# hsinnan75/Kart

Measured on AMD Instinct MI355X. Metric: mapped reads/sec (whole node), 150 bp PE, higher is better.
Workload: dtype u64

## Files before the change

### include/kart_amd.h

```cpp
#ifndef KART_AMD_H
#define KART_AMD_H

#include <stddef.h>
#include <stdint.h>

#ifdef __cplusplus
extern "C" {
#endif

#define KG_OK                0
#define KG_ERR_NO_DEVICE     1
#define KG_ERR_IO            2
#define KG_ERR_ARG           3
#define KG_ERR_CAPACITY      4
#define KG_ERR_NOMEM         5

#define KG_MODE_FAST         0
#define KG_MODE_SENSITIVE    1
#define KG_INPUT_ASCII    0x100

#define KG_OCC_THR_DEFAULT   50

#define KG_SA_SAMPLED        0
#define KG_SA_FULL           1
// ... 44 lines not shown
	uint64_t double_step_bytes;
} kg_traffic_t;

const char *kg_last_error(void);
int  kg_device_count(void);

int  kg_index_load(const char *prefix, int device, int sa_mode, kg_index **out);
void kg_index_destroy(kg_index *ix);
int  kg_index_info(const kg_index *ix, kg_index_info_t *info);
int  kg_index_contig(const kg_index *ix, int i, kg_contig_t *out);

int  kg_rank_sa_batch(kg_index *ix, const uint64_t *k, int64_t n, uint64_t *occ4, uint64_t *sa_walk, uint64_t *sa_full);
int  kg_index_selfcheck(kg_index *ix, int64_t samples, uint64_t seed, uint64_t *disagreements);

void *kg_host_alloc(size_t bytes);
void  kg_host_free(void *p);

int  kg_workspace_create(kg_index *ix, int64_t max_reads, int64_t max_bases, kg_workspace **out);
void kg_workspace_destroy(kg_workspace *ws);
int  kg_workspace_counters(kg_workspace *ws, kg_counters_t *out);
int  kg_workspace_traffic(kg_workspace *ws, kg_traffic_t *out);
int  kg_workspace_set_single_steps(kg_workspace *ws, int enabled);
int  kg_workspace_set_profiling(kg_workspace *ws, int enabled);
int  kg_workspace_kernel_ms(kg_workspace *ws, float ms[4]);

int  kg_seed_batch(kg_workspace *ws, int mode, int min_seed_len, int occ_thr,
                   const uint8_t *enc_bases, const int64_t *read_offsets, int64_t n_reads,
                   int64_t *seed_offsets, const kg_seed **seeds);

int  kg_seed_batch_device(kg_workspace *ws, int mode, int min_seed_len, int occ_thr,
                          const uint8_t *d_enc_bases, const int64_t *d_read_offsets, int64_t n_reads,
                          int64_t n_bases, int64_t *d_seed_offsets, kg_seed *d_seeds,
                          int64_t seed_capacity, void *stream);
int64_t kg_workspace_overflow(kg_workspace *ws);
int64_t kg_workspace_segment_fallbacks(kg_workspace *ws);

typedef struct {
	int64_t posDiff;
	int32_t score;
	int32_t count;
	int64_t first;
} kg_candidate;
int  kg_candidates_batch(kg_workspace *ws, int pacbio, int max_gaps, int64_t n_reads, int64_t n_seeds, int32_t *n_cands,
                         const kg_candidate **cands, int64_t *n_cands_total, const kg_seed **cand_seeds, int64_t *n_cand_seeds_total);

#define KG_ALN_NONE      0
#define KG_ALN_UNMAPPED  1
#define KG_ALN_MAPPED    2
#define KG_ALN_HOST      3
#define KG_ALN_CIGAR_MAX 48
typedef struct {
	int64_t pos;
	int64_t mate_pos;
	int32_t kind;
	int32_t flag, chr, mapq, tlen;
	int32_t score, sub_score;
	int32_t est_lo, est_hi;
	uint8_t has_mate;
	uint8_t flip;
	uint8_t cigar_len;
	uint8_t rescue;
	char    cigar[KG_ALN_CIGAR_MAX];
	int32_t next;
	uint8_t primary;
	uint8_t pad[3];
} kg_aln_record;

typedef struct {
	int64_t paired, distance;
	int64_t lo, hi;
	int32_t unmapped, unique;
	int32_t host_pairs;
	int32_t rescue_wanted;
} kg_chunk_stats;

int  kg_align_batch(kg_workspace *ws, const int64_t *chunk_off, const uint8_t *chunk_paired, int n_chunks,
                    int est_distance, int max_insert, int max_gaps, int multi_hit, int unset_flag,
                    const kg_aln_record **records, kg_chunk_stats *chunk_stats);

#define KG_STATS_RECORDS      0
#define KG_STATS_FLAG0        1
#define KG_STATS_FLAG_BITS    12
#define KG_STATS_PROPER       13
#define KG_STATS_BOTH_MAPPED  14
#define KG_STATS_SINGLETON    15
#define KG_STATS_CIGAR0       16
#define KG_STATS_CIGAR_CLASSES 5
#define KG_STATS_MAPQ0        26
#define KG_STATS_MAPQ_BINS    64
#define KG_STATS_ISIZE0       90
#define KG_STATS_ISIZE_MAX    2048
#define KG_STATS_WORDS        (KG_STATS_ISIZE0 + KG_STATS_ISIZE_MAX + 1)
int  kg_tally_records(const kg_aln_record *records, int64_t n_records, int64_t n_reads, const int64_t *chunk_off, int n_chunks, uint32_t *rows);

#define KG_ALN_CIGAR_POOLED 255
int  kg_longread_batch(kg_workspace *ws, const kg_aln_record **records, const char **cigar_pool, int64_t *cigar_bytes, int64_t *n_host_reads);
int  kg_longread_reasons(kg_workspace *ws, uint64_t out[16]);

int  kg_align_reasons(kg_workspace *ws, uint64_t out[16]);

#define KG_OP_DIAG 0
#define KG_OP_GAP1 1
#define KG_OP_GAP2 2
int  kg_nw_batch(kg_index *ix, const char *frag1, const int64_t *off1, const char *frag2,
                 const int64_t *off2, int64_t n, uint8_t *ops, int32_t *aln_len);
int  kg_nw_batch_device(kg_index *ix, const char *d_frag1, const int64_t *d_off1, const char *d_frag2,
                        const int64_t *d_off2, int64_t n, int64_t max_len, uint8_t *d_ops,
                        int32_t *d_aln_len, void *stream);

int  kg_fragments_batch(kg_index *ix, const char *frag1, const int64_t *off1, const int64_t *gpos, const int32_t *glen, int64_t n,
                        int pacbio, int max_gaps, uint8_t *ops, const int64_t *ops_off, int32_t *aln_len, uint8_t *status);

int  kg_bgzf_deflate(int device, const uint8_t *src, int64_t src_bytes, const int64_t *cuts, int64_t n_cuts,
                     uint8_t *dst, int64_t dst_capacity, int64_t *block_src, int64_t *block_off, int64_t max_blocks, int64_t *n_blocks);

#define KG_INFLATE_OK      0
#define KG_INFLATE_HEADER  1
#define KG_INFLATE_STREAM  2
#define KG_INFLATE_SIZE    3
#define KG_INFLATE_CRC     4
int  kg_bgzf_inflate(int device, const uint8_t *src, int64_t src_bytes, const int64_t *member_off, const int64_t *text_off,
                     int64_t n_members, uint8_t *dst, int64_t dst_capacity, int32_t *status);
typedef struct kg_inflater kg_inflater;
int  kg_inflater_create(int device, int64_t max_src_bytes, int64_t max_text_bytes, int64_t max_members, kg_inflater **out);
int  kg_inflater_reserve(kg_inflater *k, int64_t src_bytes, int64_t text_bytes, int64_t members);
uint8_t *kg_inflater_src(kg_inflater *k);
int  kg_inflater_run(kg_inflater *k, int64_t src_bytes, const int64_t *member_off, const int64_t *text_off, int64_t n_members,
                     const uint8_t **text, const int32_t **status, double *device_ms);
void kg_inflater_destroy(kg_inflater *k);

typedef struct kg_stream kg_stream;
typedef struct {
	int64_t max_reads;
	int64_t max_window;
	int32_t lanes;
	int32_t seed_group;
} kg_stream_config;
int   kg_stream_open(kg_index *ix, const kg_stream_config *cfg, kg_stream **out);
void  kg_stream_close(kg_stream *s);
#define KG_STREAM_FORMAT_SAM 0
#define KG_STREAM_FORMAT_BAM 1
#define KG_STREAM_FORMAT_BAM_BGZF 2
int   kg_stream_set_format(kg_stream *s, int format);
#define KG_STREAM_INPUT_FASTQ 0
#define KG_STREAM_INPUT_FASTA 1
int   kg_stream_set_input(kg_stream *s, int input);
#define KG_STREAM_TAG_MD 1
int   kg_stream_set_tags(kg_stream *s, int tags);
int   kg_stream_set_read_group(kg_stream *s, const char *id, int len);
int   kg_stream_set_unmapped(kg_stream *s, int on);
int   kg_stream_set_stats(kg_stream *s, int on);
char *kg_stream_staging(kg_stream *s, int lane, int file, int64_t *capacity);
int   kg_stream_upload(kg_stream *s, int lane, int file, int64_t from, int64_t to);

typedef struct {
	int64_t begin[2], end[2];
	int32_t eof[2];
	int32_t two_files;
	int32_t paired;
	int32_t chunk_reads;
	int32_t gz_lines;
	int64_t want_reads;
} kg_stream_window;
#define KG_STREAM_STOP_NONE      0
#define KG_STREAM_STOP_IRREGULAR 1
#define KG_STREAM_STOP_TAIL      2
typedef struct {
	int64_t n_reads, n_chunks, n_bases;
	int64_t used[2];
	int32_t stop;
	int32_t done;
} kg_stream_parsed;
int   kg_stream_parse(kg_stream *s, int lane, const kg_stream_window *w, kg_stream_parsed *out);

typedef struct {
	int32_t est_distance, max_insert, max_gaps, multi_hit, unset_flag;
	int32_t fetch_all;
} kg_stream_params;
typedef struct {
	int64_t n_reads, n_chunks;
	const char *sam;
	int64_t sam_bytes;
	const int64_t *sam_off;
	const kg_aln_record *records;
	int64_t n_records;
	const kg_chunk_stats *chunk_stats;
	const int32_t *host_reads;
	int64_t n_host_reads;
	const int64_t *cand_off;
	const kg_candidate *cands;
	const kg_seed *cand_seeds;
	const uint32_t *rec_start[2];
	const uint8_t *bgzf;
	int64_t bgzf_bytes;
	int64_t n_blocks;
	const int64_t *block_src;
	const int64_t *block_off;
	const uint8_t *un[2];
	int64_t un_bytes[2];
	const int64_t *un_off[2];
	int64_t n_units;
	const uint32_t *chunk_tally;
} kg_stream_result;
int   kg_stream_map(kg_stream *s, int lane, const kg_stream_params *prm, kg_stream_result *out);
int   kg_stream_fetch(kg_stream *s, int lane, int64_t first, int64_t count);
int   kg_stream_group_absent(kg_stream *s, int lane, int rounds);
int   kg_stream_group_abort(kg_stream *s);
int   kg_stream_fetch_reads(kg_stream *s, int lane, uint8_t *enc, int64_t *read_off);

typedef struct {
	int64_t batches, reads;
	double parse_ms, seed_ms, chain_ms, align_ms, format_ms, copy_ms;
	double search_kernel_ms;
	int64_t search_kernel_launches;
	double search_useful_bytes;
	double text_in_bytes, text_out_bytes;
	double candidates, candidate_seeds;
	double kernel_ms[16];
	int64_t kernel_launches[16];
	double aln_counts[8];
	double text_checksum[2];
	double un_kernel_ms[2];
	int64_t un_kernel_launches[2];
	double un_bytes;
	double stats_kernel_ms;
	int64_t stats_kernel_launches;
	double stats_bytes;
} kg_stream_timing_t;
int   kg_stream_timing(kg_stream *s, kg_stream_timing_t *out, int reset);

#ifdef __cplusplus
}
#endif
#endif
```

### kart_amd/api.py

```python
from __future__ import annotations

import ctypes as C
import os
import sys

import numpy as np

_HERE = os.path.dirname(os.path.abspath(__file__))
LIB_PATH = os.path.join(_HERE, "libkart_amd.so")

KG_OK = 0
KG_MODE_FAST, KG_MODE_SENSITIVE = 0, 1
KG_INPUT_ASCII = 0x100
KG_SA_SAMPLED, KG_SA_FULL = 0, 1
KG_STREAM_FORMAT_SAM, KG_STREAM_FORMAT_BAM, KG_STREAM_FORMAT_BAM_BGZF = 0, 1, 2
KG_STREAM_INPUT_FASTQ, KG_STREAM_INPUT_FASTA = 0, 1
KG_STREAM_TAG_MD = 1
KG_SA_AUTO = -1
KG_SA_FULL40 = 5
KG_SA_FULL40_WIDE = 6
KG_SA_DENSE4, KG_SA_DENSE8 = 4, 8
KG_OCC_THR_DEFAULT = 50
KG_OP_DIAG, KG_OP_GAP1, KG_OP_GAP2 = 0, 1, 2

SEED_DT = np.dtype([("gPos", "<i8"), ("rPos", "<i4"), ("len", "<i4")])
CAND_DT = np.dtype([("posDiff", "<i8"), ("score", "<i4"), ("count", "<i4"), ("first", "<i8")])
KG_ALN_NONE, KG_ALN_UNMAPPED, KG_ALN_MAPPED, KG_ALN_HOST = 0, 1, 2, 3
KG_ALN_CIGAR_MAX = 48
ALN_DT = np.dtype([("pos", "<i8"), ("mate_pos", "<i8"), ("kind", "<i4"), ("flag", "<i4"), ("chr", "<i4"), ("mapq", "<i4"), ("tlen", "<i4"),
                   ("score", "<i4"), ("sub_score", "<i4"), ("est_lo", "<i4"), ("est_hi", "<i4"), ("has_mate", "u1"), ("flip", "u1"), ("cigar_len", "u1"),
                   ("rescue", "u1"), ("cigar", "S%d" % KG_ALN_CIGAR_MAX), ("next", "<i4"), ("primary", "u1"), ("pad", "u1", (3,))])
CHUNK_STATS_DT = np.dtype([("paired", "<i8"), ("distance", "<i8"), ("lo", "<i8"), ("hi", "<i8"), ("unmapped", "<i4"), ("unique", "<i4"),
                           ("host_pairs", "<i4"), ("rescue_wanted", "<i4")])
assert ALN_DT.itemsize == 112 and CHUNK_STATS_DT.itemsize == 48
KG_STATS_RECORDS, KG_STATS_FLAG0, KG_STATS_FLAG_BITS, KG_STATS_PROPER, KG_STATS_BOTH_MAPPED, KG_STATS_SINGLETON = 0, 1, 12, 13, 14, 15
KG_STATS_CIGAR0, KG_STATS_CIGAR_CLASSES, KG_STATS_MAPQ0, KG_STATS_MAPQ_BINS, KG_STATS_ISIZE0, KG_STATS_ISIZE_MAX = 16, 5, 26, 64, 90, 2048
KG_STATS_WORDS = KG_STATS_ISIZE0 + KG_STATS_ISIZE_MAX + 1

ABI_SYMBOLS = (
    "kg_last_error", "kg_device_count", "kg_index_load", "kg_index_destroy", "kg_index_info",
    "kg_index_contig", "kg_host_alloc", "kg_host_free", "kg_rank_sa_batch", "kg_workspace_create", "kg_workspace_destroy", "kg_workspace_counters", "kg_workspace_traffic",
    "kg_workspace_overflow", "kg_workspace_segment_fallbacks", "kg_workspace_set_profiling", "kg_workspace_set_single_steps", "kg_index_selfcheck", "kg_workspace_kernel_ms", "kg_seed_batch", "kg_candidates_batch", "kg_align_batch", "kg_align_reasons", "kg_seed_batch_device", "kg_nw_batch", "kg_nw_batch_device",
    "kg_fragments_batch", "kg_longread_batch", "kg_longread_reasons",
    "kg_stream_open", "kg_stream_close", "kg_stream_staging", "kg_stream_upload", "kg_stream_parse", "kg_stream_map", "kg_stream_fetch", "kg_stream_fetch_reads", "kg_stream_timing",
    "kg_stream_group_absent", "kg_stream_group_abort", "kg_stream_set_format", "kg_stream_set_input", "kg_stream_set_tags", "kg_stream_set_read_group", "kg_stream_set_unmapped",
    "kg_stream_set_stats", "kg_tally_records",
    "kg_bgzf_deflate", "kg_bgzf_inflate", "kg_inflater_create", "kg_inflater_reserve", "kg_inflater_src", "kg_inflater_run", "kg_inflater_destroy",
)


HOST_LIB_PATH = os.path.join(_HERE, "libkart_host.so")
HOST_ABI_SYMBOLS = ("kh_last_error", "kh_open", "kh_map", "kh_close")


class KartAmdError(RuntimeError):
    pass


class IndexInfo(C.Structure):
    _fields_ = [("genome_size", C.c_int64), ("seq_len", C.c_uint64), ("primary", C.c_uint64),
                ("n_contigs", C.c_int32), ("min_seed_len", C.c_int32), ("sa_mode", C.c_int32),
                ("device", C.c_int32), ("device_bytes", C.c_uint64)]


class Contig(C.Structure):
    _fields_ = [("name", C.c_char_p), ("fwd_start", C.c_int64), ("rev_start", C.c_int64), ("len", C.c_int64)]


class Counters(C.Structure):
    _fields_ = [(n, C.c_uint64) for n in ("searches", "lf1", "lf2", "inv", "sa", "seeds", "bases")]

    def as_dict(self):
        return {n: int(getattr(self, n)) for n, _ in self._fields_}

    def algorithmic_bytes(self) -> int:
        return 64 * (self.lf1 + 2 * self.lf2 + self.inv) + 8 * self.sa + self.bases + 16 * self.seeds


class Traffic(C.Structure):
    _fields_ = [(n, C.c_uint64) for n in ("table_lookups", "rank_steps", "rank_steps_two_lines", "sa_gathers", "text_rounds", "window_words",
                                          "hits", "searches", "sa_entry_bytes", "rank_steps_two_lines_narrow", "double_steps", "double_steps_two_lines",
                                          "triple_steps", "double_step_bytes")]

    def as_dict(self):
        return {n: int(getattr(self, n)) for n, _ in self._fields_}

    def useful_bytes(self, n_reads: int) -> int:
        return (8 * self.table_lookups + 32 * self.rank_steps + self.double_step_bytes + self.sa_entry_bytes * self.sa_gathers + 48 * self.text_rounds
                + 8 * self.window_words + 20 * n_reads + 32 * self.hits)

    def min_lines(self, n_reads: int) -> int:
        return int(self.table_lookups + self.rank_steps + self.rank_steps_two_lines + self.double_steps + self.double_steps_two_lines + self.sa_gathers + self.text_rounds * (1.125 + 1.25)
                   + (8 * self.window_words + 20 * n_reads + 32 * self.hits) / 128)


class StreamConfig(C.Structure):
    _fields_ = [("max_reads", C.c_int64), ("max_window", C.c_int64), ("lanes", C.c_int32), ("seed_group", C.c_int32)]


class StreamWindow(C.Structure):
    _fields_ = [("begin", C.c_int64 * 2), ("end", C.c_int64 * 2), ("eof", C.c_int32 * 2), ("two_files", C.c_int32), ("paired", C.c_int32),
                ("chunk_reads", C.c_int32), ("gz_lines", C.c_int32), ("want_reads", C.c_int64)]


class StreamParsed(C.Structure):
    _fields_ = [("n_reads", C.c_int64), ("n_chunks", C.c_int64), ("n_bases", C.c_int64), ("used", C.c_int64 * 2), ("stop", C.c_int32), ("done", C.c_int32)]


class StreamParams(C.Structure):
    _fields_ = [(n, C.c_int32) for n in ("est_distance", "max_insert", "max_gaps", "multi_hit", "unset_flag", "fetch_all")]


class StreamResult(C.Structure):
    _fields_ = [("n_reads", C.c_int64), ("n_chunks", C.c_int64), ("sam", C.c_void_p), ("sam_bytes", C.c_int64), ("sam_off", C.POINTER(C.c_int64)),
                ("records", C.c_void_p), ("n_records", C.c_int64), ("chunk_stats", C.c_void_p), ("host_reads", C.POINTER(C.c_int32)), ("n_host_reads", C.c_int64),
                ("cand_off", C.POINTER(C.c_int64)), ("cands", C.c_void_p), ("cand_seeds", C.c_void_p), ("rec_start", C.POINTER(C.c_uint32) * 2),
                ("bgzf", C.c_void_p), ("bgzf_bytes", C.c_int64), ("n_blocks", C.c_int64), ("block_src", C.POINTER(C.c_int64)), ("block_off", C.POINTER(C.c_int64)),
                ("un", C.c_void_p * 2), ("un_bytes", C.c_int64 * 2), ("un_off", C.POINTER(C.c_int64) * 2), ("n_units", C.c_int64),
                ("chunk_tally", C.POINTER(C.c_uint32))]


class StreamTiming(C.Structure):
    _fields_ = [("batches", C.c_int64), ("reads", C.c_int64)] + [(n, C.c_double) for n in ("parse_ms", "seed_ms", "chain_ms", "align_ms", "format_ms", "copy_ms", "search_kernel_ms")] + \
               [("search_kernel_launches", C.c_int64)] + [(n, C.c_double) for n in ("search_useful_bytes", "text_in_bytes", "text_out_bytes", "candidates", "candidate_seeds")] + \
               [("kernel_ms", C.c_double * 16), ("kernel_launches", C.c_int64 * 16), ("aln_counts", C.c_double * 8), ("text_checksum", C.c_double * 2),
                ("un_kernel_ms", C.c_double * 2), ("un_kernel_launches", C.c_int64 * 2), ("un_bytes", C.c_double),
                ("stats_kernel_ms", C.c_double), ("stats_kernel_launches", C.c_int64), ("stats_bytes", C.c_double)]

    def as_dict(self):
        return {n: (list(getattr(self, n)) if n.startswith(("kernel_", "aln_counts", "un_kernel_")) else getattr(self, n)) for n, _ in self._fields_}


_lib = None


def _check_one_hip_runtime(L):
    try:
        paths = {l.split()[-1] for l in open("/proc/self/maps") if "libamdhip64" in l}
    except OSError:
        return
    if len({os.path.realpath(p_) for p_ in paths}) > 1 and "torch" in sys.modules and L.kg_device_count() <= 0:
        raise KartAmdError("two HIP runtimes are loaded in this process (%s): import torch BEFORE kart_amd.api.load_library(), or set KART_AMD_NO_TORCH=1 and do "
                           "not import torch afterwards" % ", ".join(sorted(paths)))


def load_library() -> C.CDLL:
    global _lib
    if _lib is not None:
        return _lib
    if not os.path.exists(LIB_PATH):
        raise KartAmdError(f"{LIB_PATH} is missing: build it with `python -c 'import __graft_entry__ as g; g.build()'` "
                           "(there is no CPU fallback)")
    if "torch" not in sys.modules and not os.environ.get("KART_AMD_NO_TORCH"):
        try:
            import torch
        except Exception:
            pass
    L = C.CDLL(LIB_PATH)
    _check_one_hip_runtime(L)
    L.kg_last_error.restype = C.c_char_p
    L.kg_index_load.argtypes = [C.c_char_p, C.c_int, C.c_int, C.POINTER(C.c_void_p)]
    L.kg_index_destroy.argtypes = [C.c_void_p]
    L.kg_index_destroy.restype = None
    L.kg_index_info.argtypes = [C.c_void_p, C.POINTER(IndexInfo)]
    L.kg_index_contig.argtypes = [C.c_void_p, C.c_int, C.POINTER(Contig)]
    L.kg_rank_sa_batch.argtypes = [C.c_void_p, C.c_void_p, C.c_int64, C.c_void_p, C.c_void_p, C.c_void_p]
    L.kg_workspace_create.argtypes = [C.c_void_p, C.c_int64, C.c_int64, C.POINTER(C.c_void_p)]
    L.kg_workspace_destroy.argtypes = [C.c_void_p]
    L.kg_workspace_destroy.restype = None
    L.kg_workspace_counters.argtypes = [C.c_void_p, C.POINTER(Counters)]
    L.kg_workspace_traffic.argtypes = [C.c_void_p, C.POINTER(Traffic)]
    L.kg_workspace_overflow.argtypes = [C.c_void_p]
    L.kg_workspace_set_profiling.argtypes = [C.c_void_p, C.c_int]
    L.kg_workspace_set_single_steps.argtypes = [C.c_void_p, C.c_int]
    L.kg_index_selfcheck.argtypes = [C.c_void_p, C.c_int64, C.c_uint64, C.POINTER(C.c_uint64)]
    L.kg_workspace_kernel_ms.argtypes = [C.c_void_p, C.POINTER(C.c_float * 4)]
    L.kg_workspace_overflow.restype = C.c_int64
    L.kg_workspace_segment_fallbacks.argtypes = [C.c_void_p]
    L.kg_workspace_segment_fallbacks.restype = C.c_int64
    L.kg_seed_batch.argtypes = [C.c_void_p, C.c_int, C.c_int, C.c_int, C.c_void_p, C.c_void_p, C.c_int64,
                                C.c_void_p, C.POINTER(C.c_void_p)]
    L.kg_seed_batch_device.argtypes = [C.c_void_p, C.c_int, C.c_int, C.c_int, C.c_void_p, C.c_void_p, C.c_int64,
                                       C.c_int64, C.c_void_p, C.c_void_p, C.c_int64, C.c_void_p]
    L.kg_candidates_batch.argtypes = [C.c_void_p, C.c_int, C.c_int, C.c_int64, C.c_int64, C.c_void_p, C.POINTER(C.c_void_p), C.POINTER(C.c_int64),
                                      C.POINTER(C.c_void_p), C.POINTER(C.c_int64)]
    L.kg_align_batch.argtypes = [C.c_void_p, C.c_void_p, C.c_void_p, C.c_int, C.c_int, C.c_int, C.c_int, C.c_int, C.c_int, C.POINTER(C.c_void_p), C.c_void_p]
    L.kg_align_reasons.argtypes = [C.c_void_p, C.c_void_p]
    L.kg_nw_batch.argtypes = [C.c_void_p, C.c_void_p, C.c_void_p, C.c_void_p, C.c_void_p, C.c_int64, C.c_void_p, C.c_void_p]
    L.kg_nw_batch_device.argtypes = [C.c_void_p, C.c_void_p, C.c_void_p, C.c_void_p, C.c_void_p, C.c_int64, C.c_int64,
                                     C.c_void_p, C.c_void_p, C.c_void_p]
    L.kg_fragments_batch.argtypes = [C.c_void_p, C.c_void_p, C.c_void_p, C.c_void_p, C.c_void_p, C.c_int64, C.c_int, C.c_int, C.c_void_p, C.c_void_p, C.c_void_p, C.c_void_p]
    L.kg_stream_open.argtypes = [C.c_void_p, C.POINTER(StreamConfig), C.POINTER(C.c_void_p)]
    L.kg_stream_close.argtypes = [C.c_void_p]
    L.kg_stream_close.restype = None
    L.kg_stream_staging.argtypes = [C.c_void_p, C.c_int, C.c_int, C.POINTER(C.c_int64)]
    L.kg_stream_staging.restype = C.c_void_p
    L.kg_stream_upload.argtypes = [C.c_void_p, C.c_int, C.c_int, C.c_int64, C.c_int64]
    L.kg_stream_parse.argtypes = [C.c_void_p, C.c_int, C.POINTER(StreamWindow), C.POINTER(StreamParsed)]
    L.kg_stream_map.argtypes = [C.c_void_p, C.c_int, C.POINTER(StreamParams), C.POINTER(StreamResult)]
    L.kg_stream_fetch.argtypes = [C.c_void_p, C.c_int, C.c_int64, C.c_int64]
    L.kg_stream_fetch_reads.argtypes = [C.c_void_p, C.c_int, C.c_void_p, C.c_void_p]
    L.kg_stream_group_absent.argtypes = [C.c_void_p, C.c_int, C.c_int]
    L.kg_stream_group_abort.argtypes = [C.c_void_p]
    L.kg_stream_set_format.argtypes = [C.c_void_p, C.c_int]
    L.kg_stream_set_input.argtypes = [C.c_void_p, C.c_int]
    L.kg_stream_set_tags.argtypes = [C.c_void_p, C.c_int]
    L.kg_stream_set_read_group.argtypes = [C.c_void_p, C.c_char_p, C.c_int]
    L.kg_stream_set_unmapped.argtypes = [C.c_void_p, C.c_int]
    L.kg_stream_set_stats.argtypes = [C.c_void_p, C.c_int]
    L.kg_tally_records.argtypes = [C.c_void_p, C.c_int64, C.c_int64, C.c_void_p, C.c_int, C.c_void_p]
    L.kg_stream_timing.argtypes = [C.c_void_p, C.POINTER(StreamTiming), C.c_int]
    L.kg_bgzf_deflate.argtypes = [C.c_int, C.c_void_p, C.c_int64, C.c_void_p, C.c_int64, C.c_void_p, C.c_int64, C.c_void_p, C.c_void_p, C.c_int64, C.POINTER(C.c_int64)]
    L.kg_bgzf_inflate.argtypes = [C.c_int, C.c_void_p, C.c_int64, C.c_void_p, C.c_void_p, C.c_int64, C.c_void_p, C.c_int64, C.c_void_p]
    L.kg_inflater_create.argtypes = [C.c_int, C.c_int64, C.c_int64, C.c_int64, C.POINTER(C.c_void_p)]
    L.kg_inflater_reserve.argtypes = [C.c_void_p, C.c_int64, C.c_int64, C.c_int64]
    L.kg_inflater_src.argtypes = [C.c_void_p]
    L.kg_inflater_src.restype = C.c_void_p
    L.kg_inflater_run.argtypes = [C.c_void_p, C.c_int64, C.c_void_p, C.c_void_p, C.c_int64, C.POINTER(C.c_void_p), C.POINTER(C.c_void_p), C.POINTER(C.c_double)]
    L.kg_inflater_destroy.argtypes = [C.c_void_p]
    L.kg_inflater_destroy.restype = None
    _lib = L
    return L


def _check(rc: int, what: str):
    if rc != KG_OK:
        raise KartAmdError(f"{what} failed (status {rc}): {load_library().kg_last_error().decode()}")


def device_count() -> int:
    return int(load_library().kg_device_count())


def _ptr(a):
    return a.ctypes.data_as(C.c_void_p)


BGZF_PAYLOAD = 0xff00


def bgzf_deflate(data: bytes, cuts=None, device: int = 0, dst_capacity: int | None = None, max_blocks: int | None = None):
    cuts = np.ascontiguousarray([0, len(data)] if cuts is None else cuts, dtype=np.int64)
    spans = np.maximum(np.diff(cuts), 0)
    need = int(((spans + BGZF_PAYLOAD - 1) // BGZF_PAYLOAD).sum())
    max_blocks = need if max_blocks is None else int(max_blocks)
    dst_capacity = len(data) + 31 * need if dst_capacity is None else int(dst_capacity)
    src = np.frombuffer(data, dtype=np.uint8) if len(data) else np.zeros(1, dtype=np.uint8)
    dst = np.zeros(max(1, dst_capacity), dtype=np.uint8)
    block_src = np.zeros(max_blocks + 1, dtype=np.int64)
    block_off = np.zeros(max_blocks + 1, dtype=np.int64)
    n = C.c_int64()
    _check(load_library().kg_bgzf_deflate(device, _ptr(src), len(data), _ptr(cuts), len(cuts), _ptr(dst), dst_capacity, _ptr(block_src), _ptr(block_off),
                                          max_blocks, C.byref(n)), "kg_bgzf_deflate")
    return dst[:int(block_off[n.value])].tobytes(), block_src[:n.value + 1].copy(), block_off[:n.value + 1].copy()


KG_INFLATE_OK, KG_INFLATE_HEADER, KG_INFLATE_STREAM, KG_INFLATE_SIZE, KG_INFLATE_CRC = 0, 1, 2, 3, 4
BGZF_MEMBER_MAX = 65536


def bgzf_members(data: bytes):
    member_off, text_off, at = [0], [0], 0
    while at < len(data):
        size = 0
        if len(data) - at >= 18 and data[at:at + 2] == b"\x1f\x8b":
            xlen = int.from_bytes(data[at + 10:at + 12], "little")
            x = at + 12
            while x + 6 <= min(at + 12 + xlen, len(data)):
                slen = int.from_bytes(data[x + 2:x + 4], "little")
                if data[x:x + 2] == b"BC" and slen == 2:
                    size = int.from_bytes(data[x + 4:x + 6], "little") + 1
                    break
                x += 4 + slen
        if size < 8 or at + size > len(data):
            raise KartAmdError(f"no whole BGZF member at byte {at}")
        isize = int.from_bytes(data[at + size - 4:at + size], "little")
        at += size
        member_off.append(at)
        text_off.append(text_off[-1] + (isize if isize <= BGZF_MEMBER_MAX else 0))
    return np.asarray(member_off, dtype=np.int64), np.asarray(text_off, dtype=np.int64)


def bgzf_inflate(data: bytes, member_off=None, text_off=None, device: int = 0, dst_capacity: int | None = None):
    if member_off is None:
        member_off, text_off = bgzf_members(data)
    member_off = np.ascontiguousarray(member_off, dtype=np.int64)
    if text_off is None:
        sizes = [int.from_bytes(data[e - 4:e], "little") if e >= 4 else 0 for e in member_off[1:].tolist()]
        text_off = np.concatenate([[0], np.cumsum([s if s <= BGZF_MEMBER_MAX else 0 for s in sizes], dtype=np.int64)])
    text_off = np.ascontiguousarray(text_off, dtype=np.int64)
    if len(member_off) < 1 or len(member_off) != len(text_off):
        raise KartAmdError("bgzf_inflate: member_off and text_off are tables of n + 1 offsets each")
    n = len(member_off) - 1
    dst_capacity = int(text_off[-1]) if dst_capacity is None else int(dst_capacity)
    src = np.frombuffer(data, dtype=np.uint8) if len(data) else np.zeros(1, dtype=np.uint8)
    dst = np.zeros(max(1, dst_capacity), dtype=np.uint8)
    status = np.full(max(1, n), -1, dtype=np.int32)
    _check(load_library().kg_bgzf_inflate(device, _ptr(src), len(data), _ptr(member_off), _ptr(text_off), n, _ptr(dst), dst_capacity, _ptr(status)),
           "kg_bgzf_inflate")
    return dst[:int(text_off[-1])].tobytes(), text_off.copy(), status[:n].copy()


class Inflater:

    def __init__(self, max_src_bytes: int, max_text_bytes: int, max_members: int, device: int = 0):
        self.lib = load_library()
        h = C.c_void_p()
        _check(self.lib.kg_inflater_create(device, max_src_bytes, max_text_bytes, max_members, C.byref(h)), "kg_inflater_create")
        self.h = h
        self.src_room = max_src_bytes

    def reserve(self, src_bytes: int, text_bytes: int, members: int):
        _check(self.lib.kg_inflater_reserve(self.h, src_bytes, text_bytes, members), "kg_inflater_reserve")
        self.src_room = max(self.src_room, src_bytes)

    def run(self, data: bytes, member_off, text_off):
        member_off = np.ascontiguousarray(member_off, dtype=np.int64)
        text_off = np.ascontiguousarray(text_off, dtype=np.int64)
        n = len(member_off) - 1
        src = self.lib.kg_inflater_src(self.h)
        if 0 < len(data) <= self.src_room and src:
            C.memmove(src, data, len(data))
        text, status, ms = C.c_void_p(), C.c_void_p(), C.c_double()
        _check(self.lib.kg_inflater_run(self.h, len(data), _ptr(member_off), _ptr(text_off), n, C.byref(text), C.byref(status), C.byref(ms)), "kg_inflater_run")
        out = C.string_at(text, int(text_off[-1])) if n and text_off[-1] else b""
        st = np.frombuffer(C.string_at(status, 4 * n), dtype=np.int32).copy() if n else np.zeros(0, dtype=np.int32)
        return out, st, ms.value

    def close(self):
        if self.h:
            self.lib.kg_inflater_destroy(self.h)
            self.h = None


def concat_reads(reads):
    lens = np.fromiter((len(r) for r in reads), dtype=np.int64, count=len(reads))
    offsets = np.zeros(len(reads) + 1, dtype=np.int64)
    np.cumsum(lens, out=offsets[1:])
    enc = np.concatenate(reads).astype(np.uint8, copy=False) if len(reads) else np.zeros(0, dtype=np.uint8)
    return np.ascontiguousarray(enc), offsets


class Workspace:
    def __init__(self, index: "Index", max_reads: int, max_bases: int):
        self.index = index
        self.lib = index.lib
        h = C.c_void_p()
        _check(self.lib.kg_workspace_create(index.h, max_reads, max_bases, C.byref(h)), "kg_workspace_create")
        self.h = h
        self.max_reads, self.max_bases = max_reads, max_bases
# ... 139 lines not shown

    def selfcheck(self, samples: int = 1 << 20, seed: int = 1) -> int:
        bad = C.c_uint64(0)
        _check(self.lib.kg_index_selfcheck(self.h, samples, seed, C.byref(bad)), "kg_index_selfcheck")
        return int(bad.value)

    def rank_sa(self, ks):
        ks = np.ascontiguousarray(ks, dtype=np.uint64)
        n = len(ks)
        occ4 = np.zeros((n, 4), dtype=np.uint64)
        walk = np.zeros(n, dtype=np.uint64)
        full = np.zeros(n, dtype=np.uint64)
        _check(self.lib.kg_rank_sa_batch(self.h, _ptr(ks), n, _ptr(occ4), _ptr(walk), _ptr(full)), "kg_rank_sa_batch")
        return occ4, walk, full

    def _seed(self, reads, mode, min_seed_len, occ_thr):
        enc, offsets = concat_reads(reads)
        ws = self.workspace(len(reads), len(enc))
        so, seeds = ws.seed_batch(enc, offsets, mode, min_seed_len, occ_thr)
        return [seeds[so[i]:so[i + 1]] for i in range(len(reads))]

    def IdentifySeedPairs_FastMode(self, reads, min_seed_len=None, occ_thr=KG_OCC_THR_DEFAULT):
        return self._seed(reads, KG_MODE_FAST, min_seed_len, occ_thr)

    def IdentifySeedPairs_SensitiveMode(self, reads, min_seed_len=None, occ_thr=KG_OCC_THR_DEFAULT):
        return self._seed(reads, KG_MODE_SENSITIVE, min_seed_len, occ_thr)

    def nw_ops(self, pairs):
        n = len(pairs)
        if n == 0:
            return []
        off1 = np.zeros(n + 1, dtype=np.int64)
        off2 = np.zeros(n + 1, dtype=np.int64)
        np.cumsum([len(a) for a, _ in pairs], out=off1[1:])
        np.cumsum([len(b) for _, b in pairs], out=off2[1:])
        f1 = np.frombuffer(b"".join(a for a, _ in pairs) + b"\0", dtype=np.uint8).copy()
        f2 = np.frombuffer(b"".join(b for _, b in pairs) + b"\0", dtype=np.uint8).copy()
        ops = np.zeros(int(off1[n] + off2[n]) + 1, dtype=np.uint8)
        alen = np.zeros(n, dtype=np.int32)
        _check(self.lib.kg_nw_batch(self.h, _ptr(f1), _ptr(off1), _ptr(f2), _ptr(off2), n, _ptr(ops), _ptr(alen)), "kg_nw_batch")
        oo = off1 + off2
        return [ops[oo[i]:oo[i] + alen[i]].copy() for i in range(n)]

    def fragments_ops(self, frags, gpos, glen, pacbio=True, max_gaps=5):
        n = len(frags)
        if n == 0:
            return [], np.zeros(0, np.uint8)
        off1 = np.zeros(n + 1, dtype=np.int64)
        np.cumsum([len(a) for a in frags], out=off1[1:])
        f1 = np.frombuffer(b"".join(frags) + b"\0" * 64, dtype=np.uint8).copy()
        g = np.ascontiguousarray(gpos, dtype=np.int64)
        gl = np.ascontiguousarray(glen, dtype=np.int32)
        oo = np.zeros(n + 1, dtype=np.int64)
        np.cumsum(np.diff(off1) + gl, out=oo[1:])
        ops = np.zeros(int(oo[n]) + 64, dtype=np.uint8)
        alen = np.zeros(n, dtype=np.int32)
        status = np.zeros(n, dtype=np.uint8)
        _check(self.lib.kg_fragments_batch(self.h, _ptr(f1), _ptr(off1), _ptr(g), _ptr(gl), n, int(pacbio), max_gaps, _ptr(ops), _ptr(oo), _ptr(alen), _ptr(status)), "kg_fragments_batch")
        return [ops[oo[i]:oo[i] + alen[i]].copy() for i in range(n)], status

    def GenerateNormalPairAlignment(self, frags, gpos, glen, text, pacbio=True, max_gaps=5):
        ops, status = self.fragments_ops(frags, gpos, glen, pacbio, max_gaps)
        out = []
        for i, a in enumerate(frags):
            out.append(None if status[i] else apply_ops(a, bytes(text[int(gpos[i]):int(gpos[i]) + int(glen[i])]), ops[i]))
        return out, status

    def nw_alignment(self, pairs):
        out = []
        for (s1, s2), ops in zip(pairs, self.nw_ops(pairs)):
            out.append(apply_ops(s1, s2, ops))
        return out


class Stream:

    FORMATS = {"sam": KG_STREAM_FORMAT_SAM, "bam": KG_STREAM_FORMAT_BAM, "bgzf": KG_STREAM_FORMAT_BAM_BGZF}
    INPUTS = {"fastq": KG_STREAM_INPUT_FASTQ, "fasta": KG_STREAM_INPUT_FASTA}

    def __init__(self, index: "Index", max_reads: int = 16000, max_window: int = 8 << 20, lanes: int = 1, seed_group: int = 0):
        self.lib = load_library()
        self.index = index
        cfg = StreamConfig(max_reads, max_window, lanes, seed_group)
        h = C.c_void_p()
        _check(self.lib.kg_stream_open(index.h, C.byref(cfg), C.byref(h)), "kg_stream_open")
        self.h = h
        self.max_window = max_window
        self.last_blocks = None
        self._last_un = {}
        self._last_stats = {}

    def close(self):
        if self.h:
            self.lib.kg_stream_close(self.h)
            self.h = None

    def set_format(self, fmt):
        _check(self.lib.kg_stream_set_format(self.h, self.FORMATS.get(fmt, fmt) if isinstance(fmt, str) else int(fmt)), "kg_stream_set_format")

    def set_input(self, kind):
        _check(self.lib.kg_stream_set_input(self.h, self.INPUTS.get(kind, -1) if isinstance(kind, str) else int(kind)), "kg_stream_set_input")

    def set_tags(self, md: bool = False):
        _check(self.lib.kg_stream_set_tags(self.h, KG_STREAM_TAG_MD if md else 0), "kg_stream_set_tags")

    def set_read_group(self, id):
        if id is None:
            _check(self.lib.kg_stream_set_read_group(self.h, None, 0), "kg_stream_set_read_group")
            return
        try:
            raw = id.encode("ascii") if isinstance(id, str) else bytes(id)
        except UnicodeEncodeError as e:
            raise KartAmdError("kg_stream_set_read_group: the ID holds a character outside '!'..'~': %s" % e) from None
        _check(self.lib.kg_stream_set_read_group(self.h, raw, len(raw)), "kg_stream_set_read_group")

    def set_unmapped(self, on: bool):
        _check(self.lib.kg_stream_set_unmapped(self.h, 1 if on else 0), "kg_stream_set_unmapped")

    def last_unmapped(self, lane: int = 0):
        return self._last_un.get(lane, [])

    def set_stats(self, on: bool):
        _check(self.lib.kg_stream_set_stats(self.h, 1 if on else 0), "kg_stream_set_stats")

    def last_stats(self, lane: int = 0):
        return self._last_stats.get(lane)

    def group_absent(self, lane: int, rounds: int):
        _check(self.lib.kg_stream_group_absent(self.h, lane, rounds), "kg_stream_group_absent")

    def group_abort(self):
        _check(self.lib.kg_stream_group_abort(self.h), "kg_stream_group_abort")

    def parse(self, text1: bytes, text2: bytes | None = None, paired: bool = True, chunk_reads: int = 4000, want_reads: int | None = None,
              eof=(True, True), begin=(0, 0), lane: int = 0, gz_lines: int = 0) -> StreamParsed:
        w = StreamWindow()
        texts = [text1] + ([text2] if text2 is not None else [])
        for f, t in enumerate(texts):
            cap = C.c_int64()
            p = self.lib.kg_stream_staging(self.h, lane, f, C.byref(cap))
            assert p and begin[f] + len(t) <= cap.value
            C.memmove(p + begin[f], t, len(t))
            w.begin[f], w.end[f], w.eof[f] = begin[f], begin[f] + len(t), 1 if eof[f] else 0
            _check(self.lib.kg_stream_upload(self.h, lane, f, begin[f], begin[f] + len(t)), "kg_stream_upload")
        w.two_files = 1 if text2 is not None else 0
        w.paired = 1 if paired else 0
        w.chunk_reads = chunk_reads
        w.gz_lines = 1 if gz_lines else 0
        w.want_reads = want_reads if want_reads is not None else chunk_reads
        out = StreamParsed()
        _check(self.lib.kg_stream_parse(self.h, lane, C.byref(w), C.byref(out)), "kg_stream_parse")
        return out

    def fetch_reads(self, parsed: StreamParsed, lane: int = 0):
        off = np.zeros(parsed.n_reads + 1, dtype=np.int64)
        enc = np.zeros(max(1, parsed.n_bases), dtype=np.uint8)
        _check(self.lib.kg_stream_fetch_reads(self.h, lane, _ptr(enc), _ptr(off)), "kg_stream_fetch_reads")
        raw = enc.tobytes()
        return [raw[off[i]:off[i + 1]] for i in range(parsed.n_reads)]

    def map(self, est_distance: int = 1500, max_insert: int = 1500, max_gaps: int = 5, multi_hit: bool = False, unset_flag: int = 0, lane: int = 0):
        prm = StreamParams(est_distance, max_insert, max_gaps, 1 if multi_hit else 0, unset_flag, 1)
        res = StreamResult()
        _check(self.lib.kg_stream_map(self.h, lane, C.byref(prm), C.byref(res)), "kg_stream_map")
        n = res.n_reads
        off = np.ctypeslib.as_array(res.sam_off, shape=(n + 1,)).copy()
        sam = C.string_at(res.sam, res.sam_bytes)
        host = [int(res.host_reads[i]) for i in range(res.n_host_reads)]
        self._last_un[lane] = [(C.string_at(res.un[f], res.un_bytes[f]) if res.un_bytes[f] else b"", np.ctypeslib.as_array(res.un_off[f], shape=(res.n_units + 1,)).copy())
                               for f in range(2) if res.un_off[f]]
        self._last_stats[lane] = np.ctypeslib.as_array(res.chunk_tally, shape=(int(res.n_chunks), KG_STATS_WORDS)).copy() if res.chunk_tally else None
        self.last_blocks = None
        if res.block_src:
            nb = res.n_blocks
            self.last_blocks = (C.string_at(res.bgzf, res.bgzf_bytes), np.ctypeslib.as_array(res.block_src, shape=(nb + 1,)).copy(),
                                np.ctypeslib.as_array(res.block_off, shape=(nb + 1,)).copy())
        return [sam[off[i]:off[i + 1]] for i in range(n)], host

    def timing(self, reset: bool = False) -> dict:
        t = StreamTiming()
        _check(self.lib.kg_stream_timing(self.h, C.byref(t), 1 if reset else 0), "kg_stream_timing")
        return t.as_dict()


def tally_records(records, n_reads: int, chunk_off):
    lib = load_library()
    recs = np.ascontiguousarray(records, dtype=ALN_DT)
    off = np.ascontiguousarray(chunk_off, dtype=np.int64)
    rows = np.zeros((max(0, len(off) - 1), KG_STATS_WORDS), dtype=np.uint32)
    _check(lib.kg_tally_records(_ptr(recs) if len(recs) else None, len(recs), int(n_reads), _ptr(off), len(off) - 1, _ptr(rows) if rows.size else _ptr(np.zeros(1, np.uint32))),
           "kg_tally_records")
    return rows


def apply_ops(s1: bytes, s2: bytes, ops: np.ndarray):
    a, b = bytearray(), bytearray()
    i = j = 0
    for op in ops:
        if op == KG_OP_DIAG:
            a.append(s1[i]); b.append(s2[j]); i += 1; j += 1
        elif op == KG_OP_GAP1:
            a.append(0x2D); b.append(s2[j]); j += 1
        else:
            a.append(s1[i]); b.append(0x2D); i += 1
    assert i == len(s1) and j == len(s2), "op string does not consume both fragments"
    return bytes(a), bytes(b)


class HostStats(C.Structure):
    _fields_ = [("total_reads", C.c_int64), ("unmapped", C.c_int64), ("unique", C.c_int64), ("paired", C.c_int64), ("distance", C.c_int64),
                ("respeculated", C.c_int64), ("map_seconds", C.c_double), ("sharded", C.c_int32), ("pad", C.c_int32),
                ("stream_reads", C.c_int64), ("stream_batches", C.c_int64), ("stage_ms", C.c_double * 6), ("search_kernel_ms", C.c_double),
                ("search_kernel_launches", C.c_int64), ("search_useful_bytes", C.c_double), ("text_in_bytes", C.c_double), ("text_out_bytes", C.c_double),
                ("candidates", C.c_double), ("candidate_seeds", C.c_double), ("kernel_ms", C.c_double * 16), ("kernel_launches", C.c_int64 * 16), ("aln_counts", C.c_double * 8),
                ("lane_seconds", C.c_double * 6), ("lanes", C.c_int32), ("pad2", C.c_int32), ("text_checksum", C.c_double * 2),
                ("bgzf_device_bytes", C.c_int64), ("bgzf_host_bytes", C.c_int64),
                ("inflate_device_bytes", C.c_int64), ("inflate_host_bytes", C.c_int64), ("inflate_device_ms", C.c_double),
                ("un_kernel_ms", C.c_double * 2), ("un_kernel_launches", C.c_int64 * 2), ("un_bytes", C.c_double),
                ("stats_kernel_ms", C.c_double), ("stats_kernel_launches", C.c_int64), ("stats_bytes", C.c_double)]

    def as_dict(self):
        return {n: (list(getattr(self, n)) if n.startswith(("kernel_", "stage_", "aln_counts", "un_kernel_")) else getattr(self, n)) for n, _ in self._fields_}


_host_lib = None


def load_host_library() -> C.CDLL:
    global _host_lib
    if _host_lib is not None:
        return _host_lib
    if not os.path.exists(HOST_LIB_PATH):
        raise KartAmdError(f"{HOST_LIB_PATH} is missing: build it with `python -c 'import __graft_entry__ as g; g.build()'`")
    load_library()
    L = C.CDLL(HOST_LIB_PATH)
    L.kh_last_error.restype = C.c_char_p
    L.kh_open.argtypes = [C.c_char_p, C.c_int, C.c_int, C.POINTER(C.c_void_p)]
    L.kh_map.argtypes = [C.c_void_p, C.c_int, C.POINTER(C.c_char_p), C.POINTER(HostStats)]
    L.kh_close.argtypes = [C.c_void_p]
    L.kh_close.restype = None
    _host_lib = L
    return L


class HostSession:

    def __init__(self, prefix: str, device: int = 0, threads: int = 4):
        self.lib = load_host_library()
        h = C.c_void_p()
        if self.lib.kh_open(prefix.encode(), device, threads, C.byref(h)) != 0:
            raise KartAmdError("kh_open failed: " + self.lib.kh_last_error().decode())
        self.h = h

    def map(self, args) -> HostStats:
        argv = (C.c_char_p * len(args))(*[str(a).encode() for a in args])
        st = HostStats()
        if self.lib.kh_map(self.h, len(args), argv, C.byref(st)) != 0:
            raise KartAmdError("kh_map failed: " + self.lib.kh_last_error().decode())
        return st

    def close(self):
        if self.h:
            self.lib.kh_close(self.h)
            self.h = None
```

### kart_amd/csrc/abi_stream.hip

```cpp
#include "abi_internal.hpp"
#include "stream_kernels.hpp"
#include "un_kernels.hpp"
#include "stats_kernels.hpp"
#include "bgzf_kernels.hpp"

#include <algorithm>
#include <chrono>
#include <condition_variable>
#include <cstdlib>
#include <cstring>
#include <memory>

#define fail kg_fail

namespace {

enum LaneWord {
	LW_TEXT_BYTES = 0,
	LW_HOST_READS = 1,
	LW_FORMAT_ERRORS = 2,
	LW_EXTRA_RECORDS = 3,
	LW_ALN_COUNTS = 8,
	LW_ALN_TRIVIAL = 14,
	LW_ALN_GENERAL = 15,
	LW_CHECKSUM = 16,
	LW_FETCH_SEEDS = 18,
	LW_BGZF = 20,
	LW_UN_BYTES = 24,
	LW_UN_CTL = 26,
	LW_WORDS = 32
};

struct Lane {
	kg_workspace *ws = nullptr;
	uint8_t *d_text[2] = {nullptr, nullptr};
	int32_t *d_tile[2] = {nullptr, nullptr};
	uint32_t *d_line_end[2] = {nullptr, nullptr};
	uint32_t *d_rec[2] = {nullptr, nullptr};
	uint64_t *d_line_acc[2] = {nullptr, nullptr};
	uint32_t *d_rec_line[2] = {nullptr, nullptr};
	int64_t *d_meta = nullptr;
	int32_t *d_read_len = nullptr;
	void *d_scan = nullptr;
	size_t scan_bytes = 0;
	int32_t *d_sam_len = nullptr, *d_host_list = nullptr;
	int64_t *d_sam_off = nullptr;
	unsigned long long *d_sam_ctl = nullptr;
	uint8_t *d_sam = nullptr;
	int64_t d_sam_capacity = 0;
	int64_t *d_cuts = nullptr, *d_range_first = nullptr;
	int64_t *d_block_src = nullptr, *d_block_off = nullptr;
	int32_t *d_block_bytes = nullptr;
	uint8_t *d_slots = nullptr, *d_bgzf = nullptr;
	int64_t bgzf_blocks = 0, d_bgzf_capacity = 0;
	unsigned long long *d_bgzf_ctl = nullptr;
	void *d_bgzf_scan = nullptr;
	size_t bgzf_scan_bytes = 0;
	int32_t *d_un_len[2] = {nullptr, nullptr};
	int64_t *d_un_off[2] = {nullptr, nullptr};
	uint8_t *d_un[2] = {nullptr, nullptr};
	int64_t d_un_capacity[2] = {0, 0};
	unsigned long long *d_un_ctl = nullptr;
	int64_t *h_un_off[2] = {nullptr, nullptr};
	uint8_t *h_un[2] = {nullptr, nullptr};
	int64_t h_un_capacity[2] = {0, 0};
	uint32_t *d_tally = nullptr, *h_tally = nullptr;
	int64_t tally_capacity = 0, h_tally_capacity = 0;
	uint8_t *h_bgzf = nullptr;
	int64_t h_bgzf_capacity = 0;
	int64_t *h_block_src = nullptr, *h_block_off = nullptr;
	char *h_text[2] = {nullptr, nullptr};
	int64_t *h_meta = nullptr;
	char *h_sam = nullptr;
	int64_t h_sam_capacity = 0;
	int64_t *h_sam_off = nullptr, *h_cand_off = nullptr;
	int32_t *h_host_list = nullptr;
	uint32_t *h_rec_hdr[2] = {nullptr, nullptr};
	kg_aln_record *h_records = nullptr;
	int64_t record_capacity = 0;
	kg_chunk_stats *h_chunk_stats = nullptr;
	int64_t chunk_capacity = 0;
	kg_candidate *h_cands = nullptr;
	kg_seed *h_cand_seeds = nullptr;
	int64_t h_cand_capacity = 0;
	unsigned long long *h_ctl = nullptr;
	int64_t mapped_reads = 0;
	const kg_aln_record *d_records = nullptr;
	kg_stream_window win{};
	kg_stream_parsed parsed{};
	bool have_batch = false;
	bool fasta = false;
	hipEvent_t ev[8] = {nullptr, nullptr, nullptr, nullptr, nullptr, nullptr, nullptr, nullptr};
	hipEvent_t ev_parsed = nullptr;
};

struct SeedGroup {
	int first = 0, size = 0;
	int64_t stride = 0, seg_bases = 0;
	kg_workspace *ws = nullptr;
	unsigned long long *h_ctl = nullptr;
	std::mutex mu;
	std::condition_variable cv;
	int64_t round = 0;
	int arrived = 0;
	bool present[kMaxSeedSegments] = {false};
	int absent_rounds[kMaxSeedSegments] = {0};
	int64_t n_reads[kMaxSeedSegments] = {0};
	int rc = KG_OK;
	int64_t seed_base[kMaxSeedSegments + 1] = {0};
	bool aborted = false;
	int order[kMaxSeedSegments] = {0};
	int n_order = 0, turn = 0;
};

struct GroupTurn {
	SeedGroup *sg = nullptr;
	bool held = false;
	bool acquire(SeedGroup &g, int j)
	{
		sg = &g;
		std::unique_lock<std::mutex> lk(g.mu);
		g.cv.wait(lk, [&]() { return g.aborted || (g.turn < g.n_order && g.order[g.turn] == j); });
		held = !g.aborted;
		return held;
	}
	void release()
	{
		if (!held) return;
		held = false;
		std::lock_guard<std::mutex> lk(sg->mu);
		sg->turn++;
		sg->cv.notify_all();
	}
	~GroupTurn() { release(); }
};

}

struct kg_stream {
	kg_index *ix = nullptr;
	kg_stream_config cfg{};
	int64_t text_capacity = 0, line_capacity = 0, rec_capacity = 0;
	std::vector<Lane> lanes;
	std::vector<std::unique_ptr<SeedGroup>> groups;
	uint8_t *d_chr_names = nullptr;
	int32_t *d_chr_name_off = nullptr;
	int min_seed_len = 13;
	int format = KG_STREAM_FORMAT_SAM;
	int input = KG_STREAM_INPUT_FASTQ;
	int tags = 0;
	bool unmapped = false;
	bool stats = false;
	uint8_t *d_rg = nullptr;
	int rg_len = 0;
	bool fasta_sized = false;
	std::mutex mu;
	kg_stream_timing_t total{};
};

namespace {

void free_lane(Lane &l)
{
	if (l.ws && l.ws->enc_borrowed) l.ws->d_enc = nullptr;
	if (l.ev_parsed) (void)hipEventDestroy(l.ev_parsed);
	if (l.ws) kg_workspace_destroy(l.ws);
	for (int f = 0; f < 2; ++f) {
		if (l.d_text[f]) (void)hipFree(l.d_text[f]);
		if (l.d_tile[f]) (void)hipFree(l.d_tile[f]);
		if (l.d_line_end[f]) (void)hipFree(l.d_line_end[f]);
		if (l.d_rec[f]) (void)hipFree(l.d_rec[f]);
		if (l.d_line_acc[f]) (void)hipFree(l.d_line_acc[f]);
		if (l.d_rec_line[f]) (void)hipFree(l.d_rec_line[f]);
		if (l.h_text[f]) (void)hipHostFree(l.h_text[f]);
		if (l.h_rec_hdr[f]) (void)hipHostFree(l.h_rec_hdr[f]);
		for (void *p : {(void *)l.d_un_len[f], (void *)l.d_un_off[f], (void *)l.d_un[f]})
			if (p) (void)hipFree(p);
		for (void *p : {(void *)l.h_un_off[f], (void *)l.h_un[f]})
			if (p) (void)hipHostFree(p);
	}
	if (l.d_un_ctl) (void)hipFree(l.d_un_ctl);
	if (l.d_tally) (void)hipFree(l.d_tally);
	if (l.h_tally) (void)hipHostFree(l.h_tally);
	for (void *p : {(void *)l.d_meta, (void *)l.d_read_len, l.d_scan, (void *)l.d_sam_len, (void *)l.d_host_list, (void *)l.d_sam_off, (void *)l.d_sam_ctl, (void *)l.d_sam,
	                (void *)l.d_cuts, (void *)l.d_range_first, (void *)l.d_block_src, (void *)l.d_block_off, (void *)l.d_block_bytes, (void *)l.d_slots, (void *)l.d_bgzf,
	                (void *)l.d_bgzf_ctl, l.d_bgzf_scan})
		if (p) (void)hipFree(p);
	for (void *p : {(void *)l.h_meta, (void *)l.h_sam, (void *)l.h_sam_off, (void *)l.h_cand_off, (void *)l.h_host_list, (void *)l.h_records, (void *)l.h_chunk_stats,
	                (void *)l.h_cands, (void *)l.h_cand_seeds, (void *)l.h_ctl, (void *)l.h_bgzf, (void *)l.h_block_src, (void *)l.h_block_off})
		if (p) (void)hipHostFree(p);
	for (hipEvent_t e : l.ev)
		if (e) (void)hipEventDestroy(e);
	l = Lane();
}

FqWindow window_of(const kg_stream *s, const Lane &l, int f)
{
	FqWindow w;
	w.text = l.d_text[f];
	w.begin = l.win.begin[f]; w.end = l.win.end[f]; w.eof = l.win.eof[f];
	w.tile_lines = l.d_tile[f];
	w.line_end = l.d_line_end[f];
	w.line_capacity = s->line_capacity;
	uint32_t *r = l.d_rec[f];
	const size_t c = (size_t)s->rec_capacity;
	w.rec_hdr = r; w.rec_name = r + c; w.rec_seq = r + 2 * c; w.rec_qual = r + 3 * c;
	w.rec_rlen = (int32_t *)(r + 4 * c); w.rec_qlen = (int32_t *)(r + 5 * c);
	w.rec_capacity = s->rec_capacity;
	w.line_acc = l.d_line_acc[f]; w.rec_line = l.d_rec_line[f];
	return w;
}

int64_t out_capacity(const kg_stream_config &cfg, int format)
{
	return 2 * cfg.max_window + (format != KG_STREAM_FORMAT_SAM ? 144 : 64) * cfg.max_reads + 4096;
}

constexpr int kRgMaxId = 255, kRgBamAt = 512, kRgBytes = 1024;
static_assert(6 + kRgMaxId + 16 <= kRgBamAt && kRgBamAt + 4 + kRgMaxId + 16 <= kRgBytes, "both forms of the longest ID and their slack must fit");

int64_t out_capacity(const kg_stream_config &cfg, int format, int tags)
{
	return out_capacity(cfg, format) + ((tags & KG_STREAM_TAG_MD) ? 32 : 0) * cfg.max_reads;
}

enum GrowOrder { kFreeFirst, kAllocFirst };
template <class T> hipError_t grow_device(T *&p, size_t bytes, GrowOrder order = kFreeFirst)
{
	T *old = p;
	if (order == kFreeFirst) {
		if (old) { hipError_t e = hipFree(old); if (e != hipSuccess) return e; }
		p = old = nullptr;
	}
	T *fresh = nullptr;
	hipError_t e = hipMalloc((void **)&fresh, bytes);
	if (e != hipSuccess) return e;
	if (old) (void)hipFree(old);
	p = fresh;
	return hipSuccess;
}
template <class T> hipError_t grow_pinned(T *&p, size_t bytes)
{
	if (p) { hipError_t e = hipHostFree(p); if (e != hipSuccess) return e; }
	p = nullptr;
	return hipHostMalloc((void **)&p, bytes, hipHostMallocDefault);
}

double search_useful_bytes(const kg_index *ix, const unsigned long long *c, int64_t reads)
{
	const double sa_bytes = ix->view.fsa32 ? 4.0 : 8.0;
	return 8.0 * (double)c[17] + 32.0 * (double)c[18] + (double)c[25] + sa_bytes * (double)c[8] + 48.0 * (double)c[20] + 8.0 * (double)c[21] + 20.0 * (double)reads + 32.0 * (double)c[1];
}

template <class T, class C> hipError_t grow_device(T *&p, C &capacity, C want, size_t bytes)
{
	hipError_t e = grow_device(p, bytes);
	capacity = e == hipSuccess ? want : p ? capacity : 0;
	return e;
}
template <class T, class C> hipError_t grow_pinned(T *&p, C &capacity, C want, size_t bytes)
{
	hipError_t e = grow_pinned(p, bytes);
	capacity = e == hipSuccess ? want : p ? capacity : 0;
	return e;
}

bool round_complete(const SeedGroup &sg)
{
	int accounted = sg.arrived;
	for (int i = 0; i < sg.size; ++i) accounted += (!sg.present[i] && sg.absent_rounds[i] != 0) ? 1 : 0;
	return accounted >= sg.size;
}

float elapsed(hipEvent_t a, hipEvent_t b)
{
	float ms = 0;
	if (hipEventElapsedTime(&ms, a, b) != hipSuccess) { (void)hipGetLastError(); return 0; }
	return ms;
}

}

extern "C" {

int kg_stream_open(kg_index *ix, const kg_stream_config *cfg, kg_stream **out)
{
	if (!ix || !cfg || !out) return fail(KG_ERR_ARG, "kg_stream_open: null argument");
	*out = nullptr;
	if (cfg->lanes < 1 || cfg->lanes > 16 || cfg->max_reads < 2 || cfg->max_window < 4096 || cfg->max_window > 0xF0000000ll)
		return fail(KG_ERR_ARG, "kg_stream_open: bad configuration (%d lanes, %lld reads, %lld bytes per window)", cfg->lanes, (long long)cfg->max_reads, (long long)cfg->max_window);
	const int group = cfg->seed_group > 1 ? cfg->seed_group : 0;
	if (group && (group > kMaxSeedSegments || cfg->lanes % group != 0))
		return fail(KG_ERR_ARG, "kg_stream_open: seed_group %d must divide the %d lanes and be at most %d", group, cfg->lanes, kMaxSeedSegments);
	if (!ix->d_text) return fail(KG_ERR_ARG, "kg_stream_open: the index holds no text");
	HIP_TRY(hipSetDevice(ix->device));
	std::unique_ptr<kg_stream, void (*)(kg_stream *)> s(new kg_stream(), kg_stream_close);
	s->ix = ix;
	s->cfg = *cfg;
	s->text_capacity = (cfg->max_window + 4096 + 255) & ~255ll;
	s->line_capacity = cfg->max_window / 16 + 4096;
	s->rec_capacity = s->line_capacity / 4 + 1;
	{
		kg_index_info_t info;
		kg_index_info(ix, &info);
		s->min_seed_len = info.min_seed_len;
		std::vector<int32_t> off{0};
		std::string names;
		for (const ContigRec &c : ix->contigs) { names += c.name; off.push_back((int32_t)names.size()); }
		HIP_TRY(hipMalloc((void **)&s->d_chr_names, names.size() + 16));
		HIP_TRY(hipMalloc((void **)&s->d_chr_name_off, 4 * off.size()));
		HIP_TRY(hipMemcpy(s->d_chr_names, names.data(), names.size(), hipMemcpyHostToDevice));
		HIP_TRY(hipMemcpy(s->d_chr_name_off, off.data(), 4 * off.size(), hipMemcpyHostToDevice));
		HIP_TRY(hipMalloc((void **)&s->d_rg, kRgBytes));
		HIP_TRY(hipMemset(s->d_rg, 0, kRgBytes));
	}
	s->lanes.resize((size_t)cfg->lanes);
	const int64_t n = cfg->max_reads;
	const int64_t seg_bases = (cfg->max_window + 4096 + 64 + 255) & ~255ll;
	for (int g = 0; group && g < cfg->lanes / group; ++g) {
		s->groups.push_back(std::unique_ptr<SeedGroup>(new SeedGroup()));
		SeedGroup *sg = s->groups.back().get();
		sg->first = g * group; sg->size = group;
		sg->stride = n + 8; sg->seg_bases = seg_bases;
		int rc = kg_workspace_create(ix, sg->stride * group, seg_bases * group, &sg->ws);
		if (rc != KG_OK) return rc;
		kg_workspace *gw = sg->ws;
		HIP_TRY(hipMalloc((void **)&gw->d_enc, (size_t)gw->max_bases + 64));
		HIP_TRY(hipMalloc((void **)&gw->d_read_off, 8 * (size_t)(gw->max_reads + 1)));
		HIP_TRY(hipMalloc((void **)&gw->d_seed_off, 8 * (size_t)(gw->max_reads + 1)));
		HIP_TRY(hipMalloc((void **)&gw->group_read_len, 4 * (size_t)(gw->max_reads + 1)));
		HIP_TRY(hipMemsetAsync(gw->d_enc, 'N', (size_t)gw->max_bases + 64, gw->stream));
		HIP_TRY(hipMemsetAsync(gw->d_read_off, 0, 8 * (size_t)(gw->max_reads + 1), gw->stream));
		HIP_TRY(hipMemsetAsync(gw->group_read_len, 0, 4 * (size_t)(gw->max_reads + 1), gw->stream));
		HIP_TRY(hipStreamSynchronize(gw->stream));
		HIP_TRY(hipHostMalloc((void **)&sg->h_ctl, 8 * kCtlWords, hipHostMallocDefault));
		(void)kg_workspace_set_profiling(gw, 1);
	}
	for (size_t li = 0; li < s->lanes.size(); ++li) {
		Lane &l = s->lanes[li];
		int rc = kg_workspace_create(ix, n + 8, cfg->max_window + 4096, &l.ws);
		if (rc != KG_OK) return rc;
		kg_workspace *ws = l.ws;
		if (group) {
			SeedGroup &sg = *s->groups[li / (size_t)group];
			ws->d_enc = sg.ws->d_enc + (int64_t)(li % (size_t)group) * sg.seg_bases;
			ws->enc_borrowed = true;
			HIP_TRY(hipEventCreateWithFlags(&l.ev_parsed, hipEventDisableTiming));
		} else
		HIP_TRY(hipMalloc((void **)&ws->d_enc, (size_t)ws->max_bases + 64));
		HIP_TRY(hipMalloc((void **)&ws->d_read_off, 8 * (size_t)(ws->max_reads + 1)));
		HIP_TRY(hipMalloc((void **)&ws->d_seed_off, 8 * (size_t)(ws->max_reads + 1)));
		(void)kg_workspace_set_profiling(ws, 1);
		const int64_t n_tiles = s->text_capacity / kFqTile + 2;
		for (int f = 0; f < 2; ++f) {
			HIP_TRY(hipMalloc((void **)&l.d_text[f], (size_t)s->text_capacity));
			HIP_TRY(hipMalloc((void **)&l.d_tile[f], 4 * (size_t)(n_tiles + 1)));
			HIP_TRY(hipMalloc((void **)&l.d_line_end[f], 4 * (size_t)s->line_capacity));
			HIP_TRY(hipMalloc((void **)&l.d_rec[f], 4 * 6 * (size_t)s->rec_capacity));
			HIP_TRY(hipHostMalloc((void **)&l.h_text[f], (size_t)s->text_capacity, hipHostMallocDefault));
			HIP_TRY(hipHostMalloc((void **)&l.h_rec_hdr[f], 4 * (size_t)(n + 8), hipHostMallocDefault));
		}
		HIP_TRY(hipMalloc((void **)&l.d_meta, 8 * FQM_WORDS));
		HIP_TRY(hipMalloc((void **)&l.d_read_len, 4 * (size_t)(n + 8)));
		l.scan_bytes = fq_scan_temp_bytes(std::max<int64_t>(n + 8, n_tiles + 1));
		HIP_TRY(hipMalloc(&l.d_scan, l.scan_bytes ? l.scan_bytes : 256));
		HIP_TRY(hipMalloc((void **)&l.d_sam_len, 4 * (size_t)(n + 8)));
		HIP_TRY(hipMalloc((void **)&l.d_host_list, 4 * (size_t)(n + 8)));
		HIP_TRY(hipMalloc((void **)&l.d_sam_off, 8 * (size_t)(n + 8)));
		HIP_TRY(hipMalloc((void **)&l.d_sam_ctl, 8 * 4));
		HIP_TRY(hipHostMalloc((void **)&l.h_meta, 8 * (FQM_WORDS + LW_WORDS), hipHostMallocDefault));
		HIP_TRY(hipHostMalloc((void **)&l.h_sam_off, 8 * (size_t)(n + 8), hipHostMallocDefault));
		HIP_TRY(hipHostMalloc((void **)&l.h_cand_off, 8 * (size_t)(n + 8), hipHostMallocDefault));
		HIP_TRY(hipHostMalloc((void **)&l.h_host_list, 4 * (size_t)(n + 8), hipHostMallocDefault));
		HIP_TRY(hipHostMalloc((void **)&l.h_ctl, 8 * kCtlWords, hipHostMallocDefault));
		l.d_sam_capacity = out_capacity(*cfg, KG_STREAM_FORMAT_SAM);
		HIP_TRY(hipMalloc((void **)&l.d_sam, (size_t)l.d_sam_capacity));
		l.h_sam_capacity = l.d_sam_capacity;
		HIP_TRY(hipHostMalloc((void **)&l.h_sam, (size_t)l.h_sam_capacity, hipHostMallocDefault));
		l.record_capacity = n + n / 4 + 4096;
		HIP_TRY(hipHostMalloc((void **)&l.h_records, sizeof(kg_aln_record) * (size_t)l.record_capacity, hipHostMallocDefault));
		for (hipEvent_t &e : l.ev) HIP_TRY(hipEventCreate(&e));
	}
	HIP_TRY(hipDeviceSynchronize());
	*out = s.release();
	return KG_OK;
}

void kg_stream_close(kg_stream *s)
{
	if (!s) return;
	(void)hipSetDevice(s->ix->device);
	for (Lane &l : s->lanes) free_lane(l);
	for (std::unique_ptr<SeedGroup> &sg : s->groups) {
		if (sg->ws && sg->ws->group_read_len) { (void)hipFree(sg->ws->group_read_len); sg->ws->group_read_len = nullptr; }
		if (sg->ws) kg_workspace_destroy(sg->ws);
		if (sg->h_ctl) (void)hipHostFree(sg->h_ctl);
	}
	if (s->d_chr_names) (void)hipFree(s->d_chr_names);
	if (s->d_chr_name_off) (void)hipFree(s->d_chr_name_off);
	if (s->d_rg) (void)hipFree(s->d_rg);
	delete s;
}

static int bgzf_room(kg_stream *s, Lane &l, int64_t blocks, int64_t bytes)
{
	if (!l.d_cuts) {
		const size_t n = (size_t)s->cfg.max_reads + 8;
		HIP_TRY(hipMalloc((void **)&l.d_cuts, 8 * n));
		HIP_TRY(hipMalloc((void **)&l.d_range_first, 8 * n));
		HIP_TRY(hipMalloc((void **)&l.d_bgzf_ctl, 8 * BGZ_WORDS));
	}
	if (blocks > l.bgzf_blocks) {
		const int64_t want = blocks + blocks / 4 + 64;
		const size_t scan_bytes = bgzf_scan_temp_bytes(std::max<int64_t>(s->cfg.max_reads + 8, want + 1));
		l.bgzf_blocks = 0;
		HIP_TRY(grow_device(l.d_block_src, 8 * (size_t)(want + 1)));
		HIP_TRY(grow_device(l.d_block_off, 8 * (size_t)(want + 1)));
		HIP_TRY(grow_device(l.d_block_bytes, 4 * (size_t)(want + 1)));
		HIP_TRY(grow_device(l.d_slots, (size_t)(want * kBgzfSlot)));
		HIP_TRY(grow_device(l.d_bgzf_scan, scan_bytes ? scan_bytes : 256));
		HIP_TRY(grow_pinned(l.h_block_src, 8 * (size_t)(want + 1)));
		HIP_TRY(grow_pinned(l.h_block_off, 8 * (size_t)(want + 1)));
		l.bgzf_scan_bytes = scan_bytes;
		l.bgzf_blocks = want;
	}
	const int64_t room = bytes + 31 * blocks;
	if (room > l.d_bgzf_capacity) HIP_TRY(grow_device(l.d_bgzf, l.d_bgzf_capacity, room + room / 8, (size_t)(room + room / 8)));
	if (!l.h_bgzf) HIP_TRY(grow_pinned(l.h_bgzf, l.h_bgzf_capacity, room / 2 + 4096, (size_t)(room / 2 + 4096)));
	return KG_OK;
}

static int grow_output(kg_stream *s, int64_t want)
{
	for (Lane &l : s->lanes) {
		if (l.d_sam_capacity < want) {
			HIP_TRY(hipStreamSynchronize(l.ws->stream));
			HIP_TRY(grow_device(l.d_sam, l.d_sam_capacity, want, (size_t)want));
		}
		if (l.h_sam_capacity < want) {
			HIP_TRY(hipStreamSynchronize(l.ws->stream));
			HIP_TRY(grow_pinned(l.h_sam, l.h_sam_capacity, want, (size_t)want));
		}
	}
	return KG_OK;
}

int kg_stream_set_format(kg_stream *s, int format)
{
	if (!s) return fail(KG_ERR_ARG, "kg_stream_set_format: null stream");
	if (format != KG_STREAM_FORMAT_SAM && format != KG_STREAM_FORMAT_BAM && format != KG_STREAM_FORMAT_BAM_BGZF)
		return fail(KG_ERR_ARG, "kg_stream_set_format: unknown format %d (KG_STREAM_FORMAT_SAM, KG_STREAM_FORMAT_BAM or KG_STREAM_FORMAT_BAM_BGZF)", format);
	HIP_TRY(hipSetDevice(s->ix->device));
	const int64_t want = out_capacity(s->cfg, format, s->tags);
	{
		int rc = grow_output(s, want);
		if (rc != KG_OK) return rc;
	}
	for (Lane &l : s->lanes) {
		if (format == KG_STREAM_FORMAT_BAM_BGZF) {
			HIP_TRY(hipStreamSynchronize(l.ws->stream));
			int rc = bgzf_room(s, l, bgzf_max_blocks(want, s->cfg.max_reads / 4000 + s->cfg.max_reads / 100 + 1), want);
			if (rc != KG_OK) return rc;
		}
	}
	s->format = format;
	return KG_OK;
}

int kg_stream_set_tags(kg_stream *s, int tags)
{
	if (!s) return fail(KG_ERR_ARG, "kg_stream_set_tags: null stream");
	if (tags & ~KG_STREAM_TAG_MD) return fail(KG_ERR_ARG, "kg_stream_set_tags: unknown tags 0x%x (KG_STREAM_TAG_MD)", tags);
	HIP_TRY(hipSetDevice(s->ix->device));
	int rc = grow_output(s, out_capacity(s->cfg, s->format, tags));
	if (rc != KG_OK) return rc;
	s->tags = tags;
	return KG_OK;
}

int kg_stream_set_read_group(kg_stream *s, const char *id, int len)
{
	if (!s) return fail(KG_ERR_ARG, "kg_stream_set_read_group: null stream");
	if (!id && len != 0) return fail(KG_ERR_ARG, "kg_stream_set_read_group: no ID but a length of %d", len);
	if (id && (len < 1 || len > kRgMaxId)) return fail(KG_ERR_ARG, "kg_stream_set_read_group: an ID has 1 to %d bytes, not %d (NULL clears the read group)", kRgMaxId, len);
	for (int i = 0; id && i < len; ++i)
		if (id[i] < '!' || id[i] > '~') return fail(KG_ERR_ARG, "kg_stream_set_read_group: byte %d of the ID (0x%02x) is outside '!'..'~'", i, (unsigned)(unsigned char)id[i]);
	HIP_TRY(hipSetDevice(s->ix->device));
	if (id) {
		uint8_t form[kRgBytes] = {0};
		memcpy(form, "\tRG:Z:", 6); memcpy(form + 6, id, (size_t)len);
		memcpy(form + kRgBamAt, "RGZ", 3); memcpy(form + kRgBamAt + 3, id, (size_t)len);
		HIP_TRY(hipMemcpy(s->d_rg, form, kRgBytes, hipMemcpyHostToDevice));
	}
	s->rg_len = id ? len : 0;
	return KG_OK;
}

int kg_stream_set_unmapped(kg_stream *s, int on)
{
	if (!s) return fail(KG_ERR_ARG, "kg_stream_set_unmapped: null stream");
	s->unmapped = on != 0;
	return KG_OK;
}

int kg_stream_set_stats(kg_stream *s, int on)
{
	if (!s) return fail(KG_ERR_ARG, "kg_stream_set_stats: null stream");
	s->stats = on != 0;
	return KG_OK;
}

int kg_stream_set_input(kg_stream *s, int input)
{
	if (!s) return fail(KG_ERR_ARG, "kg_stream_set_input: null stream");
	if (input != KG_STREAM_INPUT_FASTQ && input != KG_STREAM_INPUT_FASTA) return fail(KG_ERR_ARG, "kg_stream_set_input: unknown input %d (KG_STREAM_INPUT_FASTQ or KG_STREAM_INPUT_FASTA)", input);
	HIP_TRY(hipSetDevice(s->ix->device));
	if (input == KG_STREAM_INPUT_FASTA) {
		const size_t want_scan = fa_scan_temp_bytes(s->line_capacity);
		const int64_t rec_capacity = s->line_capacity / 2 + 1;
		for (Lane &l : s->lanes) {
			if (s->fasta_sized) break;
			HIP_TRY(hipStreamSynchronize(l.ws->stream));
			for (int f = 0; f < 2; ++f) {
				HIP_TRY(grow_device(l.d_rec[f], 4 * 6 * (size_t)rec_capacity, kAllocFirst));
				if (!l.d_line_acc[f]) HIP_TRY(hipMalloc((void **)&l.d_line_acc[f], 8 * (size_t)(s->line_capacity + 1)));
				if (!l.d_rec_line[f]) HIP_TRY(hipMalloc((void **)&l.d_rec_line[f], 4 * (size_t)(rec_capacity + 1)));
				HIP_TRY(hipMemset(l.d_line_acc[f], 0, 8 * (size_t)(s->line_capacity + 1)));
				HIP_TRY(hipMemset(l.d_rec_line[f], 0, 4 * (size_t)(rec_capacity + 1)));
			}
			if (l.scan_bytes < want_scan) {
				HIP_TRY(hipStreamSynchronize(l.ws->stream));
				HIP_TRY(grow_device(l.d_scan, l.scan_bytes, want_scan, want_scan));
			}
		}
	}
	if (input == KG_STREAM_INPUT_FASTA && !s->fasta_sized) { s->rec_capacity = s->line_capacity / 2 + 1; s->fasta_sized = true; }
	s->input = input;
	return KG_OK;
}

char *kg_stream_staging(kg_stream *s, int lane, int file, int64_t *capacity)
{
	if (!s || lane < 0 || lane >= (int)s->lanes.size() || file < 0 || file > 1) return nullptr;
	if (capacity) *capacity = s->cfg.max_window;
	return s->lanes[(size_t)lane].h_text[file];
}

int kg_stream_upload(kg_stream *s, int lane, int file, int64_t from, int64_t to)
{
	if (!s || lane < 0 || lane >= (int)s->lanes.size() || file < 0 || file > 1) return fail(KG_ERR_ARG, "kg_stream_upload: bad argument");
	if (from < 0 || to < from || to > s->cfg.max_window) return fail(KG_ERR_ARG, "kg_stream_upload: range [%lld, %lld) outside the staging buffer", (long long)from, (long long)to);
	if (to == from) return KG_OK;
	Lane &l = s->lanes[(size_t)lane];
	HIP_TRY(hipSetDevice(s->ix->device));
	HIP_TRY(hipMemcpyAsync(l.d_text[file] + from, l.h_text[file] + from, (size_t)(to - from), hipMemcpyHostToDevice, l.ws->stream));
	return KG_OK;
}

int kg_stream_parse(kg_stream *s, int lane, const kg_stream_window *w, kg_stream_parsed *out)
{
	if (!s || !w || !out || lane < 0 || lane >= (int)s->lanes.size()) return fail(KG_ERR_ARG, "kg_stream_parse: bad argument");
	Lane &l = s->lanes[(size_t)lane];
	const int nf = w->two_files ? 2 : 1;
	for (int f = 0; f < nf; ++f)
		if (w->begin[f] < 0 || w->end[f] < w->begin[f] || w->end[f] > s->cfg.max_window) return fail(KG_ERR_ARG, "kg_stream_parse: window %d outside the staging buffer", f);
	if (w->chunk_reads < 2 || (w->chunk_reads & 1) || w->want_reads < w->chunk_reads || w->want_reads > s->cfg.max_reads || w->want_reads % w->chunk_reads)
		return fail(KG_ERR_ARG, "kg_stream_parse: want_reads must be a multiple of chunk_reads (an even number) within the stream's batch size");
	HIP_TRY(hipSetDevice(s->ix->device));
	l.win = *w;
	l.have_batch = false;
	l.fasta = s->input == KG_STREAM_INPUT_FASTA;
	kg_workspace *ws = l.ws;
	FqArgs a;
	a.w[0] = window_of(s, l, 0);
	a.w[1] = window_of(s, l, 1);
	if (!w->two_files) { a.w[1].begin = a.w[1].end = 0; a.w[1].eof = 1; }
	a.two_files = w->two_files ? 1 : 0;
	a.paired = w->paired ? 1 : 0;
	a.chunk_reads = w->chunk_reads;
	a.fasta = s->input == KG_STREAM_INPUT_FASTA ? 1 : 0;
	a.gz_lines = w->gz_lines ? 1 : 0;
	a.max_reads = s->cfg.max_reads;
	a.want_reads = w->want_reads;
	a.meta = l.d_meta;
	a.read_len = l.d_read_len;
	a.read_off = ws->d_read_off;
	a.enc = ws->d_enc;
	a.n_reads = 0;
	hipStream_t st = ws->stream;
	KtUse kt_use(ws->profiling ? &ws->kt : nullptr);
	HIP_TRY(hipEventRecord(l.ev[0], st));
	HIP_TRY(launch_fq_parse(a, l.d_scan, l.scan_bytes, s->ix->n_cu, st));
	HIP_TRY(hipMemcpyAsync(l.h_meta, l.d_meta, 8 * FQM_WORDS, hipMemcpyDeviceToHost, st));
	HIP_TRY(kgi_sync(ws));
	kg_stream_parsed &p = l.parsed;
	p.n_reads = l.h_meta[FQM_READS]; p.n_chunks = l.h_meta[FQM_CHUNKS]; p.n_bases = l.h_meta[FQM_BASES];
	p.used[0] = l.h_meta[FQM_USED0]; p.used[1] = w->two_files ? l.h_meta[FQM_USED1] : 0;
	p.stop = (int32_t)l.h_meta[FQM_STOP]; p.done = (int32_t)l.h_meta[FQM_DONE];
	if (p.n_bases > ws->max_bases) return fail(KG_ERR_CAPACITY, "kg_stream_parse: %lld bases exceed the lane's workspace (%lld)", (long long)p.n_bases, (long long)ws->max_bases);
	if (p.n_reads > 0) {
		a.n_reads = p.n_reads;
		HIP_TRY(launch_fq_materialise(a, s->ix->n_cu, st));
		const int64_t r0 = w->two_files ? p.n_reads / 2 : p.n_reads;
		HIP_TRY(hipMemcpyAsync(l.h_rec_hdr[0], a.w[0].rec_hdr, 4 * (size_t)r0, hipMemcpyDeviceToHost, st));
		if (w->two_files) HIP_TRY(hipMemcpyAsync(l.h_rec_hdr[1], a.w[1].rec_hdr, 4 * (size_t)r0, hipMemcpyDeviceToHost, st));
	}
	if (!s->groups.empty() && p.n_reads > 0) {
		SeedGroup &sg = *s->groups[(size_t)lane / (size_t)s->cfg.seed_group];
		const int j = lane - sg.first;
		HIP_TRY(launch_group_publish(ws->d_read_off, p.n_reads, sg.stride, (int64_t)j * sg.seg_bases, sg.ws->d_read_off + (int64_t)j * sg.stride,
		                             sg.ws->group_read_len + (int64_t)j * sg.stride, s->ix->n_cu, st));
		HIP_TRY(hipEventRecord(l.ev_parsed, st));
	}
	HIP_TRY(hipEventRecord(l.ev[1], st));
	l.have_batch = p.n_reads > 0;
	*out = p;
	return KG_OK;
}

static int group_seed(kg_stream *s, int lane, int64_t n, int64_t n_bases, int64_t *n_seeds, bool *was_leader, float *search_ms, double *useful_bytes)
{
	SeedGroup &sg = *s->groups[(size_t)lane / (size_t)s->cfg.seed_group];
	Lane &l = s->lanes[(size_t)lane];
	const int j = lane - sg.first;
	*was_leader = false;
	std::unique_lock<std::mutex> lk(sg.mu);
	if (sg.aborted) return fail(KG_ERR_ARG, "kg_stream_map: the stream's seeding groups were aborted");
	if (sg.absent_rounds[j] < 0) return fail(KG_ERR_ARG, "kg_stream_map: lane %d was declared absent until further notice (kg_stream_group_absent) and arrives with a batch", lane);
	if (!sg.cv.wait_for(lk, std::chrono::seconds(600), [&]() { return sg.absent_rounds[j] == 0 || sg.aborted; })) {
		sg.aborted = true;
		sg.cv.notify_all();
		return fail(KG_ERR_ARG, "kg_stream_map: lane %d waited 600 s for the round it declared itself absent from", lane);
	}
	if (sg.aborted) return fail(KG_ERR_ARG, "kg_stream_map: the stream's seeding groups were aborted");
	const int64_t my_round = sg.round;
	sg.present[j] = true;
	sg.n_reads[j] = n;
	sg.arrived++;
	auto run_round = [&]() {
		kg_workspace *gw = sg.ws;
		int64_t counts[kMaxSeedSegments];
		int rc = KG_OK;
		for (int i = 0; i < sg.size && rc == KG_OK; ++i) {
			counts[i] = sg.present[i] ? sg.n_reads[i] : 0;
			if (hipStreamWaitEvent(gw->stream, s->lanes[(size_t)(sg.first + i)].ev_parsed, 0) != hipSuccess) rc = fail(KG_ERR_NO_DEVICE, "kg_stream_map: hipStreamWaitEvent");
		}
		if (rc == KG_OK) rc = kgi_seed_group(gw, KG_MODE_FAST | KG_INPUT_ASCII, s->min_seed_len, KG_OCC_THR_DEFAULT, sg.size, sg.stride, counts, sg.seed_base);
		if (rc == KG_OK && (hipMemcpyAsync(sg.h_ctl, gw->d_ctl, 8 * kCtlWords, hipMemcpyDeviceToHost, gw->stream) != hipSuccess || kgi_sync(gw) != hipSuccess))
			rc = fail(KG_ERR_NO_DEVICE, "kg_stream_map: reading the group's counters back");
		sg.rc = rc;
		sg.n_order = 0; sg.turn = 0;
		for (int i = 0; i < sg.size; ++i)
			if (sg.present[i]) sg.order[sg.n_order++] = i;
		for (int i = 0; i < sg.size; ++i) {
			sg.present[i] = false;
			if (sg.absent_rounds[i] > 0) sg.absent_rounds[i]--;
		}
		sg.arrived = 0;
		sg.round++;
		sg.cv.notify_all();
	};
	const std::chrono::steady_clock::time_point give_up = std::chrono::steady_clock::now() + std::chrono::seconds(600);
	auto leave = [&]() {
		if (sg.round == my_round && sg.present[j]) { sg.present[j] = false; sg.arrived--; }
	};
	for (;;) {
		if (sg.aborted) { leave(); return fail(KG_ERR_ARG, "kg_stream_map: the stream's seeding groups were aborted"); }
		if (sg.round != my_round) break;
		if (round_complete(sg)) {
			run_round();
			*was_leader = true;
			if (sg.rc == KG_OK) {
				kg_workspace *gw = sg.ws;
				*search_ms = gw->profiling && gw->ev[0] ? elapsed(gw->ev[0], gw->ev[1]) : 0;
				*useful_bytes = search_useful_bytes(s->ix, sg.h_ctl, gw->group_prefix[sg.size]);
			}
			break;
		}
		if (sg.cv.wait_until(lk, give_up) == std::cv_status::timeout) {
			sg.aborted = true;
			sg.cv.notify_all();
			leave();
			return fail(KG_ERR_ARG, "kg_stream_map: lane %d waited 600 s for the other lanes of its seeding group (a lane without a batch must call kg_stream_group_absent)", lane);
		}
	}
	if (sg.rc != KG_OK) return sg.rc;
	const int64_t first = sg.seed_base[j], count = (j + 1 < sg.size ? sg.seed_base[j + 1] : sg.seed_base[sg.size]) - first;
	lk.unlock();
	kg_workspace *ws = l.ws, *gw = sg.ws;
	if (count > ws->seed_capacity) {
		if (ws->d_seeds) HIP_TRY(hipFree(ws->d_seeds));
		ws->d_seeds = nullptr;
		const int64_t want = std::max<int64_t>(count + count / 4, 8 * ws->max_reads + 1024);
		HIP_TRY(hipMalloc((void **)&ws->d_seeds, sizeof(kg_seed) * (size_t)want));
		ws->seed_capacity = want;
	}
	HIP_TRY(launch_group_rebase(gw->d_seed_off + (int64_t)j * sg.stride, n, first, ws->d_seed_off, s->ix->n_cu, ws->stream));
	if (count > 0) HIP_TRY(hipMemcpyAsync(ws->d_seeds, gw->d_seeds + first, sizeof(kg_seed) * (size_t)count, hipMemcpyDeviceToDevice, ws->stream));
	ws->last_reads = n; ws->last_seeds = count; ws->last_cands = -1; ws->last_ascii = true;
	(void)n_bases;
	*n_seeds = count;
	return KG_OK;
}


struct MapCall {
	const kg_stream_params *prm = nullptr;
	int64_t n = 0;
	int n_chunks = 0;
	bool grouped = false, group_leader = false;
	float group_search_ms = 0;
	double group_useful = 0;
	int64_t n_seeds = 0, totals[2] = {0, 0};
	AlnArgs a;
	SamArgs q;
	MdRef mdref{};
	bool md = false;
	bool checksum = false;
	bool bgzf = false;
	bool un = false;
	UnArgs u{};
	int64_t un_bytes[2] = {0, 0};
	bool tally = false;
	int64_t sam_bytes = 0, n_host = 0, extra = 0;
};

static int map_seed(kg_stream *s, int lane, MapCall &m, GroupTurn &turn)
{
	Lane &l = s->lanes[(size_t)lane];
	kg_workspace *ws = l.ws;
	int rc;
	if (m.grouped) {
		rc = group_seed(s, lane, m.n, l.parsed.n_bases, &m.n_seeds, &m.group_leader, &m.group_search_ms, &m.group_useful);
		static const bool no_turns = getenv("KG_GROUP_NO_TURNS") != nullptr;
		SeedGroup &sg = *s->groups[(size_t)lane / (size_t)s->cfg.seed_group];
		if (rc == KG_OK && !no_turns && !turn.acquire(sg, lane - sg.first)) rc = fail(KG_ERR_ARG, "kg_stream_map: the stream's seeding groups were aborted");
		if (rc != KG_OK) {
			std::lock_guard<std::mutex> lk(sg.mu);
			sg.aborted = true;
			sg.cv.notify_all();
		}
	} else rc = kgi_seed_resident(ws, KG_MODE_FAST | KG_INPUT_ASCII, s->min_seed_len, KG_OCC_THR_DEFAULT, m.n, l.parsed.n_bases, &m.n_seeds);
	if (rc != KG_OK) return rc;
	if (!m.grouped) HIP_TRY(hipMemcpyAsync(l.h_ctl, ws->d_ctl, 8 * kCtlWords, hipMemcpyDeviceToHost, ws->stream));
	HIP_TRY(hipEventRecord(l.ev[2], ws->stream));
	return KG_OK;
}

static int map_chain(Lane &l, MapCall &m)
{
	int rc = kgi_chain_resident(l.ws, 0, m.prm->max_gaps, m.totals);
	if (rc != KG_OK) return rc;
	HIP_TRY(hipEventRecord(l.ev[3], l.ws->stream));
	return KG_OK;
}

static int map_report(Lane &l, MapCall &m)
{
	const int n_chunks = m.n_chunks;
	std::vector<int64_t> chunk_off((size_t)n_chunks + 1);
	std::vector<uint8_t> chunk_paired((size_t)n_chunks, (uint8_t)(l.win.paired ? 1 : 0));
	for (int c = 0; c <= n_chunks; ++c) chunk_off[(size_t)c] = std::min<int64_t>(m.n, (int64_t)c * l.win.chunk_reads);
	if (n_chunks > l.chunk_capacity) {
		const int64_t want = n_chunks + n_chunks / 2 + 64;
		HIP_TRY(grow_pinned(l.h_chunk_stats, l.chunk_capacity, want, sizeof(kg_chunk_stats) * (size_t)want));
	}
	int rc = kgi_align_resident(l.ws, chunk_off.data(), chunk_paired.data(), n_chunks, m.prm->est_distance, m.prm->max_insert, m.prm->max_gaps, m.prm->multi_hit,
	                            m.prm->unset_flag, l.record_capacity, m.a);
// ... 140 lines not shown
	if (m.n_chunks > l.h_tally_capacity) {
		const int64_t want = m.n_chunks + m.n_chunks / 2 + 64;
		HIP_TRY(grow_pinned(l.h_tally, l.h_tally_capacity, want, 4 * (size_t)KG_STATS_WORDS * (size_t)want));
	}
	StatsArgs t{};
	t.records = m.a.records;
	t.n_reads = m.n; t.n_records = m.n + m.extra;
	t.chunk_off = m.a.chunk_off; t.n_chunks = m.n_chunks;
	t.rows = l.d_tally;
	HIP_TRY(launch_stats_tally(t, l.ws->stream));
	m.tally = true;
	return KG_OK;
}

static int map_format(kg_stream *s, Lane &l, MapCall &m)
{
	hipStream_t st = l.ws->stream;
	HIP_TRY(launch_text_format(m.q, s->format != KG_STREAM_FORMAT_SAM, m.md ? &m.mdref : nullptr, s->ix->n_cu, st));
	m.checksum = getenv("KG_STREAM_CHECKSUM") != nullptr;
	if (m.checksum) HIP_TRY(launch_sam_checksum(m.q, s->ix->n_cu, st));
	if (m.un && m.un_bytes[0] + m.un_bytes[1] > 0) HIP_TRY(launch_un_copy(m.u, s->ix->n_cu, st));
	if (s->stats) {
		int rc = map_tally(l, m);
		if (rc != KG_OK) return rc;
	}
	if (s->format == KG_STREAM_FORMAT_BAM_BGZF) {
		int rc = map_bgzf(s, l, m);
		if (rc != KG_OK) return rc;
	}
	HIP_TRY(hipEventRecord(l.ev[5], st));
	return KG_OK;
}

static int map_copy_out(Lane &l, MapCall &m, kg_stream_result *out)
{
	kg_workspace *ws = l.ws;
	hipStream_t st = ws->stream;
	const int64_t n = m.n, n_host = m.n_host, extra = m.extra, *totals = m.totals;
	const AlnArgs &a = m.a;
	int64_t *word = l.h_meta + FQM_WORDS;
	int64_t n_blocks = 0, bgzf_bytes = 0;
	if (m.bgzf) {
		HIP_TRY(kgi_sync(ws));
		const int64_t *z = word + LW_BGZF;
		n_blocks = z[BGZ_RUN]; bgzf_bytes = z[BGZ_BYTES];
		if (z[BGZ_BLOCKS] != n_blocks || n_blocks > l.bgzf_blocks) return fail(KG_ERR_NO_DEVICE, "kg_stream_map: the records make %lld BGZF blocks, the lane was sized for %lld", (long long)z[BGZ_BLOCKS], (long long)l.bgzf_blocks);
		if (z[BGZ_ERRORS] != 0) return fail(KG_ERR_NO_DEVICE, "kg_stream_map: %lld BGZF members missed the size computed for them", (long long)z[BGZ_ERRORS]);
		if (bgzf_bytes > l.d_bgzf_capacity) return fail(KG_ERR_NO_DEVICE, "kg_stream_map: %lld bytes of BGZF blocks where at most %lld can be", (long long)bgzf_bytes, (long long)l.d_bgzf_capacity);
		if (bgzf_bytes > l.h_bgzf_capacity) HIP_TRY(grow_pinned(l.h_bgzf, l.h_bgzf_capacity, bgzf_bytes + bgzf_bytes / 4, (size_t)(bgzf_bytes + bgzf_bytes / 4)));
		if (bgzf_bytes > 0) HIP_TRY(hipMemcpyAsync(l.h_bgzf, l.d_bgzf, (size_t)bgzf_bytes, hipMemcpyDeviceToHost, st));
		HIP_TRY(hipMemcpyAsync(l.h_block_src, l.d_block_src, 8 * (size_t)(n_blocks + 1), hipMemcpyDeviceToHost, st));
		HIP_TRY(hipMemcpyAsync(l.h_block_off, l.d_block_off, 8 * (size_t)(n_blocks + 1), hipMemcpyDeviceToHost, st));
	}
	if (m.sam_bytes > 0) HIP_TRY(hipMemcpyAsync(l.h_sam, l.d_sam, (size_t)m.sam_bytes, hipMemcpyDeviceToHost, st));
	HIP_TRY(hipMemcpyAsync(l.h_sam_off, l.d_sam_off, 8 * (size_t)(n + 1), hipMemcpyDeviceToHost, st));
	if (m.un) {
		for (int f = 0; f < (l.win.two_files ? 2 : 1); ++f) {
			if (m.un_bytes[f] > 0) HIP_TRY(hipMemcpyAsync(l.h_un[f], l.d_un[f], (size_t)m.un_bytes[f], hipMemcpyDeviceToHost, st));
			HIP_TRY(hipMemcpyAsync(l.h_un_off[f], l.d_un_off[f], 8 * (size_t)(m.u.n_units + 1), hipMemcpyDeviceToHost, st));
		}
		HIP_TRY(hipMemcpyAsync(&word[LW_UN_CTL], l.d_un_ctl, 8 * 3, hipMemcpyDeviceToHost, st));
	}
	const bool all = m.prm->fetch_all != 0;
	l.mapped_reads = n; l.d_records = a.records;
	if (all) HIP_TRY(hipMemcpyAsync(l.h_records, a.records, sizeof(kg_aln_record) * (size_t)(n + extra), hipMemcpyDeviceToHost, st));
	else if (extra > 0) HIP_TRY(hipMemcpyAsync(l.h_records + n, a.records + n, sizeof(kg_aln_record) * (size_t)extra, hipMemcpyDeviceToHost, st));
	HIP_TRY(hipMemcpyAsync(l.h_chunk_stats, ws->d_chunk_stats, sizeof(kg_chunk_stats) * (size_t)m.n_chunks, hipMemcpyDeviceToHost, st));
	if (m.tally) HIP_TRY(hipMemcpyAsync(l.h_tally, l.d_tally, 4 * (size_t)KG_STATS_WORDS * (size_t)m.n_chunks, hipMemcpyDeviceToHost, st));
	if (all) HIP_TRY(hipMemcpyAsync(l.h_cand_off, ws->d_cand_off, 8 * (size_t)(n + 1), hipMemcpyDeviceToHost, st));
	if (n_host > 0) HIP_TRY(hipMemcpyAsync(l.h_host_list, l.d_host_list, 4 * (size_t)n_host, hipMemcpyDeviceToHost, st));
	if (all && totals[0] > 0) HIP_TRY(hipMemcpyAsync(l.h_cands, ws->d_dense_cands, sizeof(kg_candidate) * (size_t)totals[0], hipMemcpyDeviceToHost, st));
	if (all && totals[1] > 0) HIP_TRY(hipMemcpyAsync(l.h_cand_seeds, ws->d_dense_seeds, sizeof(kg_seed) * (size_t)totals[1], hipMemcpyDeviceToHost, st));
	HIP_TRY(hipMemcpyAsync(&word[LW_FORMAT_ERRORS], l.d_sam_ctl + 1, 8, hipMemcpyDeviceToHost, st));
	HIP_TRY(hipMemcpyAsync(&word[LW_ALN_COUNTS], ws->d_aln_ctl, 8 * 7, hipMemcpyDeviceToHost, st));
	HIP_TRY(hipMemcpyAsync(&word[LW_ALN_GENERAL], ws->d_aln_ctl + 32, 8, hipMemcpyDeviceToHost, st));
	word[LW_CHECKSUM] = word[LW_CHECKSUM + 1] = 0;
	if (m.checksum) HIP_TRY(hipMemcpyAsync(&word[LW_CHECKSUM], l.d_sam_ctl + 2, 16, hipMemcpyDeviceToHost, st));
	HIP_TRY(hipMemcpyAsync(&word[LW_ALN_TRIVIAL], ws->d_aln_ctl + 36, 8, hipMemcpyDeviceToHost, st));
	HIP_TRY(hipEventRecord(l.ev[6], st));
	HIP_TRY(kgi_sync(ws));
	if (word[LW_FORMAT_ERRORS] != 0) return fail(KG_ERR_NO_DEVICE, "kg_stream_map: %lld records were formatted to a size other than the one announced", (long long)word[LW_FORMAT_ERRORS]);
	if (m.un) {
		const bool copied = m.un_bytes[0] + m.un_bytes[1] > 0;
		for (int f = 0; f < 2; ++f)
			if (word[LW_UN_CTL + f] != (copied ? m.un_bytes[f] : 0)) return fail(KG_ERR_NO_DEVICE, "kg_stream_map: %lld bytes of unmapped reads were written for file %d, %lld announced", (long long)word[LW_UN_CTL + f], f, (long long)m.un_bytes[f]);
		if (word[LW_UN_CTL + 2] != 0) return fail(KG_ERR_NO_DEVICE, "kg_stream_map: %lld spans of unmapped reads lie outside their window or buffer", (long long)word[LW_UN_CTL + 2]);
	}
	std::sort(l.h_host_list, l.h_host_list + n_host);
	out->n_reads = n; out->n_chunks = m.n_chunks;
	out->sam = l.h_sam; out->sam_bytes = m.sam_bytes; out->sam_off = l.h_sam_off;
	out->records = l.h_records; out->n_records = n + extra;
	out->chunk_stats = l.h_chunk_stats;
	out->host_reads = l.h_host_list; out->n_host_reads = n_host;
	out->cand_off = l.h_cand_off; out->cands = l.h_cands; out->cand_seeds = l.h_cand_seeds;
	out->rec_start[0] = l.h_rec_hdr[0]; out->rec_start[1] = l.win.two_files ? l.h_rec_hdr[1] : nullptr;
	if (m.bgzf) {
		out->bgzf = l.h_bgzf; out->bgzf_bytes = bgzf_bytes; out->n_blocks = n_blocks;
		out->block_src = l.h_block_src; out->block_off = l.h_block_off;
	}
	if (m.un) {
		for (int f = 0; f < (l.win.two_files ? 2 : 1); ++f) { out->un[f] = l.h_un[f]; out->un_bytes[f] = m.un_bytes[f]; out->un_off[f] = l.h_un_off[f]; }
		out->n_units = m.u.n_units;
	}
	if (m.tally) out->chunk_tally = l.h_tally;
	l.have_batch = false;
	return KG_OK;
}

static void map_account(kg_stream *s, Lane &l, const MapCall &m)
{
	kg_workspace *ws = l.ws;
	const int64_t *word = l.h_meta + FQM_WORDS;
	float sk = 0;
	if (!m.grouped && ws->profiling && ws->ev[0]) sk = elapsed(ws->ev[0], ws->ev[1]);
	double useful = m.grouped ? 0.0 : search_useful_bytes(s->ix, l.h_ctl, m.n);
	if (m.grouped && m.group_leader) { sk = m.group_search_ms; useful = m.group_useful; }
	std::lock_guard<std::mutex> lk(s->mu);
	kg_stream_timing_t &t = s->total;
	t.batches += 1; t.reads += m.n;
	t.parse_ms += elapsed(l.ev[0], l.ev[1]); t.seed_ms += elapsed(l.ev[1], l.ev[2]); t.chain_ms += elapsed(l.ev[2], l.ev[3]);
	t.align_ms += elapsed(l.ev[3], l.ev[4]); t.format_ms += elapsed(l.ev[4], l.ev[5]); t.copy_ms += elapsed(l.ev[5], l.ev[6]);
	t.search_kernel_ms += sk; t.search_kernel_launches += (!m.grouped || m.group_leader) ? 1 : 0; t.search_useful_bytes += useful;
	t.text_in_bytes += (double)((l.parsed.used[0] - l.win.begin[0]) + (l.win.two_files ? l.parsed.used[1] - l.win.begin[1] : 0));
	t.text_out_bytes += (double)m.sam_bytes;
	t.un_bytes += (double)(m.un_bytes[0] + m.un_bytes[1]);
	if (m.tally) t.stats_bytes += 4.0 * KG_STATS_WORDS * (double)m.n_chunks;
	t.candidates += (double)m.totals[0]; t.candidate_seeds += (double)m.totals[1];
	for (int i = 0; i < 8; ++i) t.aln_counts[i] += (double)word[LW_ALN_COUNTS + i];
	t.text_checksum[0] += (double)(uint64_t)word[LW_CHECKSUM]; t.text_checksum[1] += (double)(uint64_t)word[LW_CHECKSUM + 1];
	for (int i = 0; i < KT_SLOTS; ++i) {
		const int used = ws->kt.used[i];
		if (!used) continue;
		ws->kt.used[i] = 0;
		double &ms = i < 16 ? t.kernel_ms[i] : i == KT_STATS ? t.stats_kernel_ms : t.un_kernel_ms[i - 16];
		for (int j = 0; j < used; ++j) ms += elapsed(ws->kt.b[i][j], ws->kt.e[i][j]);
		(i < 16 ? t.kernel_launches[i] : i == KT_STATS ? t.stats_kernel_launches : t.un_kernel_launches[i - 16]) += used;
	}
}

int kg_stream_map(kg_stream *s, int lane, const kg_stream_params *prm, kg_stream_result *out)
{
	if (!s || !prm || !out || lane < 0 || lane >= (int)s->lanes.size()) return fail(KG_ERR_ARG, "kg_stream_map: bad argument");
	Lane &l = s->lanes[(size_t)lane];
	if (!l.have_batch) return fail(KG_ERR_ARG, "kg_stream_map: no parsed batch in lane %d (kg_stream_parse first)", lane);
	memset(out, 0, sizeof(*out));
	HIP_TRY(hipSetDevice(s->ix->device));
	KtUse kt_use(l.ws->profiling ? &l.ws->kt : nullptr);
	MapCall m;
	m.prm = prm;
	m.n = l.parsed.n_reads;
	m.n_chunks = (int)l.parsed.n_chunks;
	m.grouped = !s->groups.empty();
	GroupTurn turn;
	int rc;
	if ((rc = map_seed(s, lane, m, turn)) != KG_OK) return rc;
	if ((rc = map_chain(l, m)) != KG_OK) return rc;
	if ((rc = map_report(l, m)) != KG_OK) return rc;
	if ((rc = map_size_text(s, l, m)) != KG_OK) return rc;
	if ((rc = map_format(s, l, m)) != KG_OK) return rc;
	static const bool turn_early = getenv("KG_GROUP_TURN_EARLY") != nullptr;
	if (turn_early) turn.release();
	if ((rc = map_copy_out(l, m, out)) != KG_OK) return rc;
	map_account(s, l, m);
	return KG_OK;
}

int kg_stream_group_absent(kg_stream *s, int lane, int rounds)
{
	if (!s || lane < 0 || lane >= (int)s->lanes.size()) return fail(KG_ERR_ARG, "kg_stream_group_absent: bad argument");
	if (s->groups.empty()) return KG_OK;
	SeedGroup &sg = *s->groups[(size_t)lane / (size_t)s->cfg.seed_group];
	const int j = lane - sg.first;
	std::unique_lock<std::mutex> lk(sg.mu);
	if (sg.present[j]) return fail(KG_ERR_ARG, "kg_stream_group_absent: lane %d is inside a round", lane);
	if (rounds != 0) {
		Lane &l = s->lanes[(size_t)lane];
		HIP_TRY(hipSetDevice(s->ix->device));
		HIP_TRY(launch_group_publish(l.ws->d_read_off, 0, sg.stride, (int64_t)j * sg.seg_bases, sg.ws->d_read_off + (int64_t)j * sg.stride, sg.ws->group_read_len + (int64_t)j * sg.stride,
		                             s->ix->n_cu, l.ws->stream));
		HIP_TRY(hipEventRecord(l.ev_parsed, l.ws->stream));
	}
	sg.absent_rounds[j] = rounds;
	if (rounds == 0) sg.aborted = false;
	const bool complete = round_complete(sg);
	if (rounds != 0 && sg.arrived > 0 && complete) sg.cv.notify_all();
	if (rounds > 0 && sg.arrived == 0 && complete) {
		for (int i = 0; i < sg.size; ++i)
			if (sg.absent_rounds[i] > 0) sg.absent_rounds[i]--;
		sg.round++;
		sg.cv.notify_all();
	}
	return KG_OK;
}

int kg_stream_group_abort(kg_stream *s)
{
	if (!s) return fail(KG_ERR_ARG, "kg_stream_group_abort: null stream");
	for (std::unique_ptr<SeedGroup> &sg : s->groups) {
		std::lock_guard<std::mutex> lk(sg->mu);
		sg->aborted = true;
		sg->cv.notify_all();
	}
	return KG_OK;
}

int kg_stream_fetch_reads(kg_stream *s, int lane, uint8_t *enc, int64_t *read_off)
{
	if (!s || lane < 0 || lane >= (int)s->lanes.size() || !read_off) return fail(KG_ERR_ARG, "kg_stream_fetch_reads: bad argument");
	Lane &l = s->lanes[(size_t)lane];
	if (!l.have_batch) return fail(KG_ERR_ARG, "kg_stream_fetch_reads: no parsed batch in lane %d", lane);
	HIP_TRY(hipSetDevice(s->ix->device));
	HIP_TRY(kgi_sync(l.ws));
	HIP_TRY(hipMemcpy(read_off, l.ws->d_read_off, 8 * (size_t)(l.parsed.n_reads + 1), hipMemcpyDeviceToHost));
	if (enc && l.parsed.n_bases > 0) HIP_TRY(hipMemcpy(enc, l.ws->d_enc, (size_t)l.parsed.n_bases, hipMemcpyDeviceToHost));
	return KG_OK;
}

int kg_stream_fetch(kg_stream *s, int lane, int64_t first, int64_t count)
{
	if (!s || lane < 0 || lane >= (int)s->lanes.size()) return fail(KG_ERR_ARG, "kg_stream_fetch: bad lane");
	Lane &l = s->lanes[(size_t)lane];
	if (first < 0 || count < 0 || first + count > l.mapped_reads || !l.d_records) return fail(KG_ERR_ARG, "kg_stream_fetch: reads [%lld, %lld) are not of the lane's mapped batch (%lld reads)", (long long)first, (long long)(first + count), (long long)l.mapped_reads);
	if (count == 0) return KG_OK;
	kg_workspace *ws = l.ws;
	HIP_TRY(hipSetDevice(ws->ix->device));
	hipStream_t st = ws->stream;
	int64_t *seeds_at = l.h_meta + FQM_WORDS + LW_FETCH_SEEDS;
	HIP_TRY(hipMemcpyAsync(l.h_records + first, l.d_records + first, sizeof(kg_aln_record) * (size_t)count, hipMemcpyDeviceToHost, st));
	HIP_TRY(hipMemcpyAsync(l.h_cand_off + first, ws->d_cand_off + first, 8 * (size_t)(count + 1), hipMemcpyDeviceToHost, st));
	HIP_TRY(hipMemcpyAsync(&seeds_at[0], ws->d_cseed_off + first, 8, hipMemcpyDeviceToHost, st));
	HIP_TRY(hipMemcpyAsync(&seeds_at[1], ws->d_cseed_off + first + count, 8, hipMemcpyDeviceToHost, st));
	HIP_TRY(kgi_sync(ws));
	const int64_t c0 = l.h_cand_off[first], c1 = l.h_cand_off[first + count], s0 = seeds_at[0], s1 = seeds_at[1];
	if (c0 < 0 || c1 < c0 || c1 > l.h_cand_capacity || s0 < 0 || s1 < s0 || s1 > l.h_cand_capacity) return fail(KG_ERR_NO_DEVICE, "kg_stream_fetch: the batch's candidate offsets are not what kg_stream_map left");
	if (c1 > c0) HIP_TRY(hipMemcpyAsync(l.h_cands + c0, ws->d_dense_cands + c0, sizeof(kg_candidate) * (size_t)(c1 - c0), hipMemcpyDeviceToHost, st));
	if (s1 > s0) HIP_TRY(hipMemcpyAsync(l.h_cand_seeds + s0, ws->d_dense_seeds + s0, sizeof(kg_seed) * (size_t)(s1 - s0), hipMemcpyDeviceToHost, st));
	HIP_TRY(kgi_sync(ws));
	return KG_OK;
}

int kg_tally_records(const kg_aln_record *records, int64_t n_records, int64_t n_reads, const int64_t *chunk_off, int n_chunks, uint32_t *rows)
{
	if (!chunk_off || !rows || n_chunks < 0 || n_reads < 0 || n_records < n_reads || (n_records > 0 && !records)) return fail(KG_ERR_ARG, "kg_tally_records: bad argument");
	for (int c = 0; c < n_chunks; ++c)
		if (chunk_off[c] < 0 || chunk_off[c + 1] < chunk_off[c] || chunk_off[c + 1] > n_reads)
			return fail(KG_ERR_ARG, "kg_tally_records: chunk %d is reads [%lld, %lld) of %lld", c, (long long)chunk_off[c], (long long)chunk_off[c + 1], (long long)n_reads);
	if (n_chunks == 0) return KG_OK;
	struct Buffers {
		kg_aln_record *records = nullptr;
		int64_t *chunk_off = nullptr;
		uint32_t *rows = nullptr;
		~Buffers() { for (void *p : {(void *)records, (void *)chunk_off, (void *)rows}) if (p) (void)hipFree(p); }
	} d;
	const size_t row_bytes = 4 * (size_t)KG_STATS_WORDS * (size_t)n_chunks;
	HIP_TRY(hipMalloc((void **)&d.records, sizeof(kg_aln_record) * (size_t)std::max<int64_t>(n_records, 1)));
	HIP_TRY(hipMalloc((void **)&d.chunk_off, 8 * (size_t)(n_chunks + 1)));
	HIP_TRY(hipMalloc((void **)&d.rows, row_bytes));
	if (n_records > 0) HIP_TRY(hipMemcpy(d.records, records, sizeof(kg_aln_record) * (size_t)n_records, hipMemcpyHostToDevice));
	HIP_TRY(hipMemcpy(d.chunk_off, chunk_off, 8 * (size_t)(n_chunks + 1), hipMemcpyHostToDevice));
	StatsArgs t{};
	t.records = d.records;
	t.n_reads = n_reads; t.n_records = n_records;
	t.chunk_off = d.chunk_off; t.n_chunks = n_chunks;
	t.rows = d.rows;
	HIP_TRY(launch_stats_tally(t, nullptr));
	HIP_TRY(hipDeviceSynchronize());
	HIP_TRY(hipMemcpy(rows, d.rows, row_bytes, hipMemcpyDeviceToHost));
	return KG_OK;
}

int kg_stream_timing(kg_stream *s, kg_stream_timing_t *out, int reset)
{
	if (!s || !out) return fail(KG_ERR_ARG, "kg_stream_timing: null argument");
	std::lock_guard<std::mutex> lk(s->mu);
	*out = s->total;
	if (reset) s->total = kg_stream_timing_t{};
	return KG_OK;
}

}
```

### kart_amd/csrc/host/detail/stream.inc

```

class TaskPool {
public:
	explicit TaskPool(int n, int nice_level = 0)
	{
		for (int t = 0; t < std::max(1, n); ++t) th_.emplace_back([this, nice_level]() {
			if (nice_level > 0) setpriority(PRIO_PROCESS, (id_t)syscall(SYS_gettid), nice_level);
			loop();
		});
	}
	~TaskPool()
	{
		{
			std::lock_guard<std::mutex> lk(mu_);
			stop_ = true;
		}
		cv_.notify_all();
		for (std::thread &t : th_) t.join();
	}
	int size() const { return (int)th_.size(); }
	void run(int n, const std::function<void(int)> &fn)
	{
		if (n <= 0) return;
		if (n == 1) { fn(0); return; }
		Group g;
// ... 181 lines not shown
	bool fetched_all = false;
	std::vector<ChunkState> chunks;
	std::vector<Read> no_reads;
	std::atomic<int> writes_pending{0};
	bool last = false;
	size_t text_begin[2] = {0, 0}, text_end[2] = {0, 0};
};

inline MappedFile &file_of(Source &src, int f) { return f ? src.m2 : src.m1; }
inline const MappedFile &file_of(const Source &src, int f) { return f ? src.m2 : src.m1; }

void stream_record_cursor(const Source &src, const StreamBatch &b, int64_t r, MappedFile &one)
{
	const int f = src.sep ? (int)(r & 1) : 0;
	const int64_t j = src.sep ? r >> 1 : r;
	const MappedFile &mf = file_of(src, f);
	one.data = mf.data; one.size = mf.grow ? b.text_end[f] : mf.map_size; one.pos = b.abs0[f] + (size_t)b.res.rec_start[f][j];
	one.gz_lines = mf.gz_lines;
}

void stream_own_reads_fasta(const Ctx &cx, const Source &src, const StreamBatch &b, ChunkState &ck)
{
	const size_t nh = ck.hq.size();
	std::vector<FastaView> views(nh);
	std::vector<size_t> size_of(nh);
	size_t own = 0;
	for (size_t k = 0; k < nh; ++k) {
		const int64_t r = ck.begin + ck.hq[k];
		MappedFile one;
		stream_record_cursor(src, b, r, one);
		size_of[k] = one.size;
		if (!fasta_view_next(one, views[k])) { fprintf(stderr, "Error! a record the device parsed cannot be read back\n"); exit(1); }
		if (views[k].joined || (cx.opt.paired && (r & 1))) own += (size_t)views[k].rlen;
	}
	ck.own_chars.assign(own, '\0');
	std::string joined;
	size_t at = 0;
	for (size_t k = 0; k < nh; ++k) {
		const FastaView &v = views[k];
		const int64_t r = ck.begin + ck.hq[k];
		const bool flip = cx.opt.paired && (r & 1);
		Read &rd = ck.own_reads[k];
		rd.name = header_view(v.hdr, v.hdr_len);
		rd.raw = std::string_view(v.hdr, v.raw_len);
		rd.rlen = v.rlen;
		if (!v.joined && !flip) { rd.seq = std::string_view(v.seq ? v.seq : "", (size_t)v.rlen); continue; }
		char *dst = &ck.own_chars[at];
		const char *seq = v.seq;
		if (v.joined) {
			char *to = dst;
			if (flip) { joined.assign((size_t)v.rlen, '\0'); to = &joined[0]; }
			fasta_join(file_of(src, src.sep ? (int)(r & 1) : 0).data, size_of[k], v, to);
			seq = to;
		}
		if (flip) revcomp_into(dst, seq, (size_t)v.rlen);
		rd.seq = std::string_view(dst, (size_t)v.rlen);
		at += (size_t)v.rlen;
	}
}

void stream_own_reads_fastq(const Ctx &cx, const Source &src, const StreamBatch &b, ChunkState &ck)
{
	const size_t nh = ck.hq.size();
	size_t flipped = 0;
	std::vector<RecView> views(nh);
	for (size_t k = 0; k < nh; ++k) {
		const int64_t r = ck.begin + ck.hq[k];
		MappedFile one;
		stream_record_cursor(src, b, r, one);
		RecView &v = views[k];
		if (!view_next(one, v)) { fprintf(stderr, "Error! a record the device parsed cannot be read back\n"); exit(1); }
		v.flip = cx.opt.paired && (r & 1);
		if (v.flip) flipped += (size_t)v.rlen;
	}
	ck.own_chars.assign(flipped, '\0');
	size_t at = 0;
	for (size_t k = 0; k < nh; ++k) {
		const RecView &v = views[k];
		Read &rd = ck.own_reads[k];
		rd.name = header_view(v.hdr, v.hdr_len);
		rd.raw = std::string_view(v.hdr, (size_t)v.raw_len);
		rd.rlen = v.rlen;
		int ql = std::min(v.qual_len, v.rlen);
		const char *z = ql > 0 ? (const char *)memchr(v.qual, '\0', (size_t)ql) : nullptr;
		if (z) ql = (int)(z - v.qual);
		rd.qual = std::string_view(v.qual ? v.qual : "", (size_t)ql);
		if (!v.flip) { rd.seq = std::string_view(v.seq, (size_t)v.rlen); continue; }
		revcomp_into(&ck.own_chars[at], v.seq, (size_t)v.rlen);
		rd.seq = std::string_view(&ck.own_chars[at], (size_t)v.rlen);
		rd.qual_rev = true;
		at += (size_t)v.rlen;
	}
}

void stream_own_reads(const Ctx &cx, const Source &src, const StreamBatch &b, ChunkState &ck)
{
	ck.own_reads.assign(ck.hq.size(), Read());
	if (cx.fastq) stream_own_reads_fastq(cx, src, b, ck);
	else stream_own_reads_fasta(cx, src, b, ck);
}

void stream_chunk_pieces(const StreamBatch &b, const ChunkState &ck, std::vector<TextPiece> &out, size_t &total)
{
	const int64_t *off = b.res.sam_off;
	const char *sam = b.res.sam;
	const int step = ck.paired ? 2 : 1;
	int64_t from = ck.begin;
	size_t piece = 0;
	total = 0;
	for (size_t k = 0; k < ck.hq.size(); k += (size_t)step) {
		const int64_t r = ck.begin + ck.hq[k];
		if (off[r] > off[from]) { out.push_back(TextPiece{sam + off[from], (size_t)(off[r] - off[from])}); total += out.back().n; }
		const uint32_t n = ck.host_len[piece++];
		if (n) { out.push_back(TextPiece{nullptr, n}); total += n; }
		from = r + step;
	}
	const int64_t end = ck.begin + ck.count;
	if (off[end] > off[from]) { out.push_back(TextPiece{sam + off[from], (size_t)(off[end] - off[from])}); total += out.back().n; }
}

void stream_chunk_un_pieces(const StreamBatch &b, const ChunkState &ck, int f, std::vector<TextPiece> &out, size_t &total)
{
	const int64_t *off = b.res.un_off[f];
	const char *un = (const char *)b.res.un[f];
	const int step = ck.paired ? 2 : 1;
	int64_t from = ck.begin / step;
	size_t piece = 0;
	total = 0;
	for (size_t k = 0; k < ck.hq.size(); k += (size_t)step) {
		const int64_t u = (ck.begin + ck.hq[k]) / step;
		if (off[u] > off[from]) { out.push_back(TextPiece{un + off[from], (size_t)(off[u] - off[from])}); total += out.back().n; }
		const uint32_t n = ck.un_host_len[f][piece++];
		if (n) { out.push_back(TextPiece{nullptr, n}); total += n; }
		from = u + 1;
	}
	const int64_t end = (ck.begin + ck.count) / step;
	if (off[end] > off[from]) { out.push_back(TextPiece{un + off[from], (size_t)(off[end] - off[from])}); total += out.back().n; }
}

void stream_list_host_reads(const StreamBatch &b, ChunkState &ck)
{
	ck.hq.clear();
	const int32_t *hl = b.res.host_reads, *he = hl + b.res.n_host_reads;
	const int32_t *lo = std::lower_bound(hl, he, (int32_t)ck.begin), *hi = std::lower_bound(lo, he, (int32_t)(ck.begin + ck.count));
	if (ck.force.empty()) {
		for (const int32_t *p = lo; p < hi; ++p) ck.hq.push_back((int)(*p - ck.begin));
		return;
	}
	for (int q = 0; q < ck.count; ++q)
		if (ck.recs[ck.begin + q].kind == KG_ALN_HOST || ck.force[(size_t)q]) ck.hq.push_back(q);
}

constexpr size_t kNoEnd = ~(size_t)0;

inline int64_t stream_block_bytes(int64_t want, int nf, int64_t batches_between, size_t raw, size_t pos, double bpr, int64_t bulk_cap)
{
	const double recs = (double)want / (double)nf;
	double outstanding = (double)(raw - pos) - (double)batches_between * recs * bpr;
	if (outstanding < 0) outstanding = 0;
	const double w = recs * bpr * 1.02 + 65536 - outstanding;
	return (int64_t)std::max(0.0, std::min(w, (double)bulk_cap));
}

struct WindowPlace {
	int64_t begin = 0, end = 0;
	bool eof = false;
	size_t abs0 = 0;
	size_t text_begin = 0, text_end = 0;
	bool fits = false;
};
inline WindowPlace stream_place_window(size_t blk0, size_t blk1, size_t pos, size_t file_end, int64_t carry_cap)
{
	const int64_t carry = (int64_t)(blk0 - pos);
	WindowPlace p;
	p.fits = carry <= carry_cap;
	p.begin = carry_cap - carry;
	p.end = carry_cap + (int64_t)(blk1 - blk0);
	p.eof = blk1 == file_end;
	p.abs0 = blk0 - (size_t)carry_cap;
	p.text_begin = blk0 - (size_t)std::max<int64_t>(0, carry);
	p.text_end = blk1;
	return p;
}

struct StreamBlock {
	size_t blk0[2] = {0, 0}, blk1[2] = {0, 0};
	int64_t want = 0;
};

struct StreamFeed {
	std::mutex mu;
	std::condition_variable cv;
	int nf = 1, K = 1;
	MappedFile *file[2] = {nullptr, nullptr};
	int64_t dispatched = 0;
	int64_t parsed = 0;
	size_t pos[2] = {0, 0};
	size_t raw[2] = {0, 0};
	size_t end[2] = {0, 0};
	double bpr[2] = {0, 0};
	int64_t target = 4000;
	bool finished = false;
	bool fallback = false;
	std::map<int64_t, StreamBatch *> ready;
	int64_t committed = 0;
	bool failed = false;

	bool lane_may_start(int64_t s, const StreamBatch &b)
	{
		std::unique_lock<std::mutex> lk(mu);
		cv.wait(lk, [&]() { return failed || (b.writes_pending.load() == 0 && committed + K > s); });
		return !failed;
	}
	bool claim_block(int64_t s, int64_t bulk_cap, int64_t full_target, StreamBlock &blk)
	{
		std::unique_lock<std::mutex> lk(mu);
		cv.wait(lk, [&]() { return failed || finished || dispatched == s; });
		if (failed || finished) return false;
		blk.want = target;
		int64_t bytes_of[2] = {0, 0};
		bool grows = false;
		for (int f = 0; f < nf; ++f) {
			bytes_of[f] = stream_block_bytes(blk.want, nf, s - parsed, raw[f], pos[f], bpr[f], bulk_cap);
			grows = grows || (file[f]->grow && end[f] == kNoEnd);
		}
		if (grows) {
			size_t upto[2] = {raw[0] + (size_t)bytes_of[0], raw[1] + (size_t)bytes_of[1]};
			lk.unlock();
			size_t have[2] = {0, 0};
			bool ended[2] = {false, false};
			for (int f = 0; f < nf; ++f)
				if (file[f]->grow) have[f] = file[f]->grow->wait_for(upto[f], ended[f]);
			lk.lock();
			if (failed || finished) return false;
			for (int f = 0; f < nf; ++f)
				if (file[f]->grow) {
					if (have[f] > file[f]->size) file[f]->size = file[f]->map_size = have[f];
					if (ended[f]) end[f] = have[f];
				}
		}
		for (int f = 0; f < nf; ++f) {
			blk.blk0[f] = raw[f];
			blk.blk1[f] = std::min(end[f], raw[f] + (size_t)bytes_of[f]);
			raw[f] = blk.blk1[f];
		}
		dispatched = s + 1;
		target = std::min<int64_t>(full_target, target * 4);
		cv.notify_all();
		return true;
	}
	bool wait_parsed_before(int64_t s)
	{
		std::unique_lock<std::mutex> lk(mu);
		cv.wait(lk, [&]() { return failed || finished || parsed == s; });
		return !(failed || finished);
	}
	bool place_in_staging(int64_t s, StreamBatch &b, const StreamBlock &blk, int64_t carry_cap, kg_stream_window &w)
	{
		std::lock_guard<std::mutex> lk(mu);
		bool give_up = false, nothing = true;
		for (int f = 0; f < nf; ++f) {
			const WindowPlace p = stream_place_window(blk.blk0[f], blk.blk1[f], pos[f], end[f], carry_cap);
			if (!p.fits) give_up = true;
			w.begin[f] = p.begin; w.end[f] = p.end; w.eof[f] = p.eof;
			b.abs0[f] = p.abs0; b.text_begin[f] = p.text_begin; b.text_end[f] = p.text_end;
			nothing = nothing && p.end == p.begin;
		}
		if (give_up) fallback = true;
		if (give_up || nothing) hand_over_last(b, s);
		return !(give_up || nothing);
	}
	void publish_parse(int64_t s, StreamBatch &b, bool fits)
	{
		std::lock_guard<std::mutex> lk(mu);
		if (!fits) { finished = true; fallback = true; b.parsed = kg_stream_parsed{}; }
		else {
			for (int f = 0; f < nf; ++f) {
				const size_t before = pos[f];
				pos[f] = b.abs0[f] + (size_t)b.parsed.used[f];
				const int64_t recs = nf == 2 ? b.parsed.n_reads / 2 : b.parsed.n_reads;
				if (recs > 0) bpr[f] = (double)(pos[f] - before) / (double)recs;
			}
			if (b.parsed.done) finished = true;
			else if (b.parsed.stop != KG_STREAM_STOP_NONE) { finished = true; fallback = true; }
			else if (b.parsed.n_reads == 0 && b.win.eof[0] && (nf == 1 || b.win.eof[1])) { finished = true; fallback = true; }
		}
		b.last = finished;
		parsed = s + 1;
		cv.notify_all();
	}
	void hand_over(int64_t s, StreamBatch &b)
	{
		std::lock_guard<std::mutex> lk(mu);
		ready[s] = &b;
		cv.notify_all();
	}

	StreamBatch &take(int64_t s)
	{
		std::unique_lock<std::mutex> lk(mu);
		cv.wait(lk, [&]() { return ready.count(s) != 0; });
		std::map<int64_t, StreamBatch *>::iterator it = ready.find(s);
		StreamBatch *b = it->second;
		ready.erase(it);
		return *b;
	}
	void publish_commit(int64_t s)
	{
		std::lock_guard<std::mutex> lk(mu);
		committed = s + 1;
		cv.notify_all();
	}
	void wait_writes_done(const std::vector<std::unique_ptr<StreamBatch>> &batches)
	{
		std::unique_lock<std::mutex> lk(mu);
		cv.wait(lk, [&]() {
			for (const std::unique_ptr<StreamBatch> &b : batches)
				if (b->writes_pending.load() != 0) return false;
			return true;
		});
	}

private:
	void hand_over_last(StreamBatch &b, int64_t s)
	{
		b.seq = s; b.last = true;
		b.parsed = kg_stream_parsed{}; b.res = kg_stream_result{}; b.chunks.clear();
		finished = true;
		parsed = s + 1;
		ready[s] = &b;
		cv.notify_all();
	}
};

struct LaneTimers {
	enum Step { kWaitLane, kReadUpload, kWaitParse, kParse, kMap, kHostReads, kSteps };
	std::atomic<int64_t> ns[kSteps];
	LaneTimers() { for (std::atomic<int64_t> &a : ns) a.store(0); }
	void add(Step s, double t0) { ns[s] += (int64_t)((now_s() - t0) * 1e9); }
	double seconds(int s) const { return 1e-9 * (double)ns[s].load(); }
};

void add_timing(kg_stream_timing_t &into, const kg_stream_timing_t &from)
{
	into.batches += from.batches; into.reads += from.reads;
	into.parse_ms += from.parse_ms; into.seed_ms += from.seed_ms; into.chain_ms += from.chain_ms; into.align_ms += from.align_ms; into.format_ms += from.format_ms; into.copy_ms += from.copy_ms;
	into.search_kernel_ms += from.search_kernel_ms; into.search_kernel_launches += from.search_kernel_launches; into.search_useful_bytes += from.search_useful_bytes;
	into.text_in_bytes += from.text_in_bytes; into.text_out_bytes += from.text_out_bytes;
	into.candidates += from.candidates; into.candidate_seeds += from.candidate_seeds;
	for (int i = 0; i < 16; ++i) { into.kernel_ms[i] += from.kernel_ms[i]; into.kernel_launches[i] += from.kernel_launches[i]; }
	for (int i = 0; i < 8; ++i) into.aln_counts[i] += from.aln_counts[i];
	into.text_checksum[0] += from.text_checksum[0]; into.text_checksum[1] += from.text_checksum[1];
	for (int i = 0; i < 2; ++i) { into.un_kernel_ms[i] += from.un_kernel_ms[i]; into.un_kernel_launches[i] += from.un_kernel_launches[i]; }
	into.un_bytes += from.un_bytes;
	into.stats_kernel_ms += from.stats_kernel_ms; into.stats_kernel_launches += from.stats_kernel_launches; into.stats_bytes += from.stats_bytes;
}

struct StreamRun {
	Ctx &cx;
	Source &src;
	StreamBackend &sb;
	Writer *writer;
	std::vector<DeferredChunk> *held;
	Stats &st;
	RunTotals &tot;
	std::atomic<int> &est_latest;
	const Shard *shard;
	int64_t &bytes_out;
	static constexpr int chunk_limit = 4000;
	const int nf, K;
	const int64_t bulk_cap, carry_cap;
	const int64_t max_reads, full_target;
	const bool verbose;
	StreamFeed feed;
	std::unique_ptr<TaskPool> pool;
	std::unique_ptr<BamPacker> packer;
	std::vector<std::unique_ptr<StreamBatch>> batches;
	LaneTimers timers;

	StreamRun(Ctx &cx_, Source &src_, StreamBackend &sb_, Writer *writer_, Stats &st_, RunTotals &tot_, std::atomic<int> &est_latest_,
	          std::vector<DeferredChunk> *held_, int64_t &bytes_out_, const Shard *shard_)
		: cx(cx_), src(src_), sb(sb_), writer(writer_), held(held_), st(st_), tot(tot_), est_latest(est_latest_), shard(shard_), bytes_out(bytes_out_),
		  nf(src_.sep ? 2 : 1), K(sb_.lanes()), bulk_cap(sb_.max_window() / 4 * 3), carry_cap(sb_.max_window() - bulk_cap),
		  max_reads(sb_.max_reads() / chunk_limit * chunk_limit),
		  full_target(std::max<int64_t>(chunk_limit, std::min<int64_t>(max_reads, cx_.opt.batch_reads / chunk_limit * chunk_limit))),
		  verbose(getenv("KART_AMD_VERBOSE") != nullptr)
	{
		{ kg_stream_timing_t drop{}; sb.timing(drop, true); }
	}

	void prime(int64_t ramp_from)
	{
		feed.nf = nf; feed.K = K;
		for (int f = 0; f < nf; ++f) {
			MappedFile &mf = file_of(src, f);
			feed.file[f] = &mf;
			feed.pos[f] = feed.raw[f] = mf.pos;
			feed.end[f] = mf.size;
			if (mf.grow) {
				bool ended = false;
				const size_t have = mf.grow->wait_for(mf.pos + ((size_t)1 << 18), ended);
				mf.size = mf.map_size = have;
				feed.end[f] = ended ? have : kNoEnd;
			}
		}
		feed.target = std::max<int64_t>(chunk_limit, std::min<int64_t>(full_target, ramp_from));
		for (int f = 0; f < nf; ++f) {
			const MappedFile &mf = file_of(src, f);
			size_t lo = feed.pos[f], hi = std::min(std::min(feed.end[f], mf.size), lo + ((size_t)1 << 18));
			int64_t lines = 0, blank = 0;
			count_lines(mf.data, lo, hi, lines, blank);
			feed.bpr[f] = !cx.fastq ? fasta_bytes_per_record(mf.data, lo, hi) : lines >= 8 ? 4.0 * (double)(hi - lo) / (double)lines : 400.0;
		}
		if (writer && !held) {
			double text = 0;
			for (int f = 0; f < nf; ++f) text += feed.end[f] != kNoEnd ? (double)(feed.end[f] - feed.pos[f]) : 4.5 * (double)src.gz_packed[f];
			writer->expect((size_t)(1.2 * text));
		}
		pool.reset(new TaskPool(std::max(1, cx.opt.threads / 2), 5));
		if (cx.opt.bam && writer && !held) packer.reset(new BamPacker(writer, std::max(1, cx.opt.threads), &feed.mu, &feed.cv));
		for (int l = 0; l < K; ++l) { batches.emplace_back(new StreamBatch()); batches.back()->lane = l; }
	}

	void lane_thread(int lane)
	{
		pin_lane_thread();
		StreamBatch &b = *batches[(size_t)lane];
		for (int64_t s = lane; lane_batch(b, s); s += K) {}
		sb.group_absent(lane, -1);
	}
	bool lane_batch(StreamBatch &b, int64_t s)
	{
		StreamBlock blk;
		kg_stream_window w{};
		if (!wait_lane_free(b, s)) return false;
		if (!feed.claim_block(s, bulk_cap, full_target, blk)) return false;
		read_and_upload(b.lane, blk);
		if (!place_window(b, s, blk, w)) return false;
		parse_and_publish(b, s, blk.want, w);
		map_or_sit_out(b);
		feed.hand_over(s, b);
		return !b.last;
	}
	bool wait_lane_free(StreamBatch &b, int64_t s)
	{
		double t0 = now_s();
		if (!feed.lane_may_start(s, b)) return false;
		timers.add(LaneTimers::kWaitLane, t0);
		return true;
	}
	void read_and_upload(int lane, const StreamBlock &blk)
	{
		double t0 = now_s();
		for (int f = 0; f < nf; ++f) {
			const MappedFile &mf = file_of(src, f);
			char *stg = sb.staging(lane, f);
			const size_t piece = (size_t)8 << 20, blk0 = blk.blk0[f], blk1 = blk.blk1[f];
			for (size_t a = blk0; a < blk1; a += piece) {
				size_t e = std::min(blk1, a + piece);
				static const bool use_pread = getenv("KART_AMD_NO_PREAD") == nullptr;
				bool done = false;
				if (use_pread && mf.fd >= 0) {
					size_t got = 0;
					while (got < e - a) {
						ssize_t k = ::pread(mf.fd, stg + carry_cap + (a - blk0) + got, e - a - got, (off_t)(a + got));
						if (k <= 0) break;
						got += (size_t)k;
					}
					done = got == e - a;
				}
				if (!done) memcpy(stg + carry_cap + (a - blk0), mf.data + a, e - a);
				sb.upload(lane, f, carry_cap + (int64_t)(a - blk0), carry_cap + (int64_t)(e - blk0));
			}
		}
		timers.add(LaneTimers::kReadUpload, t0);
	}
	bool place_window(StreamBatch &b, int64_t s, const StreamBlock &blk, kg_stream_window &w)
	{
		double t0 = now_s();
		const bool go_on = feed.wait_parsed_before(s);
		timers.add(LaneTimers::kWaitParse, t0);
		if (!go_on || !feed.place_in_staging(s, b, blk, carry_cap, w)) return false;
		for (int f = 0; f < nf; ++f) {
			const int64_t carry = carry_cap - w.begin[f];
			if (carry > 0) {
				memcpy(sb.staging(b.lane, f) + w.begin[f], file_of(src, f).data + (blk.blk0[f] - (size_t)carry), (size_t)carry);
				sb.upload(b.lane, f, w.begin[f], carry_cap);
			}
		}
		return true;
	}
	void parse_and_publish(StreamBatch &b, int64_t s, int64_t want, kg_stream_window &w)
	{
		w.two_files = src.sep ? 1 : 0;
		w.gz_lines = src.m1.gz_lines ? 1 : 0;
		w.paired = cx.opt.paired ? 1 : 0;
		w.chunk_reads = chunk_limit;
		w.want_reads = std::min<int64_t>(max_reads, std::max<int64_t>(chunk_limit, (want + want / 4) / chunk_limit * chunk_limit));
		b.win = w;
		b.seq = s;
		double tp = now_s();
		const bool fits = sb.parse(b.lane, w, b.parsed);
		timers.add(LaneTimers::kParse, tp);
		feed.publish_parse(s, b, fits);
	}
	void map_or_sit_out(StreamBatch &b)
	{
		if (b.parsed.n_reads <= 0) { b.res = kg_stream_result{}; b.chunks.clear(); sb.group_absent(b.lane, 1); return; }
		kg_stream_params prm;
		prm.est_distance = b.est_dev = est_latest.load();
		prm.max_insert = cx.opt.max_insert; prm.max_gaps = cx.opt.max_gaps; prm.multi_hit = cx.opt.multi_hit ? 1 : 0; prm.unset_flag = g_unset_flag;
		static const bool fetch_all_env = getenv("KART_AMD_FETCH_ALL") != nullptr;
		prm.fetch_all = (g_check_align || fetch_all_env) ? 1 : 0;
		b.fetched_all = prm.fetch_all != 0;
		double tm = now_s();
		sb.map(b.lane, prm, b.res);
		timers.add(LaneTimers::kMap, tm);
		double th = now_s();
		host_stage(b);
		timers.add(LaneTimers::kHostReads, th);
	}
	void host_stage(StreamBatch &b)
	{
		const kg_stream_result &res = b.res;
		b.chunks.assign((size_t)res.n_chunks, ChunkState());
		std::vector<int> busy;
		for (int c = 0; c < (int)res.n_chunks; ++c) {
			ChunkState &ck = b.chunks[(size_t)c];
			ck.begin = c * chunk_limit;
			ck.count = (int)std::min<int64_t>(chunk_limit, res.n_reads - ck.begin);
			ck.paired = cx.opt.paired;
			ck.recs = res.records;
			ck.dev = res.chunk_stats[c];
			ck.stream = true;
			if (cx.stats) {
				if (!res.chunk_tally) run_fail("the device stream returned no tally for a batch of a -stats run");
				else ck.dev_tally = res.chunk_tally + (size_t)c * KG_STATS_WORDS;
				ck.n_records_reads = res.n_reads; ck.n_records = res.n_records;
			}
			stream_list_host_reads(b, ck);
			if (!ck.hq.empty()) busy.push_back(c);
		}
		for (ChunkState &ck : b.chunks)
			if (ck.hq.empty()) {
				chunk_stage_a(cx, b.no_reads, res.cand_off, res.cands, res.cand_seeds, ck, b.est_dev); ck.text.clear(); ck.host_len.clear(); ck.st.total_reads = ck.count;
				if (cx.stats) { ck.tally = std::make_shared<Tally>(); chunk_device_tally(ck); }
			}
		if (!b.fetched_all)
			for (int c : busy) sb.fetch(b.lane, b.chunks[(size_t)c].begin, b.chunks[(size_t)c].count);
		pool->run((int)busy.size(), [&](int i) {
			ChunkState &ck = b.chunks[(size_t)busy[(size_t)i]];
			stream_own_reads(cx, src, b, ck);
			chunk_stage_a(cx, b.no_reads, res.cand_off, res.cands, res.cand_seeds, ck, b.est_dev);
		});
		std::vector<NwJobs *> parts;
		for (int c : busy)
			if (b.chunks[(size_t)c].jobs.size() > 0) parts.push_back(&b.chunks[(size_t)c].jobs);
		if (!parts.empty()) cx.kern.nw_batch(parts);
		pool->run((int)busy.size(), [&](int i) { chunk_stage_c(cx, b.no_reads, b.chunks[(size_t)busy[(size_t)i]]); });
	}

	void commit()
	{
		for (int64_t s = 0;; ++s) {
			StreamBatch &b = feed.take(s);
			double t0 = now_s();
			if (!b.chunks.empty()) {
				settle_estimates(b);
				emit_chunks(b);
				est_latest.store(est_speculated(cx, shard, tot.iPaired, tot.iDistance));
				if (shard && shard->active() && shard->rank == 0) { shard->rdv->hint_paired.store(tot.iPaired); shard->rdv->hint_distance.store(tot.iDistance); }
			}
			tot.t_commit += now_s() - t0;
			const bool last = b.last;
			const size_t text_begin[2] = {b.text_begin[0], b.text_begin[1]};
			feed.publish_commit(s);
			for (int f = 0; f < nf; ++f)
				if (file_of(src, f).grow) file_of(src, f).grow->release(text_begin[f]);
			if (last) break;
		}
	}
	void settle_estimates(StreamBatch &b)
	{
		const kg_stream_result &res = b.res;
		for (;;) {
			std::vector<std::pair<size_t, int>> redo;
			int64_t paired = tot.iPaired, distance = tot.iDistance;
			for (size_t c = 0; c < b.chunks.size(); ++c) {
				ChunkState &ck = b.chunks[c];
				if (ck.paired) {
					int est_true = held ? ck.est_used : est_distance(cx, paired, distance);
					bool valid = est_true == ck.est_used ||
					             (ck.ps.lo < est_true && est_true <= ck.ps.hi &&
					              (!ck.ps.rescue_used || std::min(est_true, cx.opt.max_insert) == std::min(ck.est_used, cx.opt.max_insert)));
					if (!valid) redo.emplace_back(c, est_true);
				}
				paired += ck.ps.paired;
				distance += ck.ps.distance;
			}
			if (redo.empty()) return;
			st.respeculated += (int64_t)redo.size();
			if (!b.fetched_all)
				for (const std::pair<size_t, int> &rd_ : redo) sb.fetch(b.lane, b.chunks[rd_.first].begin, b.chunks[rd_.first].count);
			pool->run((int)redo.size(), [&](int i) {
				ChunkState &ck = b.chunks[redo[(size_t)i].first];
				ck.force_invalid_pairs(redo[(size_t)i].second, cx.opt.max_insert);
				stream_list_host_reads(b, ck);
				stream_own_reads(cx, src, b, ck);
				chunk_stage_a(cx, b.no_reads, res.cand_off, res.cands, res.cand_seeds, ck, redo[(size_t)i].second);
				if (ck.jobs.size() > 0) { std::vector<NwJobs *> parts{&ck.jobs}; cx.kern.nw_batch(parts); }
				chunk_stage_c(cx, b.no_reads, ck);
			});
		}
	}
	void emit_chunks(StreamBatch &b)
	{
		const int n_un = cx.un_writer[0] ? (cx.un_writer[1] ? 2 : 1) : 0;
		b.writes_pending.store((int)b.chunks.size() * (1 + n_un));
		for (size_t c = 0; c < b.chunks.size(); ++c) {
			ChunkState &ck = b.chunks[c];
			for (int f = 0; f < n_un; ++f) {
				std::vector<TextPiece> un_pieces;
				size_t un_total = 0;
				stream_chunk_un_pieces(b, ck, f, un_pieces, un_total);
				cx.un_writer[f]->push_pieces(std::move(un_pieces), un_total, std::move(ck.un_text[f]), &b.writes_pending, &feed.mu, &feed.cv);
			}
			std::vector<TextPiece> pieces;
			size_t total = 0;
			stream_chunk_pieces(b, ck, pieces, total);
			if (!held) bytes_out += (int64_t)total;
			tot.dev_reads += ck.count - ck.n_host; tot.host_reads += ck.n_host;
			tot.iPaired += ck.ps.paired;
			tot.iDistance += ck.ps.distance;
			st.stream_reads += ck.count;
			if (held) { hold_chunk(b, ck, pieces, total); continue; }
			st.total_reads += ck.count;
			st.unmapped += ck.st.unmapped;
			st.unique += ck.st.unique;
			if (st.tally && ck.tally) *st.tally += *ck.tally;
			if (packer) packer->push(std::move(pieces), total, std::move(ck.text), &b.writes_pending, &b.res);
			else writer->push_pieces(std::move(pieces), total, std::move(ck.text), &b.writes_pending, &feed.mu, &feed.cv);
		}
	}
	void hold_chunk(StreamBatch &b, ChunkState &ck, const std::vector<TextPiece> &pieces, size_t total)
	{
		DeferredChunk d;
		d.paired = ck.paired; d.est_used = ck.est_used; d.ps = ck.ps; d.st = ck.st;
		d.st.total_reads = ck.count;
		d.text.reserve(total);
		size_t host_at = 0;
		for (const TextPiece &tp : pieces) {
			if (tp.p) d.text.append(tp.p, tp.n);
			else { d.text.append(ck.text.data() + host_at, tp.n); host_at += tp.n; }
		}
		const int64_t r0 = ck.begin;
		d.from_stream = true;
		d.count = ck.count;
		d.fpos[0] = b.abs0[0] + (size_t)b.res.rec_start[0][src.sep ? r0 >> 1 : r0];
		d.fpos[1] = src.sep ? b.abs0[1] + (size_t)b.res.rec_start[1][r0 >> 1] : 0;
		held->push_back(std::move(d));
		if (writer) write_held_chunk(writer, held->back());
		b.writes_pending.fetch_sub(1);
	}

	void finish()
	{
		feed.wait_writes_done(batches);
		if (packer) packer->finish();
		if (packer) { st.bgzf_device_bytes += packer->device_bytes(); st.bgzf_host_bytes += packer->host_bytes(); }
		src.m1.pos = feed.pos[0];
		if (src.sep) src.m2.pos = feed.pos[1];
	}
	void report()
	{
		for (int i = 0; i < LaneTimers::kSteps; ++i) st.lane_seconds[i] += timers.seconds(i);
		st.lanes = K;
		if (verbose)
			fprintf(stdout, "stream: lane-thread seconds (summed over %d lanes): waiting for the lane %.3f | read + upload %.3f | waiting for the parse before %.3f | parse %.3f | map (device) %.3f | host reads %.3f\n", K,
			        timers.seconds(LaneTimers::kWaitLane), timers.seconds(LaneTimers::kReadUpload), timers.seconds(LaneTimers::kWaitParse), timers.seconds(LaneTimers::kParse),
			        timers.seconds(LaneTimers::kMap), timers.seconds(LaneTimers::kHostReads));
		kg_stream_timing_t t{};
		if (!sb.timing(t, true) || t.batches <= 0) return;
		add_timing(st.device, t);
		if (verbose)
			fprintf(stdout, "device stream: %lld batches, %lld reads | stage ms (summed over lanes, stages of different lanes overlap): parse %.1f, seed %.1f (search_kernel %.2f in %lld launches, %.1f useful MB), chain %.1f, align %.1f, format %.1f, copy-out %.1f | text in %.1f MB, out %.1f MB\n",
			        (long long)t.batches, (long long)t.reads, t.parse_ms, t.seed_ms, t.search_kernel_ms, (long long)t.search_kernel_launches, t.search_useful_bytes / 1e6, t.chain_ms, t.align_ms,
			        t.format_ms, t.copy_ms, t.text_in_bytes / 1e6, t.text_out_bytes / 1e6);
	}
};

bool map_library_stream(Ctx &cx, Source &src, StreamBackend &sb, Writer *writer, Stats &st, RunTotals &tot, std::atomic<int> &est_latest,
                        std::vector<DeferredChunk> *held, int64_t &bytes_out, int64_t ramp_from, const Shard *shard)
{
	StreamRun run(cx, src, sb, writer, st, tot, est_latest, held, bytes_out, shard);
	run.prime(ramp_from);
	for (int l = 0; l < run.K; ++l) sb.group_absent(l, 0);
	std::vector<std::thread> threads;
	for (int l = 0; l < run.K; ++l) threads.emplace_back([&run, l]() { run.lane_thread(l); });
	run.commit();
	for (std::thread &t : threads) t.join();
	run.finish();
	run.report();
	return !run.feed.fallback;
}
```

### kart_amd/csrc/host/hip_backend.cpp

```cpp
#include <cstdio>
#include <algorithm>
#include <cstdlib>
#include <cstring>
#include <functional>
#include <atomic>
#include <memory>
#include <mutex>
#include <stdexcept>
#include <thread>
#include <ctime>

#include "mapper.hpp"

namespace kart {

int cli_main(int argc, char **argv, KernelBackend *(*make_backend)(const Options &, std::string &));

namespace {

[[noreturn]] void die(const char *what)
{
	fprintf(stderr, "Error! %s: %s\n", what, kg_last_error());
	exit(1);
}

static double now_sec()
{
	struct timespec ts;
	clock_gettime(CLOCK_MONOTONIC, &ts);
	return ts.tv_sec + 1e-9 * ts.tv_nsec;
}

class HipStream : public StreamBackend {
public:
	HipStream(kg_stream *s, const kg_stream_config &cfg) : s_(s), cfg_(cfg) {}
	~HipStream() override { kg_stream_close(s_); }
	int lanes() const override { return cfg_.lanes; }
	int64_t max_reads() const override { return cfg_.max_reads; }
	int64_t max_window() const override { return cfg_.max_window; }
	char *staging(int lane, int file) override { return kg_stream_staging(s_, lane, file, nullptr); }
	void upload(int lane, int file, int64_t from, int64_t to) override
	{
		if (kg_stream_upload(s_, lane, file, from, to) != KG_OK) die("kg_stream_upload");
	}
	bool parse(int lane, const kg_stream_window &w, kg_stream_parsed &out) override
	{
		int rc = kg_stream_parse(s_, lane, &w, &out);
		if (rc == KG_ERR_CAPACITY) return false;
		if (rc != KG_OK) die("kg_stream_parse");
		return true;
	}
	void map(int lane, const kg_stream_params &p, kg_stream_result &out) override
	{
		if (kg_stream_map(s_, lane, &p, &out) != KG_OK) die("kg_stream_map");
	}
	void fetch(int lane, int64_t first, int64_t count) override
	{
		if (kg_stream_fetch(s_, lane, first, count) != KG_OK) die("kg_stream_fetch");
	}
	bool timing(kg_stream_timing_t &t, bool reset) override { return kg_stream_timing(s_, &t, reset ? 1 : 0) == KG_OK; }
	int seed_group() const override { return cfg_.seed_group > 1 ? cfg_.seed_group : 0; }
	void group_absent(int lane, int rounds) override
	{
		if (kg_stream_group_absent(s_, lane, rounds) != KG_OK) die("kg_stream_group_absent");
	}
	void set_format(bool bam, bool bgzf) override
	{
		if (kg_stream_set_format(s_, !bam ? KG_STREAM_FORMAT_SAM : bgzf ? KG_STREAM_FORMAT_BAM_BGZF : KG_STREAM_FORMAT_BAM) != KG_OK) die("kg_stream_set_format");
	}
	void set_input(bool fasta) override
	{
		if (kg_stream_set_input(s_, fasta ? KG_STREAM_INPUT_FASTA : KG_STREAM_INPUT_FASTQ) != KG_OK) die("kg_stream_set_input");
	}
	void set_tags(bool md) override
	{
		if (kg_stream_set_tags(s_, md ? KG_STREAM_TAG_MD : 0) != KG_OK) die("kg_stream_set_tags");
	}
	void set_read_group(const std::string &id) override
	{
		if (kg_stream_set_read_group(s_, id.empty() ? nullptr : id.data(), (int)id.size()) != KG_OK) die("kg_stream_set_read_group");
	}
	void set_unmapped(bool on) override
	{
		if (kg_stream_set_unmapped(s_, on ? 1 : 0) != KG_OK) die("kg_stream_set_unmapped");
	}
	void set_stats(bool on) override
	{
		if (kg_stream_set_stats(s_, on ? 1 : 0) != KG_OK) die("kg_stream_set_stats");
	}
	kg_stream *handle() const { return s_; }

private:
	kg_stream *s_;
	kg_stream_config cfg_;
};

template <class T> struct PinnedBuf {
	T *p = nullptr;
	size_t cap = 0;
	~PinnedBuf() { if (p) kg_host_free(p); }
	T *get(size_t n)
	{
		if (n > cap) {
			if (p) kg_host_free(p);
			cap = n + n / 4 + 1024;
			p = (T *)kg_host_alloc(cap * sizeof(T));
			if (!p) { fprintf(stderr, "Error! out of page-locked memory\n"); exit(1); }
		}
		return p;
	}
};

class HipInflater : public MemberInflater {
public:
	explicit HipInflater(kg_inflater *k) : k_(k) {}
	~HipInflater() override { kg_inflater_destroy(k_); }
	unsigned char *src(size_t bytes) override
	{
		if ((int64_t)bytes > src_cap_) {
			if (kg_inflater_reserve(k_, (int64_t)bytes, 0, 0) != KG_OK) return nullptr;
			src_cap_ = (int64_t)bytes;
		}
		return kg_inflater_src(k_);
	}
	bool run(size_t src_bytes, const int64_t *member_off, const int64_t *text_off, size_t n, const unsigned char *&text, const int32_t *&status) override
	{
		if (kg_inflater_reserve(k_, 0, text_off[n], (int64_t)n) != KG_OK) return false;
		double ms = 0;
		const uint8_t *t = nullptr;
		if (kg_inflater_run(k_, (int64_t)src_bytes, member_off, text_off, (int64_t)n, &t, &status, &ms) != KG_OK) return false;
		text = t;
		ms_ += ms;
		return true;
	}
	double device_ms() const override { return ms_; }
private:
	kg_inflater *k_;
	int64_t src_cap_ = 0;
	double ms_ = 0;
};

class HipBackend : public KernelBackend {
public:
	double t_frag_in = 0, t_frag_call = 0; int64_t n_frag_calls = 0;
	double t_seed = 0, t_cands = 0, t_copy = 0, t_align = 0, t_reccopy = 0;
	HipBackend(kg_index *ix, const Options &opt) : ix_(ix), device_(opt.device), threads_(std::max(1, std::min(opt.threads, 16)))
	{
		kg_index_info(ix_, &info_);
		int64_t max_reads = std::max<int64_t>(opt.batch_reads, 4000ll * 4 * std::max(1, opt.threads)) + 8192;
		if (getenv("KART_AMD_TINY_WORKSPACE")) reserve(2048, 1 << 16);
		else reserve(max_reads, max_reads * 256);
	}
	int long_slot() const override { return cur_; }
	bool long_overlap() const override { return !getenv("KART_AMD_LONG_NO_OVERLAP"); }
	~HipBackend() override
	{
		stream_.reset();
		for (Slot &sl : slots_) {
			for (std::pair<kg_workspace *, int> &r : sl.retired) kg_workspace_destroy(r.first);
			if (sl.ws) kg_workspace_destroy(sl.ws);
		}
		kg_index_destroy(ix_);
	}
	bool has_stream() const override { return getenv("KART_AMD_NO_STREAM") == nullptr && getenv("KART_AMD_HOST_ALIGN") == nullptr; }
	StreamBackend *stream(int64_t max_reads, int64_t max_window, int lanes, int seed_group) override
	{
		static const bool off = getenv("KART_AMD_NO_STREAM") != nullptr || getenv("KART_AMD_HOST_ALIGN") != nullptr;
		if (off) return nullptr;
		if (seed_group < 2 || lanes % seed_group != 0) seed_group = 0;
		if (stream_ && stream_->max_reads() >= max_reads && stream_->max_window() >= max_window &&
		    (seed_group ? stream_->lanes() == lanes : stream_->lanes() >= lanes) && stream_->seed_group() == seed_group) return stream_.get();
		stream_.reset();
		kg_stream_config cfg;
		cfg.max_reads = max_reads; cfg.max_window = max_window; cfg.lanes = lanes; cfg.seed_group = seed_group;
		kg_stream *s = nullptr;
		if (kg_stream_open(ix_, &cfg, &s) != KG_OK) {
			fprintf(stderr, "Warning! no device stream (%s): the host parses and prints\n", kg_last_error());
			return nullptr;
		}
		stream_.reset(new HipStream(s, cfg));
		return stream_.get();
	}
	std::unique_ptr<MemberInflater> inflater() override
	{
		kg_inflater *k = nullptr;
		if (kg_inflater_create(device_, (int64_t)24 << 20, (int64_t)64 << 20, 4096, &k) != KG_OK) return nullptr;
		return std::unique_ptr<MemberInflater>(new HipInflater(k));
	}
	int min_seed_len() const override { return info_.min_seed_len; }
	void *host_alloc(size_t bytes) override { return kg_host_alloc(bytes); }
	void host_free(void *p) override { kg_host_free(p); }
	void seed_and_chain(int mode, bool pacbio, int max_gaps, const uint8_t *enc, const std::vector<int64_t> &off,
	                    std::vector<int32_t> &n_cands, std::vector<int64_t> &cand_off, std::vector<kg_candidate> &, std::vector<kg_seed> &,
	                    const kg_candidate *&cands, const kg_seed *&cand_seeds) override
	{
		int64_t n = (int64_t)off.size() - 1;
// ... 260 lines not shown
```

### kart_amd/csrc/host/knobs.inc

```
struct Knob { const char *name, *kind, *where, *what; };
static const Knob kKnobs[] = {
	{"KART_AMD_VERBOSE", "D", "host", "per-stage timers of the run on stdout (lane threads, device stages, writer, shards)"},
	{"KART_AMD_SA", "T", "host", "index mode: auto (default) | full | compact | wide | dense4 | dense8 | sampled (kg_index_load's sa_mode)"},
	{"KART_AMD_BATCH_READS", "T", "host", "reads per device call of the host reader's path (default 400000; whole 4000-read chunks)"},
	{"KART_AMD_STREAM_READS", "T", "host", "reads per batch of a device-stream lane (default 1120000)"},
	{"KART_AMD_STREAM_LANES", "T", "host", "lanes of the device stream (default: from the thread count, 8 at -t 16)"},
	{"KART_AMD_SEED_GROUP", "T", "host", "lanes whose batches are seeded by ONE search launch (default 4; 0: every lane seeds its own)"},
	{"KART_AMD_READER_THREADS", "T", "host", "threads of the host FASTQ reader (default (t + 1) / 2)"},
	{"KART_AMD_WRITER_THREADS", "T", "host", "threads copying text into the output file's mapping"},
	{"KART_AMD_PWRITE_THREADS", "T", "host", "of those, how many use pwrite() instead of the mapping (default 1 from 4 writer threads on)"},
	{"KART_AMD_WRITER_MODE", "A", "host", "0 a mapping per chunk, 1 windows unmapped once written (default), 2 windows + MADV_POPULATE_WRITE, 3 windows kept until the end"},
	{"KART_AMD_OUT_WINDOW_MB", "T", "host", "megabytes of the output file one shared mapping (window) of the writers covers (default 1024)"},
	{"KART_AMD_UNMAP_CPUS", "T", "host", "where the thread that unmaps written windows runs: io (the writers' CPUs, default) | lanes"},
	{"KART_AMD_WORKER_NICE", "T", "host", "nice value of the worker pool (default 5: the lane threads come first)"},
	{"KART_AMD_IO_CPUS", "T", "host", "CPU list the reader / writer threads are pinned to"},
	{"KART_AMD_LANE_CPUS", "T", "host", "CPU list the lane threads are pinned to"},
	{"KART_AMD_PREALLOC", "A", "host", "fallocate() the output ahead of the writers"},
	{"KART_AMD_NO_PREALLOC", "A", "host", "... and its off switch"},
	{"KART_AMD_NO_MMAP", "A", "host", "read plain FASTQ through getline() instead of the file's mapping"},
	{"KART_AMD_NO_MMAP_OUT", "A", "host", "write the output with pwrite() only"},
	{"KART_AMD_NO_PREAD", "A", "host", "fill the lanes' staging buffers by memcpy from the mapping instead of pread()"},
	{"KART_AMD_NO_PREFETCH", "D", "host", "the host reader's look-ahead on the main thread (profiling)"},
	{"KART_AMD_NO_BGZF", "A", "host", "inflate BGZF input as one gzip stream"},
	{"KART_AMD_NO_GZ_STREAM", "A", "host", "gz libraries through the host's gz reader (line index, views) instead of the device's FASTQ-in / SAM-out stream"},
	{"KART_AMD_GZ_NO_THP", "A", "host", "no transparent huge pages for the growing block a gz library is inflated into"},
	{"KART_AMD_GZ_AHEAD_MB", "T", "host", "megabytes of inflated text a gz library's thread may be ahead of the device stream (3072)"},
	{"KART_AMD_NO_PGZ", "A", "host", "ordinary gzip input through one gzread() stream per file instead of the several-thread reader"},
	{"KART_AMD_PGZ_CHUNK_KB", "T", "host", "compressed kilobytes per thread and round of the several-thread gzip reader (4096)"},
	{"KART_AMD_PGZ_MIN_KB", "T", "host", "smallest gzip file (compressed kilobytes) the several-thread reader takes (1024)"},
	{"KART_AMD_PGZ_DEBUG", "D", "host", "per-round timings of the several-thread gzip reader on stderr"},
	{"KART_AMD_NO_STREAM", "A", "host", "no device stream: the host parses FASTQ and prints SAM"},
	{"KART_AMD_FETCH_ALL", "A", "host", "the device stream copies every record and candidate of a batch back, not only those of the chunks the host asks for"},
	{"KART_AMD_HOST_ALIGN", "A", "host", "the per-read report on the host's workers (rounds 1-2)"},
	{"KART_AMD_HOST_LONG", "A", "host", "the -pacbio report on the host's workers (round 4)"},
	{"KART_AMD_HOST_FRAGMENTS", "A", "host", "fragment pairs planned by the host instead of kg_fragments_batch"},
	{"KART_AMD_FINISH_STRINGS", "A", "host", "the host's report pass 2 from gapped strings instead of op strings (rounds 2-3)"},
	{"KART_AMD_LONG_NO_OVERLAP", "A", "host", "-pacbio: one workspace, report and next seeding one after the other"},
	{"KART_AMD_PACBIO_CHUNKS", "T", "host", "-pacbio: chunks of the first batch"},
	{"KART_AMD_PACBIO_MAX_CHUNKS", "T", "host", "-pacbio: chunks of a full batch (batches double up to it)"},
	{"KART_AMD_FRAG_SLICE", "T", "host", "-pacbio on the host: fragment pairs per kg_fragments_batch call"},
	{"KART_AMD_FRAG_DEPTH", "T", "host", "... and how many such calls are in flight (1..3)"},
	{"KART_AMD_NO_EAGER_PARTS", "A", "host", "-parts shards hold their text back until the totals in front of them are known"},
	{"KART_AMD_NO_FILE_TURNS", "A", "host", "shards writing one file do not take turns at it"},
	{"KART_AMD_SHARD_TIMEOUT", "T", "host", "seconds a shard waits for another before it gives the run up (default 3600)"},
	{"KART_AMD_MEM_RESERVE_MB", "T", "host", "memory left to others when the output lives in tmpfs (default 512)"},
	{"KART_AMD_UNSET_FLAG", "D", "host", "what a FLAG the reference never assigns prints as (default 0; the tests use 1 << 20)"},
	{"KART_AMD_BACKTRACE", "D", "host", "kh_open installs a SIGSEGV / SIGABRT handler that prints the frames as library offsets"},
	{"KART_AMD_CHECK_ALIGN", "D", "host", "every read mapped on the host as well, device records compared with the host's text"},
	{"KART_AMD_TINY_WORKSPACE", "D", "host", "start with a workspace far too small (exercises growth while results are being read)"},
	{"KART_AMD_OUTPUT_NULL", "M", "host", "the run's text goes to /dev/null (bench.py: gpu_pipeline_value)"},
	{"KG_AUTO_COMPACT", "T", "index", "KG_SA_AUTO never takes the wide index (several processes are going to share the device)"},
	{"KG_QMER", "T", "index", "q of the q-mer table (8..16; default round(log4(2L)), one less in the compact index)"},
	{"KG_NO_QTAB", "A", "index", "no q-mer table: every search starts step by step"},
	{"KG_NO_PLANES2", "A", "index", "no two-step rank planes"},
	{"KG_NO_PLANES3", "A", "index", "no three-step rank planes"},
	{"KG_NO_DIRECT", "A", "index", "single-suffix searches are not finished against the text"},
	{"KG_FORCE_U64", "D", "index", "the 64-bit instantiations on a small index (tests)"},
	{"KG_SEARCH_BLOCKS_PER_CU", "T", "seed", "blocks of search_kernel per CU (default 6, at most 8)"},
	{"KG_FUSED_PACK", "A", "seed", "experiment: no pack pre-pass, the search reads raw codes"},
	{"KG_SORT_READS", "A", "seed", "experiment: reads drawn in the order of their first 16 bases"},
	{"KG_NO_SEGMENTS", "A", "seed", "SensitiveMode: one walk per read instead of walks from every segment start"},
	{"KG_SEG_LEN", "T", "seed", "SensitiveMode: segment length (default 512, at least 128)"},
	{"KG_SPIN_SYNC", "A", "stream", "hipStreamSynchronize instead of the blocking event wait"},
	{"KG_GROUP_NO_TURNS", "A", "stream", "the lanes of a seeding group start their stages at once"},
	{"KG_GROUP_TURN_EARLY", "A", "stream", "a lane passes its group's turn on before its copies back"},
	{"KG_STREAM_CHECKSUM", "M", "stream", "the SAM text of every batch summed on the device (kg_stream_timing_t::text_checksum)"},
	{"KG_ALN_NO_TRIVIAL", "A", "align", "no aln_trivial_kernel: every pair takes the general kernels"},
	{"KG_ALN_PAIR_HEAVY", "T", "align", "pairs with more candidate pairs (n1 x n2) than this are paired by the whole wave (32)"},
	{"KG_ALN_NO_HEAVY", "A", "align", "pairs with many candidates stay in their lane's loop instead of being the whole wave's"},
	{"KG_ALN_NO_FAST", "A", "align", "no aln_plan_fast_kernel (and no aln_trivial_kernel): every candidate takes aln_plan_kernel"},
	{"KG_ALN_NO_BINS", "A", "align", "aln_plan_kernel takes the candidates in their own order"},
	{"KG_RESCUE_SCAN", "A", "align", "the rescue kernel walks every diagonal of its window (rounds 2-3)"},
	{"KG_NW_NO_TIERS", "A", "align", "the wave-per-pair NW kernel in one tier"},
	{"KG_DBG_NO_PARTITION", "D", "align", "fragments that need the 8-mer partition go back to the host"},
	{"KG_DBG_SPILL_CAPACITY", "D", "align", "the spill list behaves as if it were this short (tests)"},
	{"KG_DBG_JOB_CAPACITY", "D", "align", "the NW job list likewise"},
	{"KG_DBG_OPS_CAPACITY", "D", "align", "the op-byte pool likewise"},
	{"KG_FRAG_NO_FAST_PAIRS", "A", "long", "IdentifyNormalPairs of a fragment on lane 0 only"},
	{"KG_FRAG_TWO_TIERS", "A", "long", "the partition kernel in two launch tiers"},
	{"KG_FRAG_PROF", "D", "long", "wave cycles per phase of the partition kernel"},
	{"KG_LONG_DEBUG", "D", "long", "dump of one read's long-read report"},
	{"KG_LONG_DEBUG_JOBS", "D", "long", "dump of the long-read report's NW jobs"},
	{"KG_LONG_DEBUG_STATUS", "D", "long", "fragment statuses of the long-read report"},
};
```

### kart_amd/csrc/host/mapper.cpp

```cpp
#include "mapper.hpp"

#include <fcntl.h>
#include <immintrin.h>
#include <sched.h>
#include <signal.h>
#include <pthread.h>
#include <sys/file.h>
#include <sys/mman.h>
#include <sys/resource.h>
#include <sys/stat.h>
#include <sys/statvfs.h>
#include <sys/vfs.h>
#include <sys/syscall.h>
#include <unistd.h>
#include <zlib.h>

#include <algorithm>
#include <cmath>
#include <cstdarg>
#include <cstdlib>
#include <atomic>
#include <climits>
#include <cstring>
#include <ctime>
#include <condition_variable>
#include <deque>
#include <functional>
#include <future>
#include <malloc.h>
#include <memory>
#include <mutex>
#include <string_view>
#include <thread>

namespace kart {

namespace {

#include "detail/types.inc"
#include "detail/normal_pairs.inc"
#include "detail/kmer.inc"
#include "detail/gap_closing.inc"
#include "detail/report.inc"
#include "detail/pairing.inc"
#include "detail/sam.inc"
#include "detail/bam.inc"
#include "detail/reader.inc"
#include "detail/shard.inc"
#include "detail/chunk_state.inc"
#include "detail/writer.inc"
#include "detail/chunk_stages.inc"
#include "detail/pgzip.inc"
#include "detail/batch_reader.inc"
#include "detail/deferred.inc"
#include "detail/pipeline.inc"
#include "detail/stream.inc"

}

bool RefData::load(const std::string &prefix, std::string &err, int threads)
{
	FILE *fp = fopen((prefix + ".ann").c_str(), "r");
	if (!fp) { err = "cannot read " + prefix + ".ann"; return false; }
	long long l_pac;
	int n_seqs;
	unsigned seed;
	if (fscanf(fp, "%lld%d%u", &l_pac, &n_seqs, &seed) != 3) { fclose(fp); err = "bad .ann header"; return false; }
	genome_size = l_pac;
	two_genome_size = 2 * genome_size;
	int64_t total = 0;
	for (int i = 0; i < n_seqs; ++i) {
		unsigned gi;
		char name[1024];
		long long offv;
		int len, n_ambs, ch;
		if (fscanf(fp, "%u%1023s", &gi, name) != 2) { fclose(fp); err = "bad .ann record"; return false; }
		while ((ch = fgetc(fp)) != '\n' && ch != EOF) {}
		if (fscanf(fp, "%lld%d%d", &offv, &len, &n_ambs) != 3) { fclose(fp); err = "bad .ann record"; return false; }
		Contig c;
		c.name = name;
		c.len = len;
		c.fwd_start = total;
		total += len;
		c.rev_start = two_genome_size - total;
		chr_end[c.fwd_start + c.len - 1] = i;
		chr_end[c.rev_start + c.len - 1] = i;
		contigs.push_back(c);
	}
	fclose(fp);
	if (FILE *fa = fopen((prefix + ".amb").c_str(), "r")) {
		long long l = 0, off = 0;
		int ns = 0, nh = 0, len = 0;
		char ch[4];
		if (fscanf(fa, "%lld%d%d", &l, &ns, &nh) == 3)
			for (int i = 0; i < nh && fscanf(fa, "%lld%d%1s", &off, &len, ch) == 3; ++i)
				if (off >= 0 && len > 0 && off + len <= genome_size) holes.push_back(Hole{off, len, (char)toupper((unsigned char)ch[0])});
		fclose(fa);
		std::sort(holes.begin(), holes.end(), [](const Hole &a, const Hole &b) { return a.start < b.start; });
	}
	std::vector<unsigned char> pac;
	if (!slurp(prefix + ".pac", pac) || (int64_t)pac.size() < genome_size / 4 + 1) { err = "cannot read " + prefix + ".pac"; return false; }
	{
		void *mem = nullptr;
		size_t bytes = (((size_t)two_genome_size + 1) + ((size_t)2 << 20) - 1) & ~(((size_t)2 << 20) - 1);
		if (posix_memalign(&mem, (size_t)2 << 20, bytes) != 0) { err = "out of memory for the reference sequence"; return false; }
		madvise(mem, bytes, MADV_HUGEPAGE);
		seq.reset((char *)mem);
	}
	seq[(size_t)two_genome_size] = '\0';
	std::vector<uint32_t> fw4(256), rc4(256);
	for (int v = 0; v < 256; ++v) {
		char f[4], r[4];
		for (int j = 0; j < 4; ++j) {
			int b = (v >> ((3 - j) << 1)) & 3;
			f[j] = "ACGT"[b];
			r[3 - j] = "TGCA"[b];
		}
		memcpy(&fw4[(size_t)v], f, 4);
		memcpy(&rc4[(size_t)v], r, 4);
	}
	int64_t whole = genome_size >> 2;
	int nt = (int)std::max<int64_t>(1, std::min<int64_t>(threads, whole >> 20));
	std::vector<std::thread> pool;
	char *out = seq.get();
	for (int t = 0; t < nt; ++t)
		pool.emplace_back([&, t]() {
			for (int64_t i = whole * t / nt, e = whole * (t + 1) / nt; i < e; ++i) {
				memcpy(out + (i << 2), &fw4[pac[(size_t)i]], 4);
				memcpy(out + (two_genome_size - (i << 2) - 4), &rc4[pac[(size_t)i]], 4);
			}
		});
	for (std::thread &th : pool) th.join();
	static const char fw[4] = {'A', 'C', 'G', 'T'}, rc[4] = {'T', 'G', 'C', 'A'};
	for (int64_t f = whole << 2; f < genome_size; ++f) {
		int b = pac[(size_t)(f >> 2)] >> ((~f & 3) << 1) & 3;
		seq[(size_t)f] = fw[b];
		seq[(size_t)(two_genome_size - 1 - f)] = rc[b];
	}
	return true;
}

int run_mapping(const Options &opt, const RefData &ref, KernelBackend &kern, FILE *out, Stats &stats)
{
	mallopt(M_MMAP_THRESHOLD, 1 << 30);
	mallopt(M_TRIM_THRESHOLD, -1);
	mallopt(M_TOP_PAD, 64 << 20);
	double t_begin = now_s();
	struct rusage ru0;
	getrusage(RUSAGE_SELF, &ru0);
	g_sections = getenv("KART_AMD_VERBOSE") != nullptr;
	{ const char *uf = getenv("KART_AMD_UNSET_FLAG"); g_unset_flag = uf ? atoi(uf) : 0; }
	run_error_reset();
	g_check_align = getenv("KART_AMD_CHECK_ALIGN") != nullptr;
	g_io_cpus = detect_io_cpus(opt.shard_count > 1 ? opt.shard_rank : -1);
	g_lane_cpus = IoCpus();
	{
		const char *e = getenv("KART_AMD_LANE_CPUS");
		if ((!e || !strcmp(e, "next")) && g_io_cpus.valid && opt.shard_count <= 1) {
			g_lane_cpus = detect_io_cpus(-2);
		} else if ((!e || !strcmp(e, "next")) && g_io_cpus.valid && opt.shard_count > 1 && count_l3_domains() >= 2 * opt.shard_count) {
			g_lane_cpus = detect_io_cpus(opt.shard_rank + opt.shard_count);
		}
	}
	Ctx cx{opt, ref, kern, kern.min_seed_len()};
	cx.frag_service = opt.pacbio && kern.has_fragments();
	struct UnFiles {
		FILE *fp[2] = {nullptr, nullptr};
		~UnFiles() { for (FILE *f : fp) if (f) fclose(f); }
	} un_files;
	for (int f = 0; f < 2; ++f) {
		const std::string &name = f ? opt.un2 : opt.un;
		if (name.empty()) continue;
		un_files.fp[f] = fopen(name.c_str(), "w+");
		if (!un_files.fp[f]) { fprintf(stderr, "Error! Cannot open file [%s]\n", name.c_str()); return 1; }
	}
	if (un_files.fp[0]) { cx.un_out[0] = un_files.fp[0]; cx.un_out[1] = un_files.fp[1]; }
	if (!opt.stats.empty() && !stats.tally) stats.tally = std::make_shared<Tally>();
	cx.stats = !opt.stats.empty();
	Options &o = const_cast<Options &>(opt);
	RunTotals tot;
	Shard shard;
	shard.rank = opt.shard_rank; shard.count = std::max(1, opt.shard_count);
	if (shard.active()) {
		if (shard.rank < 0 || shard.rank >= shard.count || shard.count > Rendezvous::kMaxRanks) { fprintf(stderr, "Error! bad shard %d/%d\n", shard.rank, shard.count); return 1; }
		shard.rdv = rendezvous_open(opt.rendezvous);
		if (!shard.rdv) { fprintf(stderr, "Error! cannot map the rendezvous file [%s]\n", opt.rendezvous.c_str()); return 1; }
		stats.sharded = true;
	}
	FILE *shard_out = nullptr;
	if (opt.bam)
		for (size_t i = 0; i < ref.contigs.size(); ++i) cx.bam_ref_id[ref.contigs[i].name] = (int)i;
	if (shard.rank == 0) {
		std::string header = "@PG\tID:kart\tPN:Kart\tVN:2.5.6\n";
		for (size_t i = 0; i < ref.contigs.size(); ++i) header += "@SQ\tSN:" + ref.contigs[i].name + "\tLN:" + std::to_string((long long)ref.contigs[i].len) + "\n";
		for (size_t i = 0; i < opt.read_groups.size(); ++i)
			if (std::find(opt.read_groups.begin(), opt.read_groups.begin() + (long)i, opt.read_groups[i]) == opt.read_groups.begin() + (long)i) header += opt.read_groups[i] + "\n";
		if (opt.bam) {
			std::string blocks;
			bgzf_append(bam_header(ref, header), blocks);
			fwrite(blocks.data(), 1, blocks.size(), out);
		} else fwrite(header.data(), 1, header.size(), out);
	}
	for (size_t lib = 0; lib < opt.files1.size(); ++lib) {
		const std::string &f1 = opt.files1[lib];
		bool gz = f1.size() >= 2 && f1.substr(f1.find_last_of('.') + 1) == "gz";
		cx.fastq = is_fastq(f1);
		cx.lib = lib;
		cx.rg_field = opt.read_groups.empty() ? std::string() : "\tRG:Z:" + opt.read_group_id(lib);
// ... 170 lines not shown
```

### kart_amd/csrc/host/mapper.hpp

```cpp
#pragma once
#include <cstdint>
#include <cstdio>
#include <cstdlib>
#include <map>
#include <memory>
#include <string>
#include <string_view>
#include <utility>
#include <vector>

#include "../../../include/kart_amd.h"

namespace kart {

struct Options {
	std::string index_prefix;
	std::vector<std::string> files1, files2;
	std::string out_name = "output.sam";
	int threads = 4;
	int max_gaps = 5;
	int max_insert = 1500;
	bool paired = false;
	bool pacbio = false;
	bool multi_hit = false;
	bool silent = false;
	bool bam = false;
	bool bz_device = false;
	bool md = false;
	std::vector<std::string> read_groups;
	std::string read_group_id(size_t lib) const;
	std::string un, un2;
	std::string stats;
	bool fz_device = false;
	int device = 0;
	std::vector<int> devices;
	int shard_rank = 0, shard_count = 1;
	std::string rendezvous;
	bool parts = false;
	int sa_mode = KG_SA_AUTO;
	int64_t batch_reads = default_batch_reads();
	int64_t stream_reads = default_stream_reads();
	static int64_t default_stream_reads() { const char *e = getenv("KART_AMD_STREAM_READS"); long long v = e ? atoll(e) : 0; return v >= 4000 ? (int64_t)v : 1120000; }
	static int64_t default_batch_reads() { const char *e = getenv("KART_AMD_BATCH_READS"); long long v = e ? atoll(e) : 0; return v >= 4000 ? (int64_t)v : 400000; }
};

struct NwJobs {
	std::string f1, f2;
	std::vector<int64_t> o1{0}, o2{0};
	std::vector<uint8_t> ops;
	std::vector<int32_t> len;
	int add(const char *a, int m, const char *b, int n)
	{
		f1.append(a, (size_t)m);
		f2.append(b, (size_t)n);
		o1.push_back((int64_t)f1.size());
		o2.push_back((int64_t)f2.size());
		return (int)o1.size() - 2;
	}
	size_t size() const { return o1.size() - 1; }
	void clear()
	{
		f1.clear(); f2.clear(); o1.assign(1, 0); o2.assign(1, 0); ops.clear(); len.clear();
	}
};

struct StreamBackend {
	virtual ~StreamBackend() {}
	virtual int lanes() const = 0;
	virtual int64_t max_reads() const = 0;
	virtual int64_t max_window() const = 0;
	virtual char *staging(int lane, int file) = 0;
	virtual void upload(int lane, int file, int64_t from, int64_t to) = 0;
	virtual bool parse(int lane, const kg_stream_window &w, kg_stream_parsed &out) = 0;
	virtual void map(int lane, const kg_stream_params &p, kg_stream_result &out) = 0;
	virtual void fetch(int lane, int64_t first, int64_t count) { (void)lane; (void)first; (void)count; }
	virtual bool timing(kg_stream_timing_t &t, bool reset) { (void)t; (void)reset; return false; }
	virtual int seed_group() const { return 0; }
	virtual void group_absent(int lane, int rounds) { (void)lane; (void)rounds; }
	virtual void set_format(bool bam, bool bgzf = false) { (void)bam; (void)bgzf; }
	virtual void set_input(bool fasta) { (void)fasta; }
	virtual void set_tags(bool md) { (void)md; }
	virtual void set_read_group(const std::string &id) { (void)id; }
	virtual void set_unmapped(bool on) { (void)on; }
	virtual void set_stats(bool on) { (void)on; }
};

struct FragJobs {
	std::string f1;
	std::vector<int64_t> o1{0}, g, oo;
	std::vector<int32_t> gl;
	std::vector<void *> owner;
	const uint8_t *ops = nullptr, *status = nullptr;
	const int32_t *len = nullptr;
	int64_t cols = 0;
	int add(const char *a, int m, int64_t gpos, int n, void *who)
	{
		f1.append(a, (size_t)m);
		o1.push_back((int64_t)f1.size());
		g.push_back(gpos); gl.push_back(n); oo.push_back(cols); owner.push_back(who);
		cols += m + n;
		return (int)g.size() - 1;
	}
	size_t size() const { return g.size(); }
	void clear() { f1.clear(); o1.assign(1, 0); g.clear(); oo.clear(); gl.clear(); owner.clear(); ops = status = nullptr; len = nullptr; cols = 0; }
};

struct MemberInflater {
	virtual ~MemberInflater() {}
	virtual unsigned char *src(size_t bytes) = 0;
	virtual bool run(size_t src_bytes, const int64_t *member_off, const int64_t *text_off, size_t n, const unsigned char *&text, const int32_t *&status) = 0;
	virtual double device_ms() const { return 0; }
};

struct KernelBackend {
	virtual ~KernelBackend() {}
	virtual std::unique_ptr<MemberInflater> inflater() { return nullptr; }
	virtual bool fragments_batch(std::vector<FragJobs *> &parts, bool pacbio, int max_gaps) { (void)parts; (void)pacbio; (void)max_gaps; return false; }
	virtual bool has_fragments() const { return false; }
	virtual bool has_stream() const { return false; }
	virtual StreamBackend *stream(int64_t max_reads, int64_t max_window, int lanes, int seed_group = 0) { (void)max_reads; (void)max_window; (void)lanes; (void)seed_group; return nullptr; }
	virtual int min_seed_len() const = 0;
	virtual void seed_and_chain(int mode, bool pacbio, int max_gaps, const uint8_t *enc, const std::vector<int64_t> &off,
	                            std::vector<int32_t> &n_cands, std::vector<int64_t> &cand_off, std::vector<kg_candidate> &own_cands,
	                            std::vector<kg_seed> &own_seeds, const kg_candidate *&cands, const kg_seed *&cand_seeds) = 0;
	virtual void *host_alloc(size_t bytes) { return malloc(bytes ? bytes : 1); }
	virtual void host_free(void *p) { free(p); }
	virtual void nw_batch(std::vector<NwJobs *> &parts) = 0;
	virtual bool align(const std::vector<int64_t> &chunk_off, const std::vector<uint8_t> &chunk_paired, int est, int max_insert, int max_gaps,
	                   bool multi_hit, int unset_flag, const kg_aln_record *&records, std::vector<kg_chunk_stats> &chunk_stats)
	{
		(void)chunk_off; (void)chunk_paired; (void)est; (void)max_insert; (void)max_gaps; (void)multi_hit; (void)unset_flag; (void)records; (void)chunk_stats;
		return false;
	}
	virtual bool align_long(int slot, const std::vector<int64_t> &chunk_off, const kg_aln_record *&records, const char *&cigar_pool, std::vector<kg_chunk_stats> &chunk_stats)
	{
		(void)slot; (void)chunk_off; (void)records; (void)cigar_pool; (void)chunk_stats;
		return false;
	}
	virtual int long_slot() const { return 0; }
	virtual bool long_enabled() const { return false; }
	virtual bool long_overlap() const { return false; }
	virtual std::string align_diagnostics() { return std::string(); }
};

struct Contig {
	std::string name;
	int64_t fwd_start, rev_start, len;
};

struct Hole {
	int64_t start, len;
	char ch;
};

struct RefData {
	int64_t genome_size = 0, two_genome_size = 0;
	std::vector<Contig> contigs;
	std::map<int64_t, int> chr_end;
	std::vector<Hole> holes;
	std::unique_ptr<char[], void (*)(void *)> seq{nullptr, free};
	bool load(const std::string &prefix, std::string &err, int threads = 16);
};

#include "detail/tally.inc"

struct Stats {
	std::shared_ptr<Tally> tally;
	int64_t total_reads = 0, unmapped = 0, unique = 0, paired = 0, distance = 0;
	double map_seconds = 0;
	int64_t respeculated = 0;
	int64_t rewritten_chunks = 0;
	int64_t stream_reads = 0;
	int64_t bgzf_device_bytes = 0, bgzf_host_bytes = 0;
	int64_t inflate_device_bytes = 0, inflate_host_bytes = 0;
	double inflate_device_ms = 0;
	kg_stream_timing_t device{};
	double lane_seconds[6] = {0, 0, 0, 0, 0, 0};
	int lanes = 0;
	bool sharded = false;
};

bool shard_totals(const std::string &rendezvous, int shard_count, Stats &sum);
void shard_mark_failed(const std::string &rendezvous, int rank = -1);
std::string run_error_message();

int run_mapping(const Options &opt, const RefData &ref, KernelBackend &kern, FILE *out, Stats &stats);

FILE *open_output(const std::string &path);
bool open_stats(const Options &opt, FILE *&fp);
bool write_stats(const Stats &st, FILE *fp);

int parse_cli(int argc, char **argv, Options &opt);

}
```

Measured before the change: 46.31 million.

## Double-buffer stream input text and prefetch blocks on per-lane feeder threads

```diff
diff --git a/include/kart_amd.h b/include/kart_amd.h
--- a/include/kart_amd.h
+++ b/include/kart_amd.h
@@ -220,6 +220,9 @@
 int   kg_stream_set_stats(kg_stream *s, int on);
 char *kg_stream_staging(kg_stream *s, int lane, int file, int64_t *capacity);
 int   kg_stream_upload(kg_stream *s, int lane, int file, int64_t from, int64_t to);
+char *kg_stream_staging_back(kg_stream *s, int lane, int file, int64_t *capacity);
+int   kg_stream_upload_back(kg_stream *s, int lane, int file, int64_t from, int64_t to);
+int   kg_stream_flip(kg_stream *s, int lane);
 
 typedef struct {
 	int64_t begin[2], end[2];
diff --git a/kart_amd/api.py b/kart_amd/api.py
--- a/kart_amd/api.py
+++ b/kart_amd/api.py
@@ -42,7 +42,7 @@
     "kg_index_contig", "kg_host_alloc", "kg_host_free", "kg_rank_sa_batch", "kg_workspace_create", "kg_workspace_destroy", "kg_workspace_counters", "kg_workspace_traffic",
     "kg_workspace_overflow", "kg_workspace_segment_fallbacks", "kg_workspace_set_profiling", "kg_workspace_set_single_steps", "kg_index_selfcheck", "kg_workspace_kernel_ms", "kg_seed_batch", "kg_candidates_batch", "kg_align_batch", "kg_align_reasons", "kg_seed_batch_device", "kg_nw_batch", "kg_nw_batch_device",
     "kg_fragments_batch", "kg_longread_batch", "kg_longread_reasons",
-    "kg_stream_open", "kg_stream_close", "kg_stream_staging", "kg_stream_upload", "kg_stream_parse", "kg_stream_map", "kg_stream_fetch", "kg_stream_fetch_reads", "kg_stream_timing",
+    "kg_stream_open", "kg_stream_close", "kg_stream_staging", "kg_stream_upload", "kg_stream_staging_back", "kg_stream_upload_back", "kg_stream_flip", "kg_stream_parse", "kg_stream_map", "kg_stream_fetch", "kg_stream_fetch_reads", "kg_stream_timing",
     "kg_stream_group_absent", "kg_stream_group_abort", "kg_stream_set_format", "kg_stream_set_input", "kg_stream_set_tags", "kg_stream_set_read_group", "kg_stream_set_unmapped",
     "kg_stream_set_stats", "kg_tally_records",
     "kg_bgzf_deflate", "kg_bgzf_inflate", "kg_inflater_create", "kg_inflater_reserve", "kg_inflater_src", "kg_inflater_run", "kg_inflater_destroy",
@@ -196,6 +196,10 @@
     L.kg_stream_staging.argtypes = [C.c_void_p, C.c_int, C.c_int, C.POINTER(C.c_int64)]
     L.kg_stream_staging.restype = C.c_void_p
     L.kg_stream_upload.argtypes = [C.c_void_p, C.c_int, C.c_int, C.c_int64, C.c_int64]
+    L.kg_stream_staging_back.argtypes = [C.c_void_p, C.c_int, C.c_int, C.POINTER(C.c_int64)]
+    L.kg_stream_staging_back.restype = C.c_void_p
+    L.kg_stream_upload_back.argtypes = [C.c_void_p, C.c_int, C.c_int, C.c_int64, C.c_int64]
+    L.kg_stream_flip.argtypes = [C.c_void_p, C.c_int]
     L.kg_stream_parse.argtypes = [C.c_void_p, C.c_int, C.POINTER(StreamWindow), C.POINTER(StreamParsed)]
     L.kg_stream_map.argtypes = [C.c_void_p, C.c_int, C.POINTER(StreamParams), C.POINTER(StreamResult)]
     L.kg_stream_fetch.argtypes = [C.c_void_p, C.c_int, C.c_int64, C.c_int64]
@@ -641,6 +645,33 @@
         _check(self.lib.kg_stream_parse(self.h, lane, C.byref(w), C.byref(out)), "kg_stream_parse")
         return out
 
+    def has_back(self, lane: int = 0) -> bool:
+        return bool(self.lib.kg_stream_staging_back(self.h, lane, 0, None))
+
+    def upload_back(self, text1: bytes, text2: bytes | None = None, begin=(0, 0), lane: int = 0):
+        for f, t in enumerate([text1] + ([text2] if text2 is not None else [])):
+            cap = C.c_int64()
+            p = self.lib.kg_stream_staging_back(self.h, lane, f, C.byref(cap))
+            assert p and begin[f] + len(t) <= cap.value
+            C.memmove(p + begin[f], t, len(t))
+            _check(self.lib.kg_stream_upload_back(self.h, lane, f, begin[f], begin[f] + len(t)), "kg_stream_upload_back")
+
+    def flip(self, lane: int = 0):
+        _check(self.lib.kg_stream_flip(self.h, lane), "kg_stream_flip")
+
+    def parse_front(self, len1: int, len2: int | None = None, paired: bool = True, chunk_reads: int = 4000, want_reads: int | None = None,
+                    eof=(True, True), begin=(0, 0), lane: int = 0) -> StreamParsed:
+        w = StreamWindow()
+        for f, n in enumerate([len1] + ([len2] if len2 is not None else [])):
+            w.begin[f], w.end[f], w.eof[f] = begin[f], begin[f] + n, 1 if eof[f] else 0
+        w.two_files = 1 if len2 is not None else 0
+        w.paired = 1 if paired else 0
+        w.chunk_reads = chunk_reads
+        w.want_reads = want_reads if want_reads is not None else chunk_reads
+        out = StreamParsed()
+        _check(self.lib.kg_stream_parse(self.h, lane, C.byref(w), C.byref(out)), "kg_stream_parse")
+        return out
+
     def fetch_reads(self, parsed: StreamParsed, lane: int = 0):
         off = np.zeros(parsed.n_reads + 1, dtype=np.int64)
         enc = np.zeros(max(1, parsed.n_bases), dtype=np.uint8)
diff --git a/kart_amd/csrc/abi_stream.hip b/kart_amd/csrc/abi_stream.hip
--- a/kart_amd/csrc/abi_stream.hip
+++ b/kart_amd/csrc/abi_stream.hip
@@ -5,6 +5,7 @@
 #include "bgzf_kernels.hpp"
 
 #include <algorithm>
+#include <atomic>
 #include <chrono>
 #include <condition_variable>
 #include <cstdlib>
@@ -34,6 +35,11 @@
 struct Lane {
 	kg_workspace *ws = nullptr;
 	uint8_t *d_text[2] = {nullptr, nullptr};
+	uint8_t *d_text_back[2] = {nullptr, nullptr};
+	char *h_text_back[2] = {nullptr, nullptr};
+	hipStream_t up_stream = nullptr;
+	bool up_stream_own = false;
+	hipEvent_t ev_text = nullptr, ev_text_back = nullptr;
 	int32_t *d_tile[2] = {nullptr, nullptr};
 	uint32_t *d_line_end[2] = {nullptr, nullptr};
 	uint32_t *d_rec[2] = {nullptr, nullptr};
@@ -153,6 +159,9 @@
 	bool stats = false;
 	uint8_t *d_rg = nullptr;
 	int rg_len = 0;
+	bool has_back = false;
+	hipStream_t up_shared = nullptr;
+	std::unique_ptr<std::atomic<int>[]> text_busy;
 	bool fasta_sized = false;
 	std::mutex mu;
 	kg_stream_timing_t total{};
@@ -160,10 +169,25 @@
 
 namespace {
 
+void free_back(Lane &l)
+{
+	for (int f = 0; f < 2; ++f) {
+		if (l.d_text_back[f]) (void)hipFree(l.d_text_back[f]);
+		if (l.h_text_back[f]) (void)hipHostFree(l.h_text_back[f]);
+		l.d_text_back[f] = nullptr; l.h_text_back[f] = nullptr;
+	}
+	if (l.ev_text) (void)hipEventDestroy(l.ev_text);
+	if (l.ev_text_back) (void)hipEventDestroy(l.ev_text_back);
+	if (l.up_stream && l.up_stream_own) (void)hipStreamDestroy(l.up_stream);
+	l.ev_text = l.ev_text_back = nullptr; l.up_stream = nullptr; l.up_stream_own = false;
+}
+
 void free_lane(Lane &l)
 {
 	if (l.ws && l.ws->enc_borrowed) l.ws->d_enc = nullptr;
 	if (l.ev_parsed) (void)hipEventDestroy(l.ev_parsed);
+	if (l.up_stream) (void)hipStreamSynchronize(l.up_stream);
+	free_back(l);
 	if (l.ws) kg_workspace_destroy(l.ws);
 	for (int f = 0; f < 2; ++f) {
 		if (l.d_text[f]) (void)hipFree(l.d_text[f]);
@@ -270,6 +294,29 @@
 	int accounted = sg.arrived;
 	for (int i = 0; i < sg.size; ++i) accounted += (!sg.present[i] && sg.absent_rounds[i] != 0) ? 1 : 0;
 	return accounted >= sg.size;
+}
+
+void open_back(kg_stream *s)
+{
+	static const bool one_upload = getenv("KG_STREAM_ONE_UPLOAD") != nullptr;
+	bool ok = true;
+	if (one_upload) ok = hipStreamCreateWithFlags(&s->up_shared, hipStreamNonBlocking) == hipSuccess;
+	for (size_t li = 0; ok && li < s->lanes.size(); ++li) {
+		Lane &l = s->lanes[li];
+		if (one_upload) l.up_stream = s->up_shared;
+		else { ok = hipStreamCreateWithFlags(&l.up_stream, hipStreamNonBlocking) == hipSuccess; l.up_stream_own = ok; }
+		ok = ok && hipEventCreateWithFlags(&l.ev_text, hipEventDisableTiming) == hipSuccess;
+		ok = ok && hipEventCreateWithFlags(&l.ev_text_back, hipEventDisableTiming) == hipSuccess;
+		for (int f = 0; ok && f < 2; ++f) {
+			ok = hipMalloc((void **)&l.d_text_back[f], (size_t)s->text_capacity) == hipSuccess;
+			ok = ok && hipHostMalloc((void **)&l.h_text_back[f], (size_t)s->text_capacity, hipHostMallocDefault) == hipSuccess;
+		}
+	}
+	s->has_back = ok;
+	if (ok) return;
+	(void)hipGetLastError();
+	for (Lane &l : s->lanes) free_back(l);
+	if (s->up_shared) { (void)hipStreamDestroy(s->up_shared); s->up_shared = nullptr; }
 }
 
 float elapsed(hipEvent_t a, hipEvent_t b)
@@ -381,6 +428,9 @@
 		HIP_TRY(hipHostMalloc((void **)&l.h_records, sizeof(kg_aln_record) * (size_t)l.record_capacity, hipHostMallocDefault));
 		for (hipEvent_t &e : l.ev) HIP_TRY(hipEventCreate(&e));
 	}
+	s->text_busy.reset(new std::atomic<int>[s->lanes.size()]);
+	for (size_t li = 0; li < s->lanes.size(); ++li) s->text_busy[li].store(0);
+	open_back(s.get());
 	HIP_TRY(hipDeviceSynchronize());
 	*out = s.release();
 	return KG_OK;
@@ -399,6 +449,7 @@
 	if (s->d_chr_names) (void)hipFree(s->d_chr_names);
 	if (s->d_chr_name_off) (void)hipFree(s->d_chr_name_off);
 	if (s->d_rg) (void)hipFree(s->d_rg);
+	if (s->up_shared) (void)hipStreamDestroy(s->up_shared);
 	delete s;
 }
 
@@ -554,6 +605,40 @@
 	Lane &l = s->lanes[(size_t)lane];
 	HIP_TRY(hipSetDevice(s->ix->device));
 	HIP_TRY(hipMemcpyAsync(l.d_text[file] + from, l.h_text[file] + from, (size_t)(to - from), hipMemcpyHostToDevice, l.ws->stream));
+	return KG_OK;
+}
+
+char *kg_stream_staging_back(kg_stream *s, int lane, int file, int64_t *capacity)
+{
+	if (!s || lane < 0 || lane >= (int)s->lanes.size() || file < 0 || file > 1 || !s->has_back) return nullptr;
+	if (capacity) *capacity = s->cfg.max_window;
+	return s->lanes[(size_t)lane].h_text_back[file];
+}
+
+int kg_stream_upload_back(kg_stream *s, int lane, int file, int64_t from, int64_t to)
+{
+	if (!s || lane < 0 || lane >= (int)s->lanes.size() || file < 0 || file > 1) return fail(KG_ERR_ARG, "kg_stream_upload_back: bad argument");
+	if (!s->has_back) return fail(KG_ERR_ARG, "kg_stream_upload_back: the stream has no back input buffers (kg_stream_staging_back returns null)");
+	if (from < 0 || to < from || to > s->cfg.max_window) return fail(KG_ERR_ARG, "kg_stream_upload_back: range [%lld, %lld) outside the staging buffer", (long long)from, (long long)to);
+	if (to == from) return KG_OK;
+	Lane &l = s->lanes[(size_t)lane];
+	HIP_TRY(hipSetDevice(s->ix->device));
+	HIP_TRY(hipMemcpyAsync(l.d_text_back[file] + from, l.h_text_back[file] + from, (size_t)(to - from), hipMemcpyHostToDevice, l.up_stream));
+	HIP_TRY(hipEventRecord(l.ev_text_back, l.up_stream));
+	return KG_OK;
+}
+
+int kg_stream_flip(kg_stream *s, int lane)
+{
+	if (!s || lane < 0 || lane >= (int)s->lanes.size()) return fail(KG_ERR_ARG, "kg_stream_flip: bad argument");
+	if (!s->has_back) return fail(KG_ERR_ARG, "kg_stream_flip: the stream has no back input buffers (kg_stream_staging_back returns null)");
+	if (s->text_busy[(size_t)lane].load() != 0) return fail(KG_ERR_ARG, "kg_stream_flip: lane %d holds a parsed batch that kg_stream_map has not returned from", lane);
+	Lane &l = s->lanes[(size_t)lane];
+	HIP_TRY(hipSetDevice(s->ix->device));
+	HIP_TRY(hipStreamWaitEvent(l.ws->stream, l.ev_text_back, 0));
+	for (int f = 0; f < 2; ++f) { std::swap(l.d_text[f], l.d_text_back[f]); std::swap(l.h_text[f], l.h_text_back[f]); }
+	std::swap(l.ev_text, l.ev_text_back);
+	l.have_batch = false;
 	return KG_OK;
 }
 
@@ -614,6 +699,7 @@
 	}
 	HIP_TRY(hipEventRecord(l.ev[1], st));
 	l.have_batch = p.n_reads > 0;
+	s->text_busy[(size_t)lane].store(l.have_batch ? 1 : 0);
 	*out = p;
 	return KG_OK;
 }
@@ -1060,6 +1146,7 @@
 	m.n_chunks = (int)l.parsed.n_chunks;
 	m.grouped = !s->groups.empty();
 	GroupTurn turn;
+	struct TextFree { std::atomic<int> &busy; ~TextFree() { busy.store(0); } } text_free{s->text_busy[(size_t)lane]};
 	int rc;
 	if ((rc = map_seed(s, lane, m, turn)) != KG_OK) return rc;
 	if ((rc = map_chain(l, m)) != KG_OK) return rc;
diff --git a/kart_amd/csrc/host/detail/block_ahead.inc b/kart_amd/csrc/host/detail/block_ahead.inc
--- /dev/null
+++ b/kart_amd/csrc/host/detail/block_ahead.inc
@@ -0,0 +1,74 @@
+template <class Block> class BlockAhead {
+public:
+	explicit BlockAhead(int lanes) : slots_((size_t)lanes) {}
+
+	bool wait_free(int lane, int64_t s)
+	{
+		std::unique_lock<std::mutex> lk(mu_);
+		Slot &x = slots_[(size_t)lane];
+		cv_.wait(lk, [&]() { return failed_ || s >= end_ || x.state == kEmpty; });
+		return !failed_ && s < end_;
+	}
+	bool stage(int lane, int64_t s, const Block &blk)
+	{
+		std::lock_guard<std::mutex> lk(mu_);
+		Slot &x = slots_[(size_t)lane];
+		if (failed_ || s >= end_) return false;
+		if (x.state != kEmpty) { failed_ = true; misuse_ = true; cv_.notify_all(); return false; }
+		x.state = kStaged; x.seq = s; x.blk = blk;
+		cv_.notify_all();
+		return true;
+	}
+	void no_more(int lane)
+	{
+		std::lock_guard<std::mutex> lk(mu_);
+		slots_[(size_t)lane].no_more = true;
+		cv_.notify_all();
+	}
+	bool take(int lane, int64_t s, Block &blk)
+	{
+		std::unique_lock<std::mutex> lk(mu_);
+		Slot &x = slots_[(size_t)lane];
+		cv_.wait(lk, [&]() { return failed_ || s >= end_ || (x.state == kStaged && x.seq == s) || (x.no_more && x.state != kStaged); });
+		if (failed_ || s >= end_ || x.state != kStaged) return false;
+		blk = x.blk;
+		x.state = kTaken;
+		return true;
+	}
+	void release(int lane)
+	{
+		std::lock_guard<std::mutex> lk(mu_);
+		Slot &x = slots_[(size_t)lane];
+		if (x.state != kTaken) { failed_ = true; misuse_ = true; }
+		x.state = kEmpty;
+		cv_.notify_all();
+	}
+	void end(int64_t first_missing)
+	{
+		std::lock_guard<std::mutex> lk(mu_);
+		end_ = std::min(end_, first_missing);
+		cv_.notify_all();
+	}
+	void fail()
+	{
+		std::lock_guard<std::mutex> lk(mu_);
+		failed_ = true;
+		cv_.notify_all();
+	}
+	bool failed() { std::lock_guard<std::mutex> lk(mu_); return failed_; }
+	bool misused() { std::lock_guard<std::mutex> lk(mu_); return misuse_; }
+
+private:
+	enum State { kEmpty, kStaged, kTaken };
+	struct Slot {
+		State state = kEmpty;
+		int64_t seq = -1;
+		bool no_more = false;
+		Block blk{};
+	};
+	std::mutex mu_;
+	std::condition_variable cv_;
+	std::vector<Slot> slots_;
+	int64_t end_ = INT64_MAX;
+	bool failed_ = false, misuse_ = false;
+};
diff --git a/kart_amd/csrc/host/detail/stream.inc b/kart_amd/csrc/host/detail/stream.inc
--- a/kart_amd/csrc/host/detail/stream.inc
+++ b/kart_amd/csrc/host/detail/stream.inc
@@ -357,41 +357,6 @@
 }
 
 constexpr size_t kNoEnd = ~(size_t)0;
-
-inline int64_t stream_block_bytes(int64_t want, int nf, int64_t batches_between, size_t raw, size_t pos, double bpr, int64_t bulk_cap)
-{
-	const double recs = (double)want / (double)nf;
-	double outstanding = (double)(raw - pos) - (double)batches_between * recs * bpr;
-	if (outstanding < 0) outstanding = 0;
-	const double w = recs * bpr * 1.02 + 65536 - outstanding;
-	return (int64_t)std::max(0.0, std::min(w, (double)bulk_cap));
-}
-
-struct WindowPlace {
-	int64_t begin = 0, end = 0;
-	bool eof = false;
-	size_t abs0 = 0;
-	size_t text_begin = 0, text_end = 0;
-	bool fits = false;
-};
-inline WindowPlace stream_place_window(size_t blk0, size_t blk1, size_t pos, size_t file_end, int64_t carry_cap)
-{
-	const int64_t carry = (int64_t)(blk0 - pos);
-	WindowPlace p;
-	p.fits = carry <= carry_cap;
-	p.begin = carry_cap - carry;
-	p.end = carry_cap + (int64_t)(blk1 - blk0);
-	p.eof = blk1 == file_end;
-	p.abs0 = blk0 - (size_t)carry_cap;
-	p.text_begin = blk0 - (size_t)std::max<int64_t>(0, carry);
-	p.text_end = blk1;
-	return p;
-}
-
-struct StreamBlock {
-	size_t blk0[2] = {0, 0}, blk1[2] = {0, 0};
-	int64_t want = 0;
-};
 
 struct StreamFeed {
 	std::mutex mu;
@@ -582,6 +547,8 @@
 	std::unique_ptr<BamPacker> packer;
 	std::vector<std::unique_ptr<StreamBatch>> batches;
 	LaneTimers timers;
+	std::unique_ptr<BlockAhead<StreamBlock>> ahead;
+	std::atomic<int64_t> feeder_ns{0};
 
 	StreamRun(Ctx &cx_, Source &src_, StreamBackend &sb_, Writer *writer_, Stats &st_, RunTotals &tot_, std::atomic<int> &est_latest_,
 	          std::vector<DeferredChunk> *held_, int64_t &bytes_out_, const Shard *shard_)
@@ -625,6 +592,25 @@
 		pool.reset(new TaskPool(std::max(1, cx.opt.threads / 2), 5));
 		if (cx.opt.bam && writer && !held) packer.reset(new BamPacker(writer, std::max(1, cx.opt.threads), &feed.mu, &feed.cv));
 		for (int l = 0; l < K; ++l) { batches.emplace_back(new StreamBatch()); batches.back()->lane = l; }
+		const char *ahead_env = getenv("KART_AMD_STREAM_AHEAD");
+		bool have_back = !(ahead_env && atoi(ahead_env) == 0);
+		for (int l = 0; have_back && l < K; ++l)
+			for (int f = 0; f < nf; ++f) have_back = have_back && sb.staging_back(l, f) != nullptr;
+		if (have_back) ahead.reset(new BlockAhead<StreamBlock>(K));
+	}
+
+	void feeder_thread(int lane)
+	{
+		pin_lane_thread();
+		for (int64_t s = lane;; s += K) {
+			StreamBlock blk;
+			if (!ahead->wait_free(lane, s)) return;
+			double t0 = now_s();
+			if (!feed.claim_block(s, bulk_cap, full_target, blk)) { ahead->no_more(lane); return; }
+			read_block(lane, blk, true);
+			feeder_ns += (int64_t)((now_s() - t0) * 1e9);
+			if (!ahead->stage(lane, s, blk)) return;
+		}
 	}
 
 	void lane_thread(int lane)
@@ -638,14 +624,32 @@
 	{
 		StreamBlock blk;
 		kg_stream_window w{};
-		if (!wait_lane_free(b, s)) return false;
-		if (!feed.claim_block(s, bulk_cap, full_target, blk)) return false;
-		read_and_upload(b.lane, blk);
-		if (!place_window(b, s, blk, w)) return false;
-		parse_and_publish(b, s, blk.want, w);
+		if (ahead) {
+			if (!take_staged(b.lane, s, blk)) return false;
+			if (!wait_lane_free(b, s)) return false;
+			sb.flip(b.lane);
+			ahead->release(b.lane);
+		} else {
+			if (!wait_lane_free(b, s)) return false;
+			if (!feed.claim_block(s, bulk_cap, full_target, blk)) return false;
+			double t0 = now_s();
+			read_block(b.lane, blk, false);
+			timers.add(LaneTimers::kReadUpload, t0);
+		}
+		const bool placed = place_window(b, s, blk, w);
+		if (placed) parse_and_publish(b, s, blk.want, w);
+		if (ahead && (!placed || b.last)) ahead->end(s + 1);
+		if (!placed) return false;
 		map_or_sit_out(b);
 		feed.hand_over(s, b);
 		return !b.last;
+	}
+	bool take_staged(int lane, int64_t s, StreamBlock &blk)
+	{
+		double t0 = now_s();
+		const bool got = ahead->take(lane, s, blk);
+		timers.add(LaneTimers::kReadUpload, t0);
+		return got;
 	}
 	bool wait_lane_free(StreamBatch &b, int64_t s)
 	{
@@ -654,12 +658,11 @@
 		timers.add(LaneTimers::kWaitLane, t0);
 		return true;
 	}
-	void read_and_upload(int lane, const StreamBlock &blk)
-	{
-		double t0 = now_s();
+	void read_block(int lane, const StreamBlock &blk, bool back)
+	{
 		for (int f = 0; f < nf; ++f) {
 			const MappedFile &mf = file_of(src, f);
-			char *stg = sb.staging(lane, f);
+			char *stg = back ? sb.staging_back(lane, f) : sb.staging(lane, f);
 			const size_t piece = (size_t)8 << 20, blk0 = blk.blk0[f], blk1 = blk.blk1[f];
 			for (size_t a = blk0; a < blk1; a += piece) {
 				size_t e = std::min(blk1, a + piece);
@@ -675,10 +678,10 @@
 					done = got == e - a;
 				}
 				if (!done) memcpy(stg + carry_cap + (a - blk0), mf.data + a, e - a);
-				sb.upload(lane, f, carry_cap + (int64_t)(a - blk0), carry_cap + (int64_t)(e - blk0));
-			}
-		}
-		timers.add(LaneTimers::kReadUpload, t0);
+				if (back) sb.upload_back(lane, f, carry_cap + (int64_t)(a - blk0), carry_cap + (int64_t)(e - blk0));
+				else sb.upload(lane, f, carry_cap + (int64_t)(a - blk0), carry_cap + (int64_t)(e - blk0));
+			}
+		}
 	}
 	bool place_window(StreamBatch &b, int64_t s, const StreamBlock &blk, kg_stream_window &w)
 	{
@@ -881,9 +884,11 @@
 		for (int i = 0; i < LaneTimers::kSteps; ++i) st.lane_seconds[i] += timers.seconds(i);
 		st.lanes = K;
 		if (verbose)
-			fprintf(stdout, "stream: lane-thread seconds (summed over %d lanes): waiting for the lane %.3f | read + upload %.3f | waiting for the parse before %.3f | parse %.3f | map (device) %.3f | host reads %.3f\n", K,
-			        timers.seconds(LaneTimers::kWaitLane), timers.seconds(LaneTimers::kReadUpload), timers.seconds(LaneTimers::kWaitParse), timers.seconds(LaneTimers::kParse),
-			        timers.seconds(LaneTimers::kMap), timers.seconds(LaneTimers::kHostReads));
+			fprintf(stdout, "stream: lane-thread seconds (summed over %d lanes): waiting for the lane %.3f | %s %.3f | waiting for the parse before %.3f | parse %.3f | map (device) %.3f | host reads %.3f\n", K,
+			        timers.seconds(LaneTimers::kWaitLane), ahead ? "waiting for the staged block" : "read + upload", timers.seconds(LaneTimers::kReadUpload), timers.seconds(LaneTimers::kWaitParse),
+			        timers.seconds(LaneTimers::kParse), timers.seconds(LaneTimers::kMap), timers.seconds(LaneTimers::kHostReads));
+		if (verbose && ahead)
+			fprintf(stdout, "stream: feeder-thread seconds (summed over %d lanes): claim + read + upload of the next blocks %.3f\n", K, 1e-9 * (double)feeder_ns.load());
 		kg_stream_timing_t t{};
 		if (!sb.timing(t, true) || t.batches <= 0) return;
 		add_timing(st.device, t);
@@ -900,10 +905,13 @@
 	StreamRun run(cx, src, sb, writer, st, tot, est_latest, held, bytes_out, shard);
 	run.prime(ramp_from);
 	for (int l = 0; l < run.K; ++l) sb.group_absent(l, 0);
-	std::vector<std::thread> threads;
+	std::vector<std::thread> threads, feeders;
+	for (int l = 0; run.ahead && l < run.K; ++l) feeders.emplace_back([&run, l]() { run.feeder_thread(l); });
 	for (int l = 0; l < run.K; ++l) threads.emplace_back([&run, l]() { run.lane_thread(l); });
 	run.commit();
 	for (std::thread &t : threads) t.join();
+	if (run.ahead) run.ahead->end(0);
+	for (std::thread &t : feeders) t.join();
 	run.finish();
 	run.report();
 	return !run.feed.fallback;
diff --git a/kart_amd/csrc/host/detail/stream_blocks.inc b/kart_amd/csrc/host/detail/stream_blocks.inc
--- /dev/null
+++ b/kart_amd/csrc/host/detail/stream_blocks.inc
@@ -0,0 +1,35 @@
+
+inline int64_t stream_block_bytes(int64_t want, int nf, int64_t batches_between, size_t raw, size_t pos, double bpr, int64_t bulk_cap)
+{
+	const double recs = (double)want / (double)nf;
+	double outstanding = (double)(raw - pos) - (double)batches_between * recs * bpr;
+	if (outstanding < 0) outstanding = 0;
+	const double w = recs * bpr * 1.02 + 65536 - outstanding;
+	return (int64_t)std::max(0.0, std::min(w, (double)bulk_cap));
+}
+
+struct WindowPlace {
+	int64_t begin = 0, end = 0;
+	bool eof = false;
+	size_t abs0 = 0;
+	size_t text_begin = 0, text_end = 0;
+	bool fits = false;
+};
+inline WindowPlace stream_place_window(size_t blk0, size_t blk1, size_t pos, size_t file_end, int64_t carry_cap)
+{
+	const int64_t carry = (int64_t)(blk0 - pos);
+	WindowPlace p;
+	p.fits = carry <= carry_cap;
+	p.begin = carry_cap - carry;
+	p.end = carry_cap + (int64_t)(blk1 - blk0);
+	p.eof = blk1 == file_end;
+	p.abs0 = blk0 - (size_t)carry_cap;
+	p.text_begin = blk0 - (size_t)std::max<int64_t>(0, carry);
+	p.text_end = blk1;
+	return p;
+}
+
+struct StreamBlock {
+	size_t blk0[2] = {0, 0}, blk1[2] = {0, 0};
+	int64_t want = 0;
+};
diff --git a/kart_amd/csrc/host/hip_backend.cpp b/kart_amd/csrc/host/hip_backend.cpp
--- a/kart_amd/csrc/host/hip_backend.cpp
+++ b/kart_amd/csrc/host/hip_backend.cpp
@@ -42,6 +42,15 @@
 	void upload(int lane, int file, int64_t from, int64_t to) override
 	{
 		if (kg_stream_upload(s_, lane, file, from, to) != KG_OK) die("kg_stream_upload");
+	}
+	char *staging_back(int lane, int file) override { return kg_stream_staging_back(s_, lane, file, nullptr); }
+	void upload_back(int lane, int file, int64_t from, int64_t to) override
+	{
+		if (kg_stream_upload_back(s_, lane, file, from, to) != KG_OK) die("kg_stream_upload_back");
+	}
+	void flip(int lane) override
+	{
+		if (kg_stream_flip(s_, lane) != KG_OK) die("kg_stream_flip");
 	}
 	bool parse(int lane, const kg_stream_window &w, kg_stream_parsed &out) override
 	{
diff --git a/kart_amd/csrc/host/knobs.inc b/kart_amd/csrc/host/knobs.inc
--- a/kart_amd/csrc/host/knobs.inc
+++ b/kart_amd/csrc/host/knobs.inc
@@ -20,6 +20,7 @@
 	{"KART_AMD_NO_MMAP", "A", "host", "read plain FASTQ through getline() instead of the file's mapping"},
 	{"KART_AMD_NO_MMAP_OUT", "A", "host", "write the output with pwrite() only"},
 	{"KART_AMD_NO_PREAD", "A", "host", "fill the lanes' staging buffers by memcpy from the mapping instead of pread()"},
+	{"KART_AMD_STREAM_AHEAD", "A", "host", "0: no feeder threads -- a stream lane claims, reads and uploads its block itself, after the batch before it in the lane is written"},
 	{"KART_AMD_NO_PREFETCH", "D", "host", "the host reader's look-ahead on the main thread (profiling)"},
 	{"KART_AMD_NO_BGZF", "A", "host", "inflate BGZF input as one gzip stream"},
 	{"KART_AMD_NO_GZ_STREAM", "A", "host", "gz libraries through the host's gz reader (line index, views) instead of the device's FASTQ-in / SAM-out stream"},
@@ -64,6 +65,7 @@
 	{"KG_SPIN_SYNC", "A", "stream", "hipStreamSynchronize instead of the blocking event wait"},
 	{"KG_GROUP_NO_TURNS", "A", "stream", "the lanes of a seeding group start their stages at once"},
 	{"KG_GROUP_TURN_EARLY", "A", "stream", "a lane passes its group's turn on before its copies back"},
+	{"KG_STREAM_ONE_UPLOAD", "A", "stream", "the lanes' back input buffers are uploaded on ONE stream instead of one per lane"},
 	{"KG_STREAM_CHECKSUM", "M", "stream", "the SAM text of every batch summed on the device (kg_stream_timing_t::text_checksum)"},
 	{"KG_ALN_NO_TRIVIAL", "A", "align", "no aln_trivial_kernel: every pair takes the general kernels"},
 	{"KG_ALN_PAIR_HEAVY", "T", "align", "pairs with more candidate pairs (n1 x n2) than this are paired by the whole wave (32)"},
diff --git a/kart_amd/csrc/host/mapper.cpp b/kart_amd/csrc/host/mapper.cpp
--- a/kart_amd/csrc/host/mapper.cpp
+++ b/kart_amd/csrc/host/mapper.cpp
@@ -54,6 +54,8 @@
 #include "detail/batch_reader.inc"
 #include "detail/deferred.inc"
 #include "detail/pipeline.inc"
+#include "detail/stream_blocks.inc"
+#include "detail/block_ahead.inc"
 #include "detail/stream.inc"
 
 }
diff --git a/kart_amd/csrc/host/mapper.hpp b/kart_amd/csrc/host/mapper.hpp
--- a/kart_amd/csrc/host/mapper.hpp
+++ b/kart_amd/csrc/host/mapper.hpp
@@ -71,6 +71,9 @@
 	virtual int64_t max_window() const = 0;
 	virtual char *staging(int lane, int file) = 0;
 	virtual void upload(int lane, int file, int64_t from, int64_t to) = 0;
+	virtual char *staging_back(int lane, int file) { (void)lane; (void)file; return nullptr; }
+	virtual void upload_back(int lane, int file, int64_t from, int64_t to) { (void)lane; (void)file; (void)from; (void)to; }
+	virtual void flip(int lane) { (void)lane; }
 	virtual bool parse(int lane, const kg_stream_window &w, kg_stream_parsed &out) = 0;
 	virtual void map(int lane, const kg_stream_params &p, kg_stream_result &out) = 0;
 	virtual void fetch(int lane, int64_t first, int64_t count) { (void)lane; (void)first; (void)count; }
```

Result: slower. 43.09 million (-7.0%).
